# AgoraIO-Community/Solo

Measured on AMD Instinct MI355X. Metric: 40 ms frames/sec (encode+decode) per GPU; concurrent real-time WB streams @1/2/4/8 MI355X, higher is better.
Workload: dtype int32 fixed point (int16 PCM, Q-format arithmetic, bit-exact); 1 GPU; BASELINE configs[2]: 4096 synthetic 16 kHz WB streams, full encode -> two-description bitstream -...; streams_per_gpu=4096, input_workers=16, launch=single process

## Files before the change

include/solo_mi355x.h:

```cpp
#ifndef SOLO_MI355X_H
#define SOLO_MI355X_H

#include <stdint.h>

#ifdef __cplusplus
extern "C" {
#endif

typedef struct {
    int32_t mode;
    int32_t targetRate_bps;
    int32_t samplerate;
    int32_t dtx_enable;
    int32_t framesize_ms;
    int32_t joint_enable;
    int32_t joint_mode;
    int32_t useMDIndex;
} USER_Ctrl_enc;

typedef struct {
    int32_t packetLoss_perc;
    int32_t samplerate;
    int32_t framesize_ms;
    int32_t joint_enable;
// ... 44 lines not shown
int32_t solo_batch_decode_streams(solo_batch_t *b, const int32_t *d_streams, int32_t n, const uint8_t *d_bits,
                                  const int16_t *d_nbytes, const uint8_t *d_recv, int32_t n_packets, int16_t *d_pcm,
                                  int32_t *d_status, void *hip_stream);
int32_t solo_recv_decode_streams(solo_batch_t *b, const int32_t *d_streams, int32_t n, int32_t n_packets, int16_t *d_pcm,
                                 int32_t *d_status, void *hip_stream);
typedef struct {
    int32_t  play;
    int32_t  queued;
    int32_t  complete;
    int32_t  ready;
    int32_t  span;
    int32_t  head;
    uint32_t inserted, late, ahead, duplicate, bad;
    uint32_t played_both, played_md1, played_md2, played_none;
    int32_t  margin_min;
} solo_recv_report_t;
typedef struct { int32_t selected, listed; } solo_recv_report_count_t;

#define SOLO_RECV_REPORT_CLEAR_MARGIN 1

int32_t solo_recv_track(solo_batch_t *b, int32_t on, void *hip_stream);
int32_t solo_recv_report(solo_batch_t *b, const int32_t *d_streams, int32_t n,
                         const int32_t *d_min_ready, int32_t min_ready, int32_t max_span, int32_t flags,
                         solo_recv_report_t *d_reports, int32_t *d_play_list, int32_t *d_play_rows,
                         solo_recv_report_count_t *d_count, void *hip_stream);
typedef struct {
    int32_t records, records_needed;
    int64_t bytes, bytes_needed;
    int32_t empty, refused;
} solo_send_count_t;
int32_t solo_send_pack(solo_batch_t *b, const uint8_t *d_bits, const int16_t *d_nbytes, const uint8_t *d_send,
                       int32_t n_packets, const int32_t *d_seq_base, int32_t first_seq,
                       solo_arrival_t *d_records, int32_t max_records, uint8_t *d_payload, int64_t payload_capacity,
                       solo_send_count_t *d_count, void *hip_stream);
int32_t solo_send_pack_streams(solo_batch_t *b, const int32_t *d_streams, int32_t n, const uint8_t *d_bits, const int16_t *d_nbytes,
                               const uint8_t *d_send, int32_t n_packets, const int32_t *d_seq_base, int32_t first_seq,
                               solo_arrival_t *d_records, int32_t max_records, uint8_t *d_payload, int64_t payload_capacity,
                               solo_send_count_t *d_count, void *hip_stream);
typedef struct {
    int32_t rows, rooms;
    int64_t clipped;
} solo_mix_count_t;
int32_t solo_mix(solo_batch_t *b, const int16_t *d_pcm_in, int32_t n, int32_t n_packets,
                 const int32_t *d_room, int32_t n_rooms, const int16_t *d_gain_q12, int32_t max_speakers,
                 int16_t *d_pcm_out, int64_t *d_energy, uint8_t *d_mixed,
                 solo_mix_count_t *d_count, void *hip_stream);
typedef struct solo_resampler solo_resampler_t;
typedef struct { int32_t rows, listed; } solo_resample_count_t;
solo_resampler_t *solo_resample_create(int32_t n_rows, int32_t fs_in, int32_t fs_out);
void solo_resample_destroy(solo_resampler_t *r);
int32_t solo_resample_out_samples(const solo_resampler_t *r, int32_t in_samples);
int32_t solo_resample_reset(solo_resampler_t *r, void *hip_stream);
int32_t solo_resample_reset_rows(solo_resampler_t *r, const int32_t *h_rows, int32_t n, void *hip_stream);
int32_t solo_resample(solo_resampler_t *r, const int16_t *d_in, int32_t n_packets, int32_t in_samples,
                      int16_t *d_out, void *hip_stream);
int32_t solo_resample_rows(solo_resampler_t *r, const int32_t *d_rows, int32_t n, const int16_t *d_in, int32_t n_packets,
                           int32_t in_samples, int16_t *d_out, solo_resample_count_t *d_count, void *hip_stream);
typedef struct { int32_t streams, refused; int64_t bytes; } solo_migrate_count_t;
int64_t solo_batch_state_bytes(const solo_batch_t *b, int32_t which);
int32_t solo_batch_export_streams(solo_batch_t *b, const int32_t *d_streams, int32_t n, int32_t which,
                                  uint8_t *d_blob, int64_t blob_stride, solo_migrate_count_t *d_count, void *hip_stream);
int32_t solo_batch_import_streams(solo_batch_t *b, const int32_t *d_streams, int32_t n, int32_t which,
                                  const uint8_t *d_blob, int64_t blob_stride, solo_migrate_count_t *d_count, void *hip_stream);
int32_t solo_batch_set_async_join(solo_batch_t *b, int32_t on);
int32_t solo_batch_wait_encode(solo_batch_t *b, void *hip_stream, int32_t which);
int32_t solo_batch_n_streams(const solo_batch_t *b);
int32_t solo_batch_slot_bytes(const solo_batch_t *b);
const char *solo_kernel_name(int32_t which);
int32_t solo_batch_set_timing(solo_batch_t *b, int32_t on);
int32_t solo_batch_last_kernel_ms(solo_batch_t *b, float *ms4);
int32_t solo_batch_last_encode_chunks(const solo_batch_t *b);
int32_t solo_debug_l0(int32_t op, int32_t n, const int32_t *d_a, const int32_t *d_b, const int32_t *d_c, int32_t *d_out);
int32_t solo_debug_sum_sqr_shift(const int16_t *d_x, int32_t rows, int32_t len, int32_t stride, int32_t odd_start,
                                 int32_t *d_energy, int32_t *d_shift);
int32_t solo_debug_waveops(int32_t mode, int32_t n_vec, int32_t waves_per_block, const int32_t *d_v, const int32_t *d_aux,
                           int32_t *d_out);
int32_t solo_debug_rowops(const int32_t *d_in, const int32_t *d_idx, int32_t *d_out, void *hip_stream);
int32_t solo_debug_nsq(int32_t n_streams, int32_t n_packets, const void *h_in, void *h_out);
int32_t solo_debug_nsq_ex(int32_t samplerate, int32_t silk_rate_bps, int32_t useMDIndex, int32_t joint, int32_t dtx, int32_t frames_per_packet,
                          int32_t n_streams, int32_t n_packets, const void *h_in, void *h_out);
int32_t solo_debug_analysis(int32_t samplerate, int32_t silk_rate_bps, int32_t useMDIndex, int32_t joint, int32_t dtx, int32_t frames_per_packet,
                            int32_t n_streams, int32_t n_packets, int32_t chunk, const int16_t *h_pcm, void *h_nsq_in, void *h_code_in,
                            int32_t *h_sizes);
int32_t solo_debug_coding(int32_t samplerate, int32_t silk_rate_bps, int32_t useMDIndex, int32_t joint, int32_t dtx, int32_t frames_per_packet,
                          int32_t n_streams, int32_t n_packets, int32_t chunk, int32_t slot_bytes, const void *h_code_in, const void *h_nsq_out,
                          uint8_t *h_bits, int16_t *h_nbytes, int32_t *h_status);
int32_t solo_debug_dec_extract(int32_t samplerate, int32_t useMDIndex, int32_t joint, int32_t frames_per_packet, int32_t n_streams,
                               int32_t n_packets, int32_t chunk, int32_t slot_bytes, const uint8_t *h_bits, const int16_t *h_nbytes,
                               const uint8_t *h_recv, void *h_recs, int32_t *h_counts);
int32_t solo_debug_dec_synth(int32_t samplerate, int32_t useMDIndex, int32_t joint, int32_t frames_per_packet, int32_t n_streams,
                             int32_t n_packets, int32_t chunk, int32_t slot_bytes, const uint8_t *h_bits, const int16_t *h_nbytes,
                             const uint8_t *h_recv, const void *h_recs, int16_t *h_pcm, int32_t *h_status, void *h_state, int32_t state_bytes);
int32_t solo_debug_clock(double *mhz_out);
const char *solo_version(void);

#ifdef __cplusplus
}
#endif
#endif
```

solo_amd/__init__.py:

```python
import ctypes as C
import os

_HERE = os.path.dirname(os.path.abspath(__file__))
LIB_PATH = os.environ.get("SOLO_LIB_OVERRIDE") or os.path.join(_HERE, "libsolo_mi355x.so")

PACKET_SAMPLES = 640
DEFAULT_SLOT_BYTES = 512

ABI_SYMBOLS = [
    "AGR_Sate_Encoder_Init", "AGR_Sate_Encoder_Encode", "AGR_Sate_Encoder_Uninit",
    "AGR_Sate_Decoder_Init", "AGR_Sate_Decoder_Decode", "AGR_Sate_Decoder_Uninit",
    "solo_batch_create", "solo_batch_destroy", "solo_batch_reset", "solo_batch_encode", "solo_batch_decode",
    "solo_batch_n_streams", "solo_batch_slot_bytes", "solo_kernel_name", "solo_version", "solo_batch_set_timing",
    "solo_batch_last_kernel_ms", "solo_batch_last_encode_chunks", "solo_batch_decode_split", "solo_batch_set_async_join",
    "solo_batch_wait_encode", "solo_debug_l0", "solo_debug_sum_sqr_shift", "solo_debug_rowops", "solo_debug_clock", "solo_debug_nsq",
    "solo_debug_waveops", "solo_debug_nsq_ex", "solo_debug_analysis", "solo_debug_coding", "solo_debug_dec_extract", "solo_debug_dec_synth",
    "solo_recv_create", "solo_recv_insert", "solo_recv_decode", "solo_recv_stats",
    "solo_batch_reset_streams", "solo_recv_reset_streams", "solo_batch_update_streams",
    "solo_batch_encode_streams", "solo_batch_decode_streams", "solo_recv_decode_streams",
    "solo_send_pack", "solo_send_pack_streams", "solo_mix", "solo_recv_track", "solo_recv_report",
    "solo_batch_state_bytes", "solo_batch_export_streams", "solo_batch_import_streams",
    "solo_resample_create", "solo_resample_destroy", "solo_resample_out_samples", "solo_resample_reset", "solo_resample_reset_rows",
    "solo_resample", "solo_resample_rows",
]


class USER_Ctrl_enc(C.Structure):
    _fields_ = [(n, C.c_int32) for n in (
        "mode", "targetRate_bps", "samplerate", "dtx_enable", "framesize_ms",
        "joint_enable", "joint_mode", "useMDIndex")]


class USER_Ctrl_dec(C.Structure):
    _fields_ = [(n, C.c_int32) for n in (
        "packetLoss_perc", "samplerate", "framesize_ms", "joint_enable", "joint_mode", "useMDIndex")]


class solo_send_count_t(C.Structure):
    _fields_ = [("records", C.c_int32), ("records_needed", C.c_int32), ("bytes", C.c_int64), ("bytes_needed", C.c_int64),
                ("empty", C.c_int32), ("refused", C.c_int32)]


class solo_mix_count_t(C.Structure):
    _fields_ = [("rows", C.c_int32), ("rooms", C.c_int32), ("clipped", C.c_int64)]


class solo_resample_count_t(C.Structure):
    _fields_ = [("rows", C.c_int32), ("listed", C.c_int32)]


class solo_migrate_count_t(C.Structure):
    _fields_ = [("streams", C.c_int32), ("refused", C.c_int32), ("bytes", C.c_int64)]


class solo_recv_report_t(C.Structure):
    _fields_ = [(n, C.c_int32) for n in ("play", "queued", "complete", "ready", "span", "head")] + \
               [(n, C.c_uint32) for n in ("inserted", "late", "ahead", "duplicate", "bad", "played_both", "played_md1", "played_md2", "played_none")] + \
               [("margin_min", C.c_int32)]


class solo_recv_report_count_t(C.Structure):
    _fields_ = [("selected", C.c_int32), ("listed", C.c_int32)]


RECV_REPORT_CLEAR_MARGIN = 1

_lib = None


def kernel_source_hash():
    import hashlib
    h = hashlib.sha256()
    d = os.path.join(_HERE, "csrc")
    for f in sorted(os.listdir(d)):
        if f.endswith((".h", ".hip", ".inc")):
            h.update(f.encode())
            h.update(open(os.path.join(d, f), "rb").read())
    flags = build_flags()
    if flags:
        h.update(" ".join(flags).encode())
    return h.hexdigest()[:16]


def build_flags():
    p = os.path.join(_HERE, "build_flags.txt")
    if not os.path.exists(p):
        return []
    return [l.strip() for l in open(p) if l.strip() and not l.strip().startswith("#")]


def load_library():
    global _lib
    if _lib is not None:
        return _lib
    if not os.path.exists(LIB_PATH):
        raise RuntimeError("libsolo_mi355x.so is not built (%s). Run `python -c 'import __graft_entry__ as g; g.build()'`; "
                           "this package has no CPU fallback." % LIB_PATH)
    lib = C.CDLL(LIB_PATH)
    lib.solo_batch_create.restype = C.c_void_p
# ... 3 lines not shown
    lib.solo_batch_reset.restype = C.c_int32
    lib.solo_batch_reset_streams.restype = C.c_int32
    lib.solo_batch_reset_streams.argtypes = [C.c_void_p, C.c_void_p, C.c_int32, C.c_int32, C.c_void_p, C.c_void_p, C.c_void_p]
    lib.solo_batch_update_streams.restype = C.c_int32
    lib.solo_batch_update_streams.argtypes = [C.c_void_p, C.c_void_p, C.c_int32, C.c_int32, C.c_void_p, C.c_void_p, C.c_void_p]
    lib.solo_recv_reset_streams.restype = C.c_int32
    lib.solo_recv_reset_streams.argtypes = [C.c_void_p, C.c_void_p, C.c_int32, C.c_void_p, C.c_void_p]
    lib.solo_batch_encode.restype = C.c_int32
    lib.solo_batch_encode.argtypes = [C.c_void_p, C.c_void_p, C.c_int32, C.c_void_p, C.c_void_p, C.c_void_p, C.c_void_p]
    lib.solo_batch_encode_streams.restype = C.c_int32
    lib.solo_batch_encode_streams.argtypes = [C.c_void_p, C.c_void_p, C.c_int32, C.c_void_p, C.c_int32, C.c_void_p, C.c_void_p, C.c_void_p, C.c_void_p]
    lib.solo_batch_decode_streams.restype = C.c_int32
    lib.solo_batch_decode_streams.argtypes = [C.c_void_p, C.c_void_p, C.c_int32, C.c_void_p, C.c_void_p, C.c_void_p, C.c_int32, C.c_void_p, C.c_void_p,
                                              C.c_void_p]
    lib.solo_recv_decode_streams.restype = C.c_int32
    lib.solo_recv_decode_streams.argtypes = [C.c_void_p, C.c_void_p, C.c_int32, C.c_int32, C.c_void_p, C.c_void_p, C.c_void_p]
    lib.solo_batch_decode.restype = C.c_int32
    lib.solo_batch_decode.argtypes = [C.c_void_p, C.c_void_p, C.c_void_p, C.c_void_p, C.c_int32, C.c_void_p, C.c_void_p, C.c_void_p]
    lib.solo_batch_n_streams.argtypes = [C.c_void_p]
    lib.solo_batch_slot_bytes.argtypes = [C.c_void_p]
    lib.solo_batch_set_timing.restype = C.c_int32
    lib.solo_batch_set_timing.argtypes = [C.c_void_p, C.c_int32]
    lib.solo_batch_last_kernel_ms.restype = C.c_int32
    lib.solo_batch_last_kernel_ms.argtypes = [C.c_void_p, C.c_void_p]
    lib.solo_batch_decode_split.restype = C.c_int32
    lib.solo_batch_decode_split.argtypes = [C.c_void_p, C.c_void_p, C.c_void_p, C.c_void_p, C.c_void_p, C.c_int32, C.c_int32, C.c_void_p,
                                            C.c_void_p, C.c_void_p]
    lib.solo_recv_create.restype = C.c_int32
    lib.solo_recv_create.argtypes = [C.c_void_p, C.c_int32, C.c_int32, C.c_int32, C.c_void_p]
    lib.solo_recv_insert.restype = C.c_int32
    lib.solo_recv_insert.argtypes = [C.c_void_p, C.c_void_p, C.c_int32, C.c_void_p, C.c_int64, C.c_void_p]
    lib.solo_recv_decode.restype = C.c_int32
    lib.solo_recv_decode.argtypes = [C.c_void_p, C.c_int32, C.c_void_p, C.c_void_p, C.c_void_p]
    lib.solo_recv_stats.restype = C.c_int32
    lib.solo_recv_stats.argtypes = [C.c_void_p, C.c_void_p, C.c_void_p]
    lib.solo_recv_track.restype = C.c_int32
    lib.solo_recv_track.argtypes = [C.c_void_p, C.c_int32, C.c_void_p]
    lib.solo_recv_report.restype = C.c_int32
    lib.solo_recv_report.argtypes = [C.c_void_p, C.c_void_p, C.c_int32, C.c_void_p, C.c_int32, C.c_int32, C.c_int32, C.c_void_p, C.c_void_p, C.c_void_p,
                                     C.c_void_p, C.c_void_p]
    _send = [C.c_void_p, C.c_void_p, C.c_void_p, C.c_int32, C.c_void_p, C.c_int32, C.c_void_p, C.c_int32, C.c_void_p, C.c_int64, C.c_void_p, C.c_void_p]
    lib.solo_send_pack.restype = C.c_int32
    lib.solo_send_pack.argtypes = [C.c_void_p] + _send
    lib.solo_send_pack_streams.restype = C.c_int32
    lib.solo_send_pack_streams.argtypes = [C.c_void_p, C.c_void_p, C.c_int32] + _send
    lib.solo_mix.restype = C.c_int32
    lib.solo_mix.argtypes = [C.c_void_p, C.c_void_p, C.c_int32, C.c_int32, C.c_void_p, C.c_int32, C.c_void_p, C.c_int32, C.c_void_p, C.c_void_p, C.c_void_p,
                             C.c_void_p, C.c_void_p]
    lib.solo_batch_state_bytes.restype = C.c_int64
    lib.solo_batch_state_bytes.argtypes = [C.c_void_p, C.c_int32]
    for f in (lib.solo_batch_export_streams, lib.solo_batch_import_streams):
        f.restype = C.c_int32
        f.argtypes = [C.c_void_p, C.c_void_p, C.c_int32, C.c_int32, C.c_void_p, C.c_int64, C.c_void_p, C.c_void_p]
    lib.solo_resample_create.restype = C.c_void_p
    lib.solo_resample_create.argtypes = [C.c_int32, C.c_int32, C.c_int32]
    lib.solo_resample_destroy.restype = None
    lib.solo_resample_destroy.argtypes = [C.c_void_p]
    lib.solo_resample_out_samples.restype = C.c_int32
    lib.solo_resample_out_samples.argtypes = [C.c_void_p, C.c_int32]
    lib.solo_resample_reset.restype = C.c_int32
    lib.solo_resample_reset.argtypes = [C.c_void_p, C.c_void_p]
    lib.solo_resample_reset_rows.restype = C.c_int32
    lib.solo_resample_reset_rows.argtypes = [C.c_void_p, C.c_void_p, C.c_int32, C.c_void_p]
    lib.solo_resample.restype = C.c_int32
    lib.solo_resample.argtypes = [C.c_void_p, C.c_void_p, C.c_int32, C.c_int32, C.c_void_p, C.c_void_p]
    lib.solo_resample_rows.restype = C.c_int32
    lib.solo_resample_rows.argtypes = [C.c_void_p, C.c_void_p, C.c_int32, C.c_void_p, C.c_int32, C.c_int32, C.c_void_p, C.c_void_p, C.c_void_p]
    lib.solo_batch_set_async_join.restype = C.c_int32
    lib.solo_batch_set_async_join.argtypes = [C.c_void_p, C.c_int32]
    lib.solo_batch_wait_encode.restype = C.c_int32
    lib.solo_batch_wait_encode.argtypes = [C.c_void_p, C.c_void_p, C.c_int32]
    lib.solo_batch_last_encode_chunks.restype = C.c_int32
    lib.solo_batch_last_encode_chunks.argtypes = [C.c_void_p]
    lib.solo_debug_rowops.restype = C.c_int32
    lib.solo_debug_rowops.argtypes = [C.c_void_p, C.c_void_p, C.c_void_p, C.c_void_p]
    lib.solo_debug_waveops.restype = C.c_int32
    lib.solo_debug_waveops.argtypes = [C.c_int32, C.c_int32, C.c_int32, C.c_void_p, C.c_void_p, C.c_void_p]
    lib.solo_debug_nsq.restype = C.c_int32
    lib.solo_debug_nsq.argtypes = [C.c_int32, C.c_int32, C.c_void_p, C.c_void_p]
    lib.solo_debug_nsq_ex.restype = C.c_int32
    lib.solo_debug_nsq_ex.argtypes = [C.c_int32] * 8 + [C.c_void_p, C.c_void_p]
    lib.solo_debug_analysis.restype = C.c_int32
    lib.solo_debug_analysis.argtypes = [C.c_int32] * 9 + [C.c_void_p, C.c_void_p, C.c_void_p, C.c_void_p]
    lib.solo_debug_coding.restype = C.c_int32
    lib.solo_debug_coding.argtypes = [C.c_int32] * 10 + [C.c_void_p, C.c_void_p, C.c_void_p, C.c_void_p, C.c_void_p]
    lib.solo_debug_dec_extract.restype = C.c_int32
    lib.solo_debug_dec_extract.argtypes = [C.c_int32] * 8 + [C.c_void_p] * 5
    lib.solo_debug_dec_synth.restype = C.c_int32
    lib.solo_debug_dec_synth.argtypes = [C.c_int32] * 8 + [C.c_void_p] * 7 + [C.c_int32]
    lib.solo_debug_clock.restype = C.c_int32
    lib.solo_debug_clock.argtypes = [C.c_void_p]
    lib.solo_kernel_name.restype = C.c_char_p
    lib.solo_kernel_name.argtypes = [C.c_int32]
    lib.solo_version.restype = C.c_char_p
    lib.AGR_Sate_Encoder_Init.restype = C.c_void_p
    lib.AGR_Sate_Encoder_Init.argtypes = [C.c_void_p]
    lib.AGR_Sate_Encoder_Encode.restype = C.c_int32
    lib.AGR_Sate_Encoder_Encode.argtypes = [C.c_void_p, C.c_void_p, C.c_void_p, C.c_int32, C.c_void_p]
    lib.AGR_Sate_Encoder_Uninit.argtypes = [C.c_void_p]
    lib.AGR_Sate_Decoder_Init.restype = C.c_void_p
    lib.AGR_Sate_Decoder_Init.argtypes = [C.c_void_p]
    lib.AGR_Sate_Decoder_Decode.restype = C.c_int32
    lib.AGR_Sate_Decoder_Decode.argtypes = [C.c_void_p, C.c_void_p, C.c_void_p, C.c_void_p, C.c_void_p, C.c_int32]
    lib.AGR_Sate_Decoder_Uninit.argtypes = [C.c_void_p]
    _lib = lib
    return lib


def shader_clock_mhz():
    v = C.c_double(0.0)
    if load_library().solo_debug_clock(C.byref(v)) != 0:
        return None
    return float(v.value)


def default_enc_ctrl(rate=13600, use_md_index=0, joint=0, dtx=0, samplerate=16000, framesize_ms=40):
    return USER_Ctrl_enc(mode=2, targetRate_bps=rate, samplerate=samplerate, dtx_enable=1 if dtx else 0, framesize_ms=framesize_ms,
                         joint_enable=1 if joint else 0, joint_mode=1 if joint else 0, useMDIndex=use_md_index)


def default_dec_ctrl(use_md_index=0, joint=0, samplerate=16000, framesize_ms=40):
    return USER_Ctrl_dec(packetLoss_perc=0, samplerate=samplerate, framesize_ms=framesize_ms, joint_enable=1 if joint else 0,
                         joint_mode=1 if joint else 0, useMDIndex=use_md_index)


class SoloBatch:

    def __init__(self, n_streams, rate=13600, encoder=True, decoder=True, slot_bytes=DEFAULT_SLOT_BYTES, use_md_index=0, joint=0, dtx=0,
                 samplerate=16000, framesize_ms=40):
        import torch
        if not torch.cuda.is_available():
            raise RuntimeError("solo_amd needs a HIP device (MI355X); there is no CPU path")
        self.torch = torch
        self.lib = load_library()
        self.n_streams = int(n_streams)
        self.slot = int(slot_bytes)
        if framesize_ms not in (20, 40):
            raise ValueError("framesize_ms must be 40 or 20")
        self._enc = default_enc_ctrl(rate, use_md_index, joint, dtx, samplerate, framesize_ms) if encoder else None
        if samplerate not in (16000, 32000):
            raise ValueError("samplerate must be 16000 or 32000")
        self.packet_samples = PACKET_SAMPLES * samplerate // 16000 * framesize_ms // 40
        self._dec = default_dec_ctrl(use_md_index, joint, samplerate, framesize_ms) if decoder else None
        self.h = self.lib.solo_batch_create(self.n_streams, C.byref(self._enc) if encoder else None,
                                            C.byref(self._dec) if decoder else None, self.slot)
        if not self.h:
            raise RuntimeError("solo_batch_create failed (unsupported configuration, no GPU, or out of memory)")
        self.device = torch.device("cuda", torch.cuda.current_device())

    def _stream(self):
        return C.c_void_p(self.torch.cuda.current_stream().cuda_stream)

    def reset(self):
        r = self.lib.solo_batch_reset(self.h, self._stream())
        if r:
            raise RuntimeError("solo_batch_reset -> %d" % r)

    _WHICH = {"enc": 1, "encoder": 1, "dec": 2, "decoder": 2, "both": 3, 1: 1, 2: 2, 3: 3}

    def _stream_list(self, streams):
        idx = [int(s) for s in (streams.tolist() if hasattr(streams, "tolist") else streams)]
        if not 0 < len(idx) <= self.n_streams:
            raise ValueError("between 1 and %d streams must be listed" % self.n_streams)
        if any(s < 0 or s >= self.n_streams for s in idx):
            raise ValueError("stream index out of range")
        if len(set(idx)) != len(idx):
# ... 529 lines not shown
```

solo_amd/csrc/solo_api.hip:

```cpp
#include <hip/hip_runtime.h>
#include <vector>
#include <stdio.h>
#include <stdlib.h>
#include <string.h>
#include <new>

#include "../../include/solo_mi355x.h"
#include "solo_dec.h"

#define SOLO_CHECK(expr)                                        \
    do {                                                        \
        hipError_t e_ = (expr);                                 \
        if (e_ != hipSuccess) return -(int32_t)e_;              \
    } while (0)

#include "solo_dec_kernels.h"
#include "solo_l0_probe.h"
#include "solo_send.h"
#include "solo_mix.h"
#include "solo_recv_report.h"
#include "solo_migrate.h"
#include "solo_resample.h"

__global__ void __launch_bounds__(64) solo_l0_probe_kernel(int op, int n, const i32* a, const i32* b, const i32* c, i32* out) {
// ... 67 lines not shown
        i32 z = sx_lcg_first(aux0);
        ROW(21, z);
        z = sx_lcg_next(z); ROW(22, z);
        z = sx_lcg_next(z); ROW(23, z);
        z = sx_lcg_next(z); ROW(24, z);
        const i32 vmin = wv_min(v);
        ROW(25, vmin);
        ROW(26, wv_min(v == vmin ? lane : SX_I32_MAX));
    } else {
        i32 a, b, c, d, e, f, g;
        i64 h;
        SOLO_WAVEOPS_CHAIN(v)
        ROW(0, a); ROW(1, b); ROW(2, c); ROW(3, d); ROW(4, e); ROW(5, f); ROW(6, g); ROW(7, (u32)h); ROW(8, (u32)((u64)h >> 32));
        const int trips = (aux0 & 7) + 1;
        i32 x = v;
        for (int t = 0; t < trips; t++) {
            if (t) x = sx_add(sx_add(x, a), sx_add(f, sx_add(g, (i32)(u32)h)));
            SOLO_WAVEOPS_CHAIN(x)
        }
        ROW(9, a); ROW(10, b); ROW(11, c); ROW(12, d); ROW(13, e); ROW(14, f); ROW(15, g); ROW(16, (u32)h); ROW(17, (u32)((u64)h >> 32));
    }
#undef ROW
#endif
}

__global__ void __launch_bounds__(256) solo_stream_list_check_kernel(const i32* map, int n, int n_streams, u32* verdict, i32* status) {
    __shared__ int bad;
    if (threadIdx.x == 0) bad = 0;
    __syncthreads();
    int mine = 0;
    for (int i = threadIdx.x; i < n; i += 256) {
        const i32 v = map[i];
        if (v < 0 || v >= n_streams || (i > 0 && map[i - 1] >= v)) mine = 1;
    }
    if (mine) atomicOr(&bad, 1);
    __syncthreads();
    const int verdict_bad = bad;
    if (threadIdx.x == 0) *verdict = (u32)verdict_bad;
    if (verdict_bad && status)
        for (int i = threadIdx.x; i < n; i += 256) status[i] = -1;
}

extern "C" const solo_dec_ops* solo_nb_dec_ops() { return &solo_dec_ops_table; }
extern "C" const solo_dec_ops* solo_wb_dec_ops();

#ifdef SOLO_WITH_ENCODER
#include "solo_enc_ops.h"
extern "C" int solo_launch_gate(const unsigned int* flag, unsigned int target, void* hip_stream);
extern "C" const solo_enc_ops* solo_nb_enc_ops();
extern "C" const solo_enc_ops* solo_wb_enc_ops();
#endif

#define SOLO_MAX_CHUNKS 64
#define SOLO_N_VERDICTS 10
struct solo_batch {
    int32_t n_streams;
    int32_t slot;
    int have_enc, have_dec;
    USER_Ctrl_enc enc_ctrl;
    USER_Ctrl_dec dec_ctrl;
    void* d_enc_state;
#ifdef SOLO_WITH_ENCODER
    const solo_enc_ops* eops;
#endif
    void* d_nsq_ring;
    hipStream_t sP, sS;
    hipEvent_t evDFork, evDJoin, evDJoin2, evP[2], evS[2];
    void* d_parsed[2];
    size_t parsed_bytes;
    int parsed_two;
    int dec_pipe_ready, dec_split, dec_chunk, dec_first;
    size_t dec_scratch_cap;
    unsigned int dec_calls;
    void* d_rc_scratch;
    size_t rc_scratch_bytes;
    void* d_enc_work;
    int32_t enc_work_packets;
    int timing;
    hipEvent_t evDec[2];
    int ev_ready, ev_enc, ev_dec;
    int pipe_ready, chunk_packets;
    hipStream_t sA, sB, sC;
    hipEvent_t evFork, evJoinA[2], evJoinC[2], evA[SOLO_MAX_CHUNKS], evB[SOLO_MAX_CHUNKS], evC[SOLO_MAX_CHUNKS];
    int async_join;
    unsigned int enc_seq;
    int evC_valid;
    int last_np, last_cp;
    hipEvent_t tev[3][SOLO_MAX_CHUNKS][2];
    int tev_ready, last_chunks;
    unsigned int* d_started;
    unsigned int started_target[SOLO_MAX_CHUNKS];
    int group_streams;
    int gate;
    int persist;
    int persist_group;
    unsigned int* d_flags;
    unsigned int ticket;
    unsigned int final_wait_ticks;
    int front_defer;
    void* d_nsq_stage;
    void* d_front_scratch;
    const solo_dec_ops* dops;
    void* d_dec_state;
    uint8_t* d_recv_ring;
    uint32_t* d_recv_lens;
    int32_t* d_recv_play;
    uint32_t* d_recv_stats;
    int32_t recv_depth, recv_slot;
    uint32_t* d_recv_trk;
    int recv_track;
    int32_t* d_recv_sel;
    uint32_t* d_verdict;
    void* d_send_scratch;
    size_t send_scratch_bytes;
    void* d_mix_scratch;
    size_t mix_scratch_bytes;
};

static int ctrl_hb_joint(int joint_enable, int joint_mode) { return joint_enable != 0 && joint_mode == 1; }
static int ctrl_silk_rate(const USER_Ctrl_enc* c) { return c->targetRate_bps - (ctrl_hb_joint(c->joint_enable, c->joint_mode) ? 800 : 1600); }
static bool ctrl_enc_supported(const USER_Ctrl_enc* c) {
    if (!(c->framesize_ms == 40 || (c->framesize_ms == 20 && c->joint_enable == 0)) || !(c->joint_enable == 0 || c->joint_mode == 1)) return false;
    if (c->samplerate == 16000) return true;
    USER_Ctrl_enc d = *c;
    if (d.targetRate_bps <= 0) d.targetRate_bps = 15600;
    return c->samplerate == 32000 && ctrl_silk_rate(&d) >= 14000;
}
static bool ctrl_dec_supported(const USER_Ctrl_dec* c) {
    return (c->samplerate == 16000 || c->samplerate == 32000) && (c->framesize_ms == 40 || (c->framesize_ms == 20 && c->joint_enable == 0)) &&
           (c->joint_enable == 0 || c->joint_mode == 1);
}
static int ctrl_hb_bytes(int joint_enable, int joint_mode, int framesize_ms) { return (ctrl_hb_joint(joint_enable, joint_mode) || framesize_ms == 20) ? SX_HB_BYTES / 2 : SX_HB_BYTES; }
static int ctrl_frames_per_packet(int framesize_ms) { return framesize_ms == 20 ? 1 : 2; }
static int ctrl_packet_samples(int samples_40ms, int framesize_ms) { return framesize_ms == 20 ? samples_40ms / 2 : samples_40ms; }
static int dec_packet_samples(const solo_batch* b) { return ctrl_packet_samples(b->dops->packet_samples, b->dec_ctrl.framesize_ms); }
static int dec_hb_mode(const solo_batch* b) { return ctrl_hb_joint(b->dec_ctrl.joint_enable, b->dec_ctrl.joint_mode) | (ctrl_frames_per_packet(b->dec_ctrl.framesize_ms) == 1 ? 2 : 0); }

static int env_int(const char* name, int dflt) {
    const char* e = getenv(name);
    return e ? atoi(e) : dflt;
}
template <typename T>
static void dev_free(T*& p) {
    if (p) (void)hipFree(p);
    p = NULL;
}

#ifdef SOLO_WITH_ENCODER
static int enc_hb_joint(const solo_batch* b) { return ctrl_hb_joint(b->enc_ctrl.joint_enable, b->enc_ctrl.joint_mode); }
static int enc_frames_per_packet(const solo_batch* b) { return ctrl_frames_per_packet(b->enc_ctrl.framesize_ms); }
static int enc_packet_samples(const solo_batch* b) { return ctrl_packet_samples(b->eops->packet_samples, b->enc_ctrl.framesize_ms); }
static int32_t solo_enc_reset(solo_batch* b, hipStream_t s) {
    SOLO_CHECK(b->eops->init(b->d_enc_state, b->n_streams, ctrl_silk_rate(&b->enc_ctrl), b->enc_ctrl.useMDIndex, enc_hb_joint(b),
                             b->enc_ctrl.dtx_enable ? 1 : 0, enc_frames_per_packet(b), s));
    return 0;
}
static void solo_enc_free(solo_batch* b) {
    dev_free(b->d_enc_state);
    dev_free(b->d_enc_work);
    dev_free(b->d_nsq_ring);
    dev_free(b->d_rc_scratch);
    dev_free(b->d_flags);
    dev_free(b->d_front_scratch);
    dev_free(b->d_nsq_stage);
}
#endif
// ... 138 lines not shown
    std::vector<SxStreamCtl> er, dr;
    if (!stream_ctl_records(b, h_streams, n, which, h_enc, h_dec, er, dr)) return -1;
    {
        const int32_t r = solo_wait_in_flight(b, s);
        if (r) return r;
    }
    if (!dr.empty()) SOLO_CHECK(reinit ? b->dops->init_list(b->d_dec_state, dr.data(), n, dec_hb_mode(b), s) : b->dops->ctl_list(b->d_dec_state, dr.data(), n, s));
#ifdef SOLO_WITH_ENCODER
    if (!er.empty())
        SOLO_CHECK(reinit ? b->eops->init_list(b->d_enc_state, er.data(), n, enc_hb_joint(b), enc_frames_per_packet(b), s)
                          : b->eops->ctl_list(b->d_enc_state, er.data(), n, s));
#endif
    return 0;
}
int32_t solo_batch_reset_streams(solo_batch_t* b, const int32_t* h_streams, int32_t n, int32_t which, const USER_Ctrl_enc* h_enc,
                                 const USER_Ctrl_dec* h_dec, void* hip_stream) {
    return stream_ctl_apply(b, true, h_streams, n, which, h_enc, h_dec, (hipStream_t)hip_stream);
}
int32_t solo_batch_update_streams(solo_batch_t* b, const int32_t* h_streams, int32_t n, int32_t which, const USER_Ctrl_enc* h_enc,
                                  const USER_Ctrl_dec* h_dec, void* hip_stream) {
    return stream_ctl_apply(b, false, h_streams, n, which, h_enc, h_dec, (hipStream_t)hip_stream);
}

solo_batch_t* solo_batch_create(int32_t n_streams, const USER_Ctrl_enc* enc, const USER_Ctrl_dec* dec, int32_t slot_bytes) {
    if (n_streams <= 0) return NULL;
    int ndev = 0;
    if (hipGetDeviceCount(&ndev) != hipSuccess || ndev <= 0) {
        fprintf(stderr, "solo_mi355x: no HIP device available -- this library has no CPU path\n");
        return NULL;
    }
    if (enc && !ctrl_enc_supported(enc)) return NULL;
    if (dec && !ctrl_dec_supported(dec)) return NULL;
    solo_batch* b = new (std::nothrow) solo_batch();
    if (!b) return NULL;
    memset(b, 0, sizeof(*b));
    b->n_streams = n_streams;
    b->slot = slot_bytes > 0 ? slot_bytes : SOLO_DEFAULT_SLOT_BYTES;
    if (enc) {
#ifdef SOLO_WITH_ENCODER
        b->have_enc = 1;
        b->enc_ctrl = *enc;
        if (b->enc_ctrl.targetRate_bps <= 0) b->enc_ctrl.targetRate_bps = 15600;
        b->eops = enc->samplerate == 32000 ? solo_wb_enc_ops() : solo_nb_enc_ops();
        if (hipMalloc(&b->d_enc_state, b->eops->state_bytes * (size_t)n_streams) != hipSuccess) { solo_batch_destroy(b); return NULL; }
#else
        delete b;
        return NULL;
#endif
    }
    if (dec) {
        b->have_dec = 1;
        b->dec_ctrl = *dec;
        b->dops = dec->samplerate == 32000 ? solo_wb_dec_ops() : solo_nb_dec_ops();
        if (enc && enc->samplerate != dec->samplerate) { solo_batch_destroy(b); return NULL; }
        if (hipMalloc(&b->d_dec_state, b->dops->state_bytes * (size_t)n_streams) != hipSuccess) { solo_batch_destroy(b); return NULL; }
    }
    if (hipMalloc((void**)&b->d_verdict, SOLO_N_VERDICTS * sizeof(uint32_t)) != hipSuccess || hipMemset(b->d_verdict, 0, SOLO_N_VERDICTS * sizeof(uint32_t)) != hipSuccess) {
        solo_batch_destroy(b);
        return NULL;
    }
    if (solo_batch_reset(b, NULL) != 0 || hipDeviceSynchronize() != hipSuccess) { solo_batch_destroy(b); return NULL; }
    return b;
}

static void solo_recv_free(solo_batch_t* b);
void solo_batch_destroy(solo_batch_t* b) {
    if (!b) return;
    solo_recv_free(b);
    dev_free(b->d_recv_trk);
    if (b->dec_pipe_ready && b->dec_split) {
        (void)hipStreamSynchronize(b->sP); (void)hipStreamSynchronize(b->sS);
        (void)hipStreamDestroy(b->sP); (void)hipStreamDestroy(b->sS);
        (void)hipEventDestroy(b->evDFork); (void)hipEventDestroy(b->evDJoin); (void)hipEventDestroy(b->evDJoin2);
        for (int i = 0; i < 2; i++) { (void)hipEventDestroy(b->evP[i]); (void)hipEventDestroy(b->evS[i]); }
    }
    for (int i = 0; i < 2; i++) dev_free(b->d_parsed[i]);
    dev_free(b->d_dec_state);
    dev_free(b->d_verdict);
    dev_free(b->d_send_scratch);
    dev_free(b->d_mix_scratch);
    if (b->ev_ready) for (int i = 0; i < 2; i++) (void)hipEventDestroy(b->evDec[i]);
    if (b->tev_ready) for (int k = 0; k < 3; k++) for (int c = 0; c < SOLO_MAX_CHUNKS; c++) for (int e = 0; e < 2; e++) (void)hipEventDestroy(b->tev[k][c][e]);
    if (b->pipe_ready) {
        (void)hipStreamSynchronize(b->sA); (void)hipStreamSynchronize(b->sB); (void)hipStreamSynchronize(b->sC);
        (void)hipStreamDestroy(b->sA); (void)hipStreamDestroy(b->sB); (void)hipStreamDestroy(b->sC);
        dev_free(b->d_started);
        (void)hipEventDestroy(b->evFork);
        for (int i = 0; i < 2; i++) { (void)hipEventDestroy(b->evJoinA[i]); (void)hipEventDestroy(b->evJoinC[i]); }
        for (int c = 0; c < SOLO_MAX_CHUNKS; c++) (void)hipEventDestroy(b->evC[c]);
        for (int c = 0; c < SOLO_MAX_CHUNKS; c++) { (void)hipEventDestroy(b->evA[c]); (void)hipEventDestroy(b->evB[c]); }
    }
#ifdef SOLO_WITH_ENCODER
    solo_enc_free(b);
#endif
    delete b;
}

#define SOLO_DEC_FIRST_CHUNK 64
#define SOLO_DEC_CHUNK_DEFAULT 64
static_assert(2 * sizeof(SxExtracted) + 8 == 2216, "include/solo_mi355x.h documents 2216 bytes of extraction records (2 x 1104 B + two list entries) per packet (16 kHz API rate)");
static int32_t solo_decode_impl(solo_batch_t* b, const int32_t* map, int32_t n, const uint8_t* d_bits, const int16_t* d_nbytes, const uint8_t* d_recv,
                                int32_t n_packets, int16_t* d_pcm, int32_t* d_status, hipStream_t st) {
    const int ns = map ? n : b->n_streams;
    uint32_t* verdict = map ? b->d_verdict + 2 : NULL;
    const bool tm = b->timing && b->ev_ready;
    if (!b->dec_pipe_ready) {
        b->dec_split = env_int("SOLO_DEC_SPLIT", 1);
        if (ctrl_frames_per_packet(b->dec_ctrl.framesize_ms) == 1) b->dec_split = 0;
        b->dec_chunk = env_int("SOLO_DEC_CHUNK", SOLO_DEC_CHUNK_DEFAULT);
        if (b->dec_chunk <= 0) b->dec_chunk = 1 << 30;
        b->dec_first = env_int("SOLO_DEC_FIRST_CHUNK", SOLO_DEC_FIRST_CHUNK);
        if (b->dec_first <= 0) b->dec_first = SOLO_DEC_FIRST_CHUNK;
        const char* e = getenv("SOLO_DEC_SCRATCH_CAP");
        b->dec_scratch_cap = e ? (size_t)strtoull(e, NULL, 10) : 0;
        if (b->dec_scratch_cap == 0) b->dec_scratch_cap = (size_t)1 << 30;
        if (b->dec_split) {
            SOLO_CHECK(hipStreamCreateWithFlags(&b->sP, hipStreamNonBlocking));
            SOLO_CHECK(hipStreamCreateWithFlags(&b->sS, hipStreamNonBlocking));
            SOLO_CHECK(hipEventCreateWithFlags(&b->evDFork, hipEventDisableTiming));
            SOLO_CHECK(hipEventCreateWithFlags(&b->evDJoin, hipEventDisableTiming));
            SOLO_CHECK(hipEventCreateWithFlags(&b->evDJoin2, hipEventDisableTiming));
            for (int i = 0; i < 2; i++) {
                SOLO_CHECK(hipEventCreateWithFlags(&b->evP[i], hipEventDisableTiming));
                SOLO_CHECK(hipEventCreateWithFlags(&b->evS[i], hipEventDisableTiming));
            }
        }
        b->dec_pipe_ready = 1;
    }
    if (tm) (void)hipEventRecord(b->evDec[0], st);
    if (!b->dec_split) {
        if (map) SOLO_CHECK(launch_list_check(b, map, n, verdict, d_status, st));
        const hipError_t e = b->dops->decode(b->d_dec_state, d_bits, d_nbytes, d_recv, ns, n_packets, b->slot, d_pcm, d_status, map, verdict, st);
        if (tm) { (void)hipEventRecord(b->evDec[1], st); b->ev_dec = 1; }
        SOLO_CHECK(e);
        return 0;
    }
    const size_t rec_bytes = b->dops->extracted_bytes;
    int cp = n_packets < b->dec_chunk ? n_packets : b->dec_chunk;
    {
        const size_t fit = b->dec_scratch_cap / ((size_t)ns * rec_bytes);
        if ((size_t)cp > fit) cp = fit < 1 ? 1 : (int)fit;
    }
    const int c0 = (n_packets > 2 * b->dec_first && cp > b->dec_first) ? b->dec_first : cp;
    const int nchunks = 1 + (n_packets - c0 + cp - 1) / cp;
    const size_t need = (size_t)ns * (size_t)cp * rec_bytes + 256;
    if (need > b->parsed_bytes || (nchunks > 1 && !b->parsed_two)) {
        SOLO_CHECK(hipStreamSynchronize(st));
        (void)hipStreamSynchronize(b->sP);
        (void)hipStreamSynchronize(b->sS);
        for (int i = 0; i < 2; i++) dev_free(b->d_parsed[i]);
        b->parsed_bytes = 0;
        for (int i = 0; i < 2; i++) SOLO_CHECK(hipMalloc(&b->d_parsed[i], i == 0 || nchunks > 1 ? need : 256));
        b->parsed_bytes = need;
        b->parsed_two = nchunks > 1;
    }
    if (b->dec_calls > 0) {
        SOLO_CHECK(hipStreamWaitEvent(st, b->evDJoin, 0));
        SOLO_CHECK(hipStreamWaitEvent(st, b->evDJoin2, 0));
    }
    if (map) SOLO_CHECK(launch_list_check(b, map, n, verdict, d_status, st));
    SOLO_CHECK(hipEventRecord(b->evDFork, st));
    SOLO_CHECK(hipStreamWaitEvent(b->sP, b->evDFork, 0));
    SOLO_CHECK(hipStreamWaitEvent(b->sS, b->evDFork, 0));
    b->dec_calls++;
    hipError_t lerr = hipSuccess;
    for (int c = 0; c < nchunks && lerr == hipSuccess; c++) {
        const int p0 = c == 0 ? 0 : c0 + (c - 1) * cp, pc = c == 0 ? c0 : ((p0 + cp <= n_packets) ? cp : n_packets - p0), k = c & 1;
        if (c >= 2 && (lerr = hipStreamWaitEvent(b->sP, b->evS[k], 0)) != hipSuccess) break;
// ... 277 lines not shown
}
int32_t solo_resample(solo_resampler_t* r, const int16_t* d_in, int32_t n_packets, int32_t in_samples, int16_t* d_out, void* hip_stream) {
    if (!r) return -1;
    return resample_call(r, NULL, r->n_rows, d_in, n_packets, in_samples, d_out, NULL, (hipStream_t)hip_stream);
}
int32_t solo_resample_rows(solo_resampler_t* r, const int32_t* d_rows, int32_t n, const int16_t* d_in, int32_t n_packets, int32_t in_samples,
                           int16_t* d_out, solo_resample_count_t* d_count, void* hip_stream) {
    if (!r || !d_rows || !d_count) return -1;
    return resample_call(r, d_rows, n, d_in, n_packets, in_samples, d_out, d_count, (hipStream_t)hip_stream);
}

static_assert(sizeof(solo_migrate_count_t) == sizeof(SxMigCount), "include/solo_mi355x.h and solo_migrate.h agree");
static bool migrate_which_ok(const solo_batch* b, int32_t which) {
    return b && which > 0 && which <= SX_MIG_ALL && !((which & SX_MIG_ENC) && !b->have_enc) && !((which & SX_MIG_DEC) && !b->have_dec) &&
           !((which & SX_MIG_RECV) && !b->d_recv_ring);
}
static SxMigHandle migrate_handle(const solo_batch* b) {
    SxMigHandle h;
    memset(&h, 0, sizeof(h));
    h.n_streams = b->n_streams;
#ifdef SOLO_WITH_ENCODER
    if (b->have_enc) {
        h.enc = (uint8_t*)b->d_enc_state;
        h.g.enc_rate = b->enc_ctrl.samplerate; h.g.enc_mode = sx_mig_mode(enc_frames_per_packet(b), enc_hb_joint(b)); h.g.enc_bytes = (int32_t)b->eops->state_bytes;
    }
#endif
    if (b->have_dec) {
        h.dec = (uint8_t*)b->d_dec_state;
        h.g.dec_rate = b->dec_ctrl.samplerate;
        h.g.dec_mode = sx_mig_mode(ctrl_frames_per_packet(b->dec_ctrl.framesize_ms), ctrl_hb_joint(b->dec_ctrl.joint_enable, b->dec_ctrl.joint_mode));
        h.g.dec_bytes = (int32_t)b->dops->state_bytes;
    }
    if (b->d_recv_ring) {
        h.ring = b->d_recv_ring; h.lens = b->d_recv_lens; h.play = b->d_recv_play; h.trk = b->d_recv_trk;
        h.g.depth = b->recv_depth; h.g.slot = b->recv_slot;
    }
    return h;
}
int64_t solo_batch_state_bytes(const solo_batch_t* b, int32_t which) {
    if (!migrate_which_ok(b, which)) return -1;
    const SxMigHandle h = migrate_handle(b);
    return SX_MIG_HDR_BYTES + sx_mig_body_bytes(sx_mig_geom_of(h.g, which), which);
}
static bool migrate_args_ok(const solo_batch* b, const int32_t* d_streams, int32_t n, int32_t which, const uint8_t* d_blob, int64_t blob_stride,
                            const solo_migrate_count_t* d_count) {
    if (!migrate_which_ok(b, which) || !d_streams || !d_blob || !d_count || n <= 0 || n > b->n_streams) return false;
    return blob_stride >= solo_batch_state_bytes(b, which) && !(blob_stride & 15) && !((uintptr_t)d_blob & 15);
}
int32_t solo_batch_export_streams(solo_batch_t* b, const int32_t* d_streams, int32_t n, int32_t which, uint8_t* d_blob, int64_t blob_stride,
                                  solo_migrate_count_t* d_count, void* hip_stream) {
    if (!migrate_args_ok(b, d_streams, n, which, d_blob, blob_stride, d_count)) return -1;
    hipStream_t st = (hipStream_t)hip_stream;
    {
        const int32_t r = solo_wait_in_flight(b, st);
        if (r) return r;
    }
    uint32_t* verdict = b->d_verdict + 7;
    SOLO_CHECK(launch_list_check(b, d_streams, n, verdict, NULL, st));
    SOLO_CHECK(solo_migrate_export_launch(migrate_handle(b), d_streams, n, which, d_blob, (long long)blob_stride, (SxMigCount*)d_count, verdict, st));
    return 0;
}
int32_t solo_batch_import_streams(solo_batch_t* b, const int32_t* d_streams, int32_t n, int32_t which, const uint8_t* d_blob, int64_t blob_stride,
                                  solo_migrate_count_t* d_count, void* hip_stream) {
    if (!migrate_args_ok(b, d_streams, n, which, d_blob, blob_stride, d_count)) return -1;
    hipStream_t st = (hipStream_t)hip_stream;
    {
        const int32_t r = solo_wait_in_flight(b, st);
        if (r) return r;
    }
    uint32_t* verdict = b->d_verdict + 8;
    SOLO_CHECK(launch_list_check(b, d_streams, n, verdict, NULL, st));
    SOLO_CHECK(solo_migrate_import_launch(migrate_handle(b), d_streams, n, which, d_blob, (long long)blob_stride, (SxMigCount*)d_count, verdict, st));
    return 0;
}

#ifdef SOLO_WITH_ENCODER
static int32_t solo_enc_pipe_setup(solo_batch* b) {
    const solo_enc_ops* ops = b->eops;
    int lo = 0, hi = 0;
    (void)hipDeviceGetStreamPriorityRange(&lo, &hi);
    SOLO_CHECK(hipStreamCreateWithPriority(&b->sA, hipStreamNonBlocking, lo));
    SOLO_CHECK(hipStreamCreateWithPriority(&b->sB, hipStreamNonBlocking, hi));
    SOLO_CHECK(hipStreamCreateWithPriority(&b->sC, hipStreamNonBlocking, lo));
    SOLO_CHECK(hipEventCreateWithFlags(&b->evFork, hipEventDisableTiming));
    for (int i = 0; i < 2; i++) {
        SOLO_CHECK(hipEventCreateWithFlags(&b->evJoinA[i], hipEventDisableTiming));
        SOLO_CHECK(hipEventCreateWithFlags(&b->evJoinC[i], hipEventDisableTiming));
    }
    for (int c = 0; c < SOLO_MAX_CHUNKS; c++) {
        SOLO_CHECK(hipEventCreateWithFlags(&b->evA[c], hipEventDisableTiming));
        SOLO_CHECK(hipEventCreateWithFlags(&b->evB[c], hipEventDisableTiming));
        SOLO_CHECK(hipEventCreateWithFlags(&b->evC[c], hipEventDisableTiming));
    }
    int dev = 0, ncu = 0;
    SOLO_CHECK(hipGetDevice(&dev));
    SOLO_CHECK(hipDeviceGetAttribute(&ncu, hipDeviceAttributeMultiprocessorCount, dev));
    b->persist = env_int("SOLO_ENC_PERSIST", 0) != 0;
    b->chunk_packets = env_int("SOLO_ENC_CHUNK", 1);
    if (b->chunk_packets < 0) b->chunk_packets = 1;
    b->gate = getenv("SOLO_ENC_GATE") ? (env_int("SOLO_ENC_GATE", 0) != 0) : -1;
    const int g_env = env_int("SOLO_ENC_GROUP", -1);
    b->group_streams = g_env >= 0 ? g_env : 8192;
    b->persist_group = g_env > 0 ? ((g_env + 3) & ~3) : ((ops->front_per_cu * (ncu > 0 ? ncu : 256)) & ~3);
    if (b->persist_group < 4) b->persist_group = 4;
    {
        const long us = env_int("SOLO_ENC_FINAL_WAIT_US", 20000);
        b->front_defer = us < 0;
        b->final_wait_ticks = (unsigned int)((us < 0 ? 0 : (us > 10000000 ? 10000000 : us)) * 100);
    }
    {
        int gs = (b->group_streams > 0 && b->group_streams < b->n_streams) ? b->group_streams : b->n_streams;
        if (b->persist && b->persist_group > gs) gs = b->persist_group < b->n_streams ? b->persist_group : b->n_streams;
        SOLO_CHECK(hipMalloc(&b->d_nsq_ring, ops->nsq_ring_bytes(gs)));
    }
    SOLO_CHECK(hipMalloc((void**)&b->d_started, SOLO_MAX_CHUNKS * sizeof(unsigned int)));
    SOLO_CHECK(hipMemset(b->d_started, 0, SOLO_MAX_CHUNKS * sizeof(unsigned int)));
    memset(b->started_target, 0, sizeof(b->started_target));
    if (b->persist) {
        const size_t nflags = (size_t)b->n_streams * 2 + (size_t)b->n_streams / 4 + 1 + 4;
        SOLO_CHECK(hipMalloc((void**)&b->d_flags, nflags * sizeof(unsigned int)));
        SOLO_CHECK(hipMemset(b->d_flags, 0, nflags * sizeof(unsigned int)));
        const int gs = b->persist_group < b->n_streams ? b->persist_group : b->n_streams;
        SOLO_CHECK(hipMalloc(&b->d_front_scratch, ops->front_scratch_bytes(gs)));
        SOLO_CHECK(hipMalloc(&b->d_nsq_stage, ops->nsq_stage_bytes(gs)));
    }
    b->ticket = 0;
    b->pipe_ready = 1;
    return 0;
}

static int32_t solo_encode_persist(solo_batch* b, const int16_t* d_pcm, int32_t n_packets, uint8_t* d_bits, int16_t* d_nbytes, int32_t* d_status,
                                   hipStream_t st, void* nin, void* nout, void* cin) {
    const solo_enc_ops* ops = b->eops;
    const int G = b->persist_group, ngroups = (b->n_streams + G - 1) / G;
    const bool tm = b->timing && b->tev_ready && ngroups <= SOLO_MAX_CHUNKS;
    unsigned int* ana = b->d_flags;
    unsigned int* nsqf = ana + b->n_streams;
    unsigned int* prog = nsqf + (size_t)b->n_streams / 4 + 1;
    unsigned int* err = prog + b->n_streams;
    const unsigned int ticket0 = b->ticket;
    b->ticket += (unsigned int)n_packets;
    const size_t frame_samples = (size_t)enc_packet_samples(b);
    SOLO_CHECK(hipEventRecord(b->evFork, st));
    SOLO_CHECK(hipStreamWaitEvent(b->sA, b->evFork, 0));
    SOLO_CHECK(hipStreamWaitEvent(b->sB, b->evFork, 0));
    if (b->enc_seq > 0) {
        const int jp = (int)((b->enc_seq - 1u) & 1u);
        SOLO_CHECK(hipStreamWaitEvent(b->sA, b->evJoinC[jp], 0));
        SOLO_CHECK(hipStreamWaitEvent(b->sB, b->evJoinC[jp], 0));
        SOLO_CHECK(hipStreamWaitEvent(b->sB, b->evJoinA[jp], 0));
    }
    b->evC_valid = 0;
    b->last_np = n_packets;
    b->last_cp = 0;
    hipError_t lerr = hipSuccess;
    for (int g = 0; g < ngroups && lerr == hipSuccess; g++) {
        const int s0 = g * G, ns = (s0 + G <= b->n_streams) ? G : b->n_streams - s0, c = g % SOLO_MAX_CHUNKS;
        const size_t pk0 = (size_t)s0 * (size_t)n_packets;
        void* g_states = (char*)b->d_enc_state + (size_t)s0 * ops->state_bytes;
        void* g_nin = (char*)nin + pk0 * 2 * ops->nsq_in_bytes;
        void* g_nout = (char*)nout + pk0 * 2 * ops->nsq_out_bytes;
        void* g_cin = (char*)cin + pk0 * ops->code_in_bytes;
        const int16_t* g_pcm = d_pcm + pk0 * frame_samples;
        uint8_t* g_bits = d_bits + pk0 * (size_t)b->slot;
        int16_t* g_nbytes = d_nbytes + pk0 * 2;
        int32_t* g_status = d_status ? d_status + s0 : NULL;
        if ((lerr = hipEventRecord(b->evA[c], b->sA)) != hipSuccess) break;
        if ((lerr = hipStreamWaitEvent(b->sB, b->evA[c], 0)) != hipSuccess) break;
        if (tm) (void)hipEventRecord(b->tev[0][c][0], b->sA);
        lerr = ops->front(g_states, g_pcm, ns, n_packets, g_nin, g_cin, g_nout, ana + s0, nsqf + s0 / 4, prog + s0, ticket0, b->front_defer ? 2 : 0, b->final_wait_ticks, b->slot,
                          g_bits, g_nbytes, g_status, b->d_front_scratch, &b->d_started[c], b->sA);
        if (lerr != hipSuccess) break;
        b->started_target[c] += (unsigned int)((ns + ops->front_waves - 1) / ops->front_waves);
        if (tm) (void)hipEventRecord(b->tev[0][c][1], b->sA);
        if (b->gate != 0) (void)solo_launch_gate(&b->d_started[c], b->started_target[c], b->sB);
        if (tm) (void)hipEventRecord(b->tev[1][c][0], b->sB);
        lerr = (hipError_t)ops->nsq_persist(g_states, g_nin, g_nout, ns, n_packets, NULL, b->d_nsq_ring, ana + s0, nsqf + s0 / 4, ticket0, err, b->d_nsq_stage, b->sB);
        if (lerr != hipSuccess) break;
        if (tm) (void)hipEventRecord(b->tev[1][c][1], b->sB);
        if ((lerr = hipEventRecord(b->evB[c], b->sB)) != hipSuccess) break;
        if ((lerr = hipStreamWaitEvent(b->sA, b->evB[c], 0)) != hipSuccess) break;
        if (tm) (void)hipEventRecord(b->tev[2][c][0], b->sA);
        lerr = ops->front(g_states, g_pcm, ns, n_packets, g_nin, g_cin, g_nout, ana + s0, nsqf + s0 / 4, prog + s0, ticket0, 1, 0u, b->slot, g_bits, g_nbytes,
                          g_status, b->d_front_scratch, NULL, b->sA);
        if (tm) (void)hipEventRecord(b->tev[2][c][1], b->sA);
    }
    const int js = (int)(b->enc_seq & 1u);
    b->enc_seq++;
    (void)hipEventRecord(b->evJoinA[js], b->sA);
    (void)hipEventRecord(b->evJoinC[js], b->sB);
    if (!b->async_join || lerr != hipSuccess) {
        (void)hipStreamWaitEvent(st, b->evJoinA[js], 0);
        (void)hipStreamWaitEvent(st, b->evJoinC[js], 0);
    }
    b->last_chunks = (lerr == hipSuccess && (tm || ngroups <= SOLO_MAX_CHUNKS)) ? ngroups : 0;
    if (tm && lerr == hipSuccess) b->ev_enc = 1;
    SOLO_CHECK(lerr);
    SOLO_CHECK(hipGetLastError());
    return 0;
}

static int32_t solo_encode_impl(solo_batch_t* b, const int32_t* map, int32_t n, const int16_t* d_pcm, int32_t n_packets, uint8_t* d_bits, int16_t* d_nbytes,
                                int32_t* d_status, hipStream_t st) {
    const size_t np = (size_t)b->n_streams * (size_t)n_packets;
    const solo_enc_ops* ops = b->eops;
    if (map && (unsigned long long)b->n_streams * (unsigned long long)ops->state_bytes >= (1ull << 32)) return -1;
    const unsigned long long per_wave = 64ull / (unsigned long long)ops->nsq_workgroups(64);
    if (((per_wave - 1ull) * 2ull * (unsigned long long)n_packets + 1ull) * (unsigned long long)ops->nsq_out_bytes >= (1ull << 32)) return -1;
    const size_t sz_in = np * 2 * ops->nsq_in_bytes, sz_out = np * 2 * ops->nsq_out_bytes, sz_code = np * ops->code_in_bytes;
    if (n_packets > b->enc_work_packets) {
        SOLO_CHECK(hipStreamSynchronize(st));
        if (b->pipe_ready) { (void)hipStreamSynchronize(b->sA); (void)hipStreamSynchronize(b->sB); (void)hipStreamSynchronize(b->sC); }
        dev_free(b->d_enc_work);
        SOLO_CHECK(hipMalloc(&b->d_enc_work, sz_in + sz_out + sz_code + 256));
        b->enc_work_packets = n_packets;
    }
    void* nin = b->d_enc_work;
    void* nout = (char*)b->d_enc_work + ((sz_in + 63) & ~(size_t)63);
    void* cin = (char*)nout + ((sz_out + 63) & ~(size_t)63);
    void* states = b->d_enc_state;
    if (!b->pipe_ready) {
        const int32_t r = solo_enc_pipe_setup(b);
        if (r) return r;
    }
    if (!map && b->persist && n_packets >= 2) return solo_encode_persist(b, d_pcm, n_packets, d_bits, d_nbytes, d_status, st, nin, nout, cin);

    int cp = b->chunk_packets > 0 ? b->chunk_packets : n_packets;
    int nchunks = (n_packets + cp - 1) / cp;
    if (nchunks > SOLO_MAX_CHUNKS) { cp = (n_packets + SOLO_MAX_CHUNKS - 1) / SOLO_MAX_CHUNKS; nchunks = (n_packets + cp - 1) / cp; }
    {
        const int gs = (b->group_streams > 0 && b->group_streams < b->n_streams) ? b->group_streams : b->n_streams;
        const size_t need = ops->rc_scratch_bytes(gs, cp);
        if (need > b->rc_scratch_bytes) {
            if (b->d_rc_scratch) {
                SOLO_CHECK(hipStreamSynchronize(b->sC));
                dev_free(b->d_rc_scratch);
                b->rc_scratch_bytes = 0;
            }
            SOLO_CHECK(hipMalloc(&b->d_rc_scratch, need));
            b->rc_scratch_bytes = need;
        }
    }
    const bool tm_req = b->timing && b->tev_ready;
    uint32_t* verdict = NULL;
    if (map) {
        b->evC_valid = 0;
        verdict = b->d_verdict + (b->enc_seq & 1u);
        if (b->enc_seq >= 2) {
            SOLO_CHECK(hipStreamWaitEvent(st, b->evJoinA[b->enc_seq & 1u], 0));
            SOLO_CHECK(hipStreamWaitEvent(st, b->evJoinC[b->enc_seq & 1u], 0));
        }
        SOLO_CHECK(launch_list_check(b, map, n, verdict, d_status, st));
    }
    if (b->enc_seq > 0 && (b->last_np != n_packets || b->last_cp != cp || b->evC_valid == 0)) {
        SOLO_CHECK(hipStreamWaitEvent(b->sA, b->evJoinC[(b->enc_seq - 1u) & 1u], 0));
        SOLO_CHECK(hipStreamWaitEvent(b->sB, b->evJoinA[(b->enc_seq - 1u) & 1u], 0));
        b->evC_valid = 0;
    }
    b->last_np = n_packets;
    b->last_cp = cp;
    SOLO_CHECK(hipEventRecord(b->evFork, st));
    SOLO_CHECK(hipStreamWaitEvent(b->sA, b->evFork, 0));
    SOLO_CHECK(hipStreamWaitEvent(b->sB, b->evFork, 0));
    SOLO_CHECK(hipStreamWaitEvent(b->sC, b->evFork, 0));
    const int nall = map ? n : b->n_streams;
    const int G = b->group_streams > 0 ? b->group_streams : nall;
    const int ngroups = (nall + G - 1) / G;
    const bool tm = tm_req && (size_t)ngroups * (size_t)nchunks <= SOLO_MAX_CHUNKS;
    const size_t frame_samples = (size_t)enc_packet_samples(b);
    int idx = 0;
    hipError_t lerr = hipSuccess;
    for (int g = 0; g < ngroups && lerr == hipSuccess; g++) {
        const int s0 = g * G, ns = (s0 + G <= nall) ? G : nall - s0;
        const size_t pk0 = (size_t)s0 * (size_t)n_packets;
        void* g_states = map ? states : (char*)states + (size_t)s0 * ops->state_bytes;
        const int32_t* g_map = map ? map + s0 : NULL;
        const int16_t* g_pcm = d_pcm + pk0 * frame_samples;
        void* g_nin = (char*)nin + pk0 * 2 * ops->nsq_in_bytes;
        void* g_nout = (char*)nout + pk0 * 2 * ops->nsq_out_bytes;
        void* g_cin = (char*)cin + pk0 * ops->code_in_bytes;
        uint8_t* g_bits = d_bits + pk0 * (size_t)b->slot;
        int16_t* g_nbytes = d_nbytes + pk0 * 2;
        int32_t* g_status = d_status ? d_status + s0 : NULL;
        for (int cc = 0; cc < nchunks; cc++, idx++) {
            const int c = idx % SOLO_MAX_CHUNKS, cprev = (idx + SOLO_MAX_CHUNKS - 1) % SOLO_MAX_CHUNKS;
            const int p0 = cc * cp, pc = (p0 + cp <= n_packets) ? cp : n_packets - p0;
            if (ngroups == 1 && cc < b->evC_valid) SOLO_CHECK(hipStreamWaitEvent(b->sA, b->evC[c], 0));
            if (idx > 0 && b->gate > 0) (void)solo_launch_gate(&b->d_started[cprev], b->started_target[cprev], b->sA);
            if (tm) (void)hipEventRecord(b->tev[0][c][0], b->sA);
            if ((lerr = ops->analysis(g_states, g_pcm, ns, n_packets, p0, pc, g_nin, g_cin, g_map, verdict, b->sA)) != hipSuccess) break;
            if (tm) (void)hipEventRecord(b->tev[0][c][1], b->sA);
            SOLO_CHECK(hipEventRecord(b->evA[c], b->sA));
            SOLO_CHECK(hipStreamWaitEvent(b->sB, b->evA[c], 0));
            if (tm) (void)hipEventRecord(b->tev[1][c][0], b->sB);
#ifdef SX_EXPERIMENTS
            static const int exp_skip = env_int("SOLO_EXP_SKIP", 0);
#else
            constexpr int exp_skip = 0;
#endif
            if (!(exp_skip & 1)) {
            if ((lerr = (hipError_t)ops->nsq(g_states, g_nin, g_nout, ns, n_packets, p0, pc, &b->d_started[c], b->d_nsq_ring, g_map, verdict, b->sB)) != hipSuccess) break;
            b->started_target[c] += (unsigned int)ops->nsq_workgroups(ns);
            }
            if (tm) (void)hipEventRecord(b->tev[1][c][1], b->sB);
            SOLO_CHECK(hipEventRecord(b->evB[c], b->sB));
            SOLO_CHECK(hipStreamWaitEvent(b->sC, b->evB[c], 0));
            if (tm) (void)hipEventRecord(b->tev[2][c][0], b->sC);
            if (!(exp_skip & 2))
            if ((lerr = ops->coding(g_states, g_cin, g_nout, ns, n_packets, p0, pc, b->slot, g_bits, g_nbytes, g_status, b->d_rc_scratch, g_map, verdict, b->sC)) != hipSuccess) break;
            if (tm) (void)hipEventRecord(b->tev[2][c][1], b->sC);
            SOLO_CHECK(hipEventRecord(b->evC[c], b->sC));
        }
    }
    const bool ok = lerr == hipSuccess;
    b->evC_valid = (ok && ngroups == 1 && !map) ? nchunks : 0;
    const int js = (int)(b->enc_seq & 1u);
    b->enc_seq++;
    (void)hipEventRecord(b->evJoinA[js], b->sA);
    (void)hipEventRecord(b->evJoinC[js], b->sC);
    if (!b->async_join || !ok) {
        (void)hipStreamWaitEvent(st, b->evJoinA[js], 0);
        (void)hipStreamWaitEvent(st, b->evJoinC[js], 0);
    }
    if (!ok) {
        (void)hipEventRecord(b->evFork, b->sB);
        (void)hipStreamWaitEvent(st, b->evFork, 0);
    }
    b->last_chunks = !ok ? 0 : (tm ? ngroups * nchunks : (ngroups == 1 ? nchunks : 0));
    if (tm && ok) b->ev_enc = 1;
    SOLO_CHECK(lerr);
    SOLO_CHECK(hipGetLastError());
    return 0;
}
int32_t solo_batch_encode(solo_batch_t* b, const int16_t* d_pcm, int32_t n_packets, uint8_t* d_bits, int16_t* d_nbytes,
                          int32_t* d_status, void* hip_stream) {
    if (!b || !b->have_enc || !d_pcm || !d_bits || !d_nbytes || n_packets <= 0) return -1;
    return solo_encode_impl(b, NULL, 0, d_pcm, n_packets, d_bits, d_nbytes, d_status, (hipStream_t)hip_stream);
}
int32_t solo_batch_encode_streams(solo_batch_t* b, const int32_t* d_streams, int32_t n, const int16_t* d_pcm, int32_t n_packets, uint8_t* d_bits,
                                  int16_t* d_nbytes, int32_t* d_status, void* hip_stream) {
    if (!b || !b->have_enc || !d_streams || n <= 0 || n > b->n_streams || !d_pcm || !d_bits || !d_nbytes || n_packets <= 0) return -1;
    return solo_encode_impl(b, d_streams, n, d_pcm, n_packets, d_bits, d_nbytes, d_status, (hipStream_t)hip_stream);
}
#else
int32_t solo_batch_encode(solo_batch_t*, const int16_t*, int32_t, uint8_t*, int16_t*, int32_t*, void*) { return -1; }
int32_t solo_batch_encode_streams(solo_batch_t*, const int32_t*, int32_t, const int16_t*, int32_t, uint8_t*, int16_t*, int32_t*, void*) { return -1; }
#endif

struct solo_single {
    solo_batch* b;
    uint8_t* d_blk;
    uint8_t* h_blk;
    int16_t* d_pcm;
    uint8_t* d_bits;
    int16_t* d_nbytes;
    int32_t* d_status;
    int is_enc;
};
#define SOLO_SINGLE_PCM_OFF 16
#define SOLO_SINGLE_NB_OFF (16 + 2 * SX_PACKET * 2)
#define SOLO_SINGLE_BITS_OFF (SOLO_SINGLE_NB_OFF + 16)

static void single_free(solo_single* h) {
    if (!h) return;
    if (h->d_blk) (void)hipFree(h->d_blk);
    if (h->h_blk) (void)hipHostFree(h->h_blk);
    solo_batch_destroy(h->b);
    free(h);
}

static solo_single* single_new(const USER_Ctrl_enc* e, const USER_Ctrl_dec* d) {
    solo_single* h = (solo_single*)calloc(1, sizeof(solo_single));
    if (!h) return NULL;
    h->is_enc = e != NULL;
    h->b = solo_batch_create(1, e, d, 1024 + 64);
    const size_t blk = h->b ? (size_t)SOLO_SINGLE_BITS_OFF + (size_t)h->b->slot : 0;
    if (!h->b || hipHostMalloc((void**)&h->h_blk, blk, hipHostMallocDefault) != hipSuccess) { single_free(h); return NULL; }
    memset(h->h_blk, 0, blk);
    if (hipMalloc((void**)&h->d_blk, blk) != hipSuccess || hipMemset(h->d_blk, 0, blk) != hipSuccess) {
        single_free(h);
        return NULL;
    }
    h->d_status = (int32_t*)h->d_blk;
    h->d_pcm = (int16_t*)(h->d_blk + SOLO_SINGLE_PCM_OFF);
    h->d_nbytes = (int16_t*)(h->d_blk + SOLO_SINGLE_NB_OFF);
    h->d_bits = h->d_blk + SOLO_SINGLE_BITS_OFF;
    return h;
}

void* AGR_Sate_Encoder_Init(USER_Ctrl_enc* enc_Ctrl) {
    if (!enc_Ctrl) return NULL;
    if (enc_Ctrl->targetRate_bps <= 0) enc_Ctrl->targetRate_bps = 15600;
    return single_new(enc_Ctrl, NULL);
}

int32_t AGR_Sate_Encoder_Encode(void* st, const int16_t* pcm, uint8_t* bits, int32_t bufSize, int16_t* nBytesOut) {
    solo_single* h = (solo_single*)st;
    if (!h || !h->is_enc) return -1;
    const size_t pcm_bytes = (size_t)enc_packet_samples(h->b) * 2;
    memcpy(h->h_blk + SOLO_SINGLE_PCM_OFF, pcm, pcm_bytes);
// ... 138 lines not shown
        return -1;
    const size_t rec = (ops->extracted_bytes - 2 * sizeof(uint32_t)) / 2;
    const size_t np = (size_t)n_streams * n_packets, sz_bits = np * (size_t)slot_bytes, sz_nb = np * 2 * sizeof(int16_t);
    const size_t samples = (size_t)(ops->packet_samples / 2 * frames_per_packet), sz_pcm = np * samples * sizeof(int16_t), sz_st = (size_t)n_streams * sizeof(int32_t);
    const int cp = chunk > 0 && chunk < n_packets ? chunk : n_packets;
    const size_t sz_recs = (size_t)n_streams * cp * ops->extracted_bytes + 256;
    void *st = NULL, *d_bits = NULL, *d_nb = NULL, *d_recv = NULL, *d_recs = NULL, *d_pcm = NULL, *d_status = NULL;
    int32_t rc = -1;
    bool ok = hipMalloc(&st, ops->state_bytes * (size_t)n_streams) == hipSuccess && hipMalloc(&d_bits, sz_bits) == hipSuccess && hipMalloc(&d_nb, sz_nb) == hipSuccess &&
              hipMalloc(&d_pcm, sz_pcm) == hipSuccess && hipMalloc(&d_status, sz_st) == hipSuccess && hipMalloc(&d_recv, np) == hipSuccess &&
              (!h_recs || hipMalloc(&d_recs, sz_recs) == hipSuccess) && hipMemset(d_pcm, 0, sz_pcm) == hipSuccess && hipMemset(d_status, 0xFF, sz_st) == hipSuccess &&
              ops->init(st, n_streams, (joint ? 1 : 0) | (frames_per_packet == 1 ? 2 : 0), useMDIndex, (hipStream_t)0) == hipSuccess;
    if (ok && h_recs) {
        ok = hipMemcpy(d_bits, h_bits, sz_bits, hipMemcpyHostToDevice) == hipSuccess && hipMemcpy(d_nb, h_nbytes, sz_nb, hipMemcpyHostToDevice) == hipSuccess &&
             (h_recv ? hipMemcpy(d_recv, h_recv, np, hipMemcpyHostToDevice) : hipMemset(d_recv, 3, np)) == hipSuccess;
    }
    int launch = 0;
    for (int p0 = 0; ok && p0 < n_packets; p0 += cp, launch++) {
        const int pc = p0 + cp <= n_packets ? cp : n_packets - p0;
        if (h_recs) {
            ok = hipMemcpy2D(d_recs, (size_t)pc * 2 * rec, (const char*)h_recs + (size_t)p0 * 2 * rec, (size_t)n_packets * 2 * rec, (size_t)pc * 2 * rec, (size_t)n_streams,
                             hipMemcpyHostToDevice) == hipSuccess &&
                 ops->synth(st, (const uint8_t*)d_bits, (const int16_t*)d_nb, (const uint8_t*)d_recv, n_streams, n_packets, p0, pc, slot_bytes, d_recs, (int16_t*)d_pcm,
                            (int32_t*)d_status, NULL, NULL, (hipStream_t)0) == hipSuccess && hipDeviceSynchronize() == hipSuccess &&
                 hipMemcpy2D(h_pcm + (size_t)p0 * samples, (size_t)n_packets * samples * 2, (const int16_t*)d_pcm + (size_t)p0 * samples, (size_t)n_packets * samples * 2,
                             (size_t)pc * samples * 2, (size_t)n_streams, hipMemcpyDeviceToHost) == hipSuccess;
        } else {
            ok = hipMemcpy2D(d_bits, (size_t)pc * slot_bytes, h_bits + (size_t)p0 * slot_bytes, (size_t)n_packets * slot_bytes, (size_t)pc * slot_bytes, (size_t)n_streams,
                             hipMemcpyHostToDevice) == hipSuccess &&
                 hipMemcpy2D(d_nb, (size_t)pc * 4, h_nbytes + (size_t)p0 * 2, (size_t)n_packets * 4, (size_t)pc * 4, (size_t)n_streams, hipMemcpyHostToDevice) == hipSuccess &&
                 (h_recv ? hipMemcpy2D(d_recv, (size_t)pc, h_recv + p0, (size_t)n_packets, (size_t)pc, (size_t)n_streams, hipMemcpyHostToDevice) : hipMemset(d_recv, 3, np)) ==
                     hipSuccess &&
                 ops->decode(st, (const uint8_t*)d_bits, (const int16_t*)d_nb, (const uint8_t*)d_recv, n_streams, pc, slot_bytes, (int16_t*)d_pcm, (int32_t*)d_status, NULL,
                             NULL, (hipStream_t)0) == hipSuccess && hipDeviceSynchronize() == hipSuccess &&
                 hipMemcpy2D(h_pcm + (size_t)p0 * samples, (size_t)n_packets * samples * 2, d_pcm, (size_t)pc * samples * 2, (size_t)pc * samples * 2, (size_t)n_streams,
                             hipMemcpyDeviceToHost) == hipSuccess;
        }
        ok = ok && hipMemcpy(h_status + (size_t)launch * n_streams, d_status, sz_st, hipMemcpyDeviceToHost) == hipSuccess &&
             (!h_state || hipMemcpy2D((char*)h_state + (size_t)launch * n_streams * state_bytes, (size_t)state_bytes, st, ops->state_bytes, (size_t)state_bytes,
                                      (size_t)n_streams, hipMemcpyDeviceToHost) == hipSuccess);
    }
    if (ok) rc = (int32_t)rec;
    (void)hipFree(st); (void)hipFree(d_bits); (void)hipFree(d_nb); (void)hipFree(d_recv); (void)hipFree(d_recs); (void)hipFree(d_pcm); (void)hipFree(d_status);
    return rc;
}

#ifdef SOLO_WITH_ENCODER
static const solo_enc_ops* debug_enc_ops(int32_t samplerate) { return samplerate == 16000 ? solo_nb_enc_ops() : (samplerate == 32000 ? solo_wb_enc_ops() : NULL); }
static bool debug_enc_args(const solo_enc_ops* ops, int32_t fpp, int32_t n_streams, int32_t n_packets) {
    return ops && (fpp == 1 || fpp == 2) && n_streams > 0 && n_packets > 0 && (long long)n_streams * n_packets <= (1 << 20);
}
int32_t solo_debug_nsq_ex(int32_t samplerate, int32_t silk_rate_bps, int32_t useMDIndex, int32_t joint, int32_t dtx, int32_t frames_per_packet,
                          int32_t n_streams, int32_t n_packets, const void* h_in, void* h_out) {
    const solo_enc_ops* ops = debug_enc_ops(samplerate);
    if (!debug_enc_args(ops, frames_per_packet, n_streams, n_packets) || !h_in || !h_out) return -1;
    const size_t sz_in = (size_t)n_streams * n_packets * 2 * ops->nsq_in_bytes, sz_out = (size_t)n_streams * n_packets * 2 * ops->nsq_out_bytes;
    void *st = NULL, *d_in = NULL, *d_out = NULL, *ring = NULL;
    int32_t rc = -1;
    if (hipMalloc(&st, ops->state_bytes * (size_t)n_streams) == hipSuccess && hipMalloc(&d_in, sz_in) == hipSuccess && hipMalloc(&d_out, sz_out) == hipSuccess &&
        hipMalloc(&ring, ops->nsq_ring_bytes(n_streams)) == hipSuccess && hipMemset(d_out, 0, sz_out) == hipSuccess &&
        ops->init(st, n_streams, silk_rate_bps, useMDIndex, joint, dtx, frames_per_packet, (hipStream_t)0) == hipSuccess &&
        hipMemcpy(d_in, h_in, sz_in, hipMemcpyHostToDevice) == hipSuccess &&
        ops->nsq(st, d_in, d_out, n_streams, n_packets, 0, n_packets, NULL, ring, NULL, NULL, NULL) == 0 && hipDeviceSynchronize() == hipSuccess &&
        hipMemcpy(h_out, d_out, sz_out, hipMemcpyDeviceToHost) == hipSuccess)
        rc = (int32_t)ops->nsq_out_bytes;
    (void)hipFree(st); (void)hipFree(d_in); (void)hipFree(d_out); (void)hipFree(ring);
    return rc;
}
int32_t solo_debug_nsq(int32_t n_streams, int32_t n_packets, const void* h_in, void* h_out) {
    return solo_debug_nsq_ex(16000, 12000, 0, 0, 0, 2, n_streams, n_packets, h_in, h_out);
}
int32_t solo_debug_analysis(int32_t samplerate, int32_t silk_rate_bps, int32_t useMDIndex, int32_t joint, int32_t dtx, int32_t frames_per_packet,
                            int32_t n_streams, int32_t n_packets, int32_t chunk, const int16_t* h_pcm, void* h_nsq_in, void* h_code_in, int32_t* h_sizes) {
    const solo_enc_ops* ops = debug_enc_ops(samplerate);
    if (!ops) return -1;
    if (h_sizes) {
        h_sizes[0] = (int32_t)ops->nsq_in_bytes; h_sizes[1] = (int32_t)ops->nsq_out_bytes; h_sizes[2] = (int32_t)ops->code_in_bytes;
        h_sizes[3] = ops->packet_samples; h_sizes[4] = ops->front_waves;
    }
    if (n_streams == 0) return (int32_t)ops->nsq_in_bytes;
    if (!debug_enc_args(ops, frames_per_packet, n_streams, n_packets) || chunk < 0 || !h_pcm || !h_nsq_in || !h_code_in) return -1;
    const size_t np = (size_t)n_streams * n_packets;
    const size_t sz_pcm = np * (size_t)(ops->packet_samples / 2 * frames_per_packet) * 2, sz_in = np * 2 * ops->nsq_in_bytes, sz_code = np * ops->code_in_bytes;
    void *st = NULL, *d_pcm = NULL, *d_in = NULL, *d_code = NULL;
    int32_t rc = -1;
    const int cp = chunk > 0 ? chunk : n_packets;
    bool ok = hipMalloc(&st, ops->state_bytes * (size_t)n_streams) == hipSuccess && hipMalloc(&d_pcm, sz_pcm) == hipSuccess && hipMalloc(&d_in, sz_in) == hipSuccess &&
              hipMalloc(&d_code, sz_code) == hipSuccess && hipMemset(d_in, 0, sz_in) == hipSuccess && hipMemset(d_code, 0, sz_code) == hipSuccess &&
              ops->init(st, n_streams, silk_rate_bps, useMDIndex, joint, dtx, frames_per_packet, (hipStream_t)0) == hipSuccess &&
              hipMemcpy(d_pcm, h_pcm, sz_pcm, hipMemcpyHostToDevice) == hipSuccess;
    for (int p0 = 0; ok && p0 < n_packets; p0 += cp)
        ok = ops->analysis(st, (const int16_t*)d_pcm, n_streams, n_packets, p0, p0 + cp <= n_packets ? cp : n_packets - p0, d_in, d_code, NULL, NULL, (hipStream_t)0) == hipSuccess;
    if (ok && hipDeviceSynchronize() == hipSuccess && hipMemcpy(h_nsq_in, d_in, sz_in, hipMemcpyDeviceToHost) == hipSuccess &&
        hipMemcpy(h_code_in, d_code, sz_code, hipMemcpyDeviceToHost) == hipSuccess)
        rc = (int32_t)ops->nsq_in_bytes;
    (void)hipFree(st); (void)hipFree(d_pcm); (void)hipFree(d_in); (void)hipFree(d_code);
    return rc;
}
int32_t solo_debug_coding(int32_t samplerate, int32_t silk_rate_bps, int32_t useMDIndex, int32_t joint, int32_t dtx, int32_t frames_per_packet,
                          int32_t n_streams, int32_t n_packets, int32_t chunk, int32_t slot_bytes, const void* h_code_in, const void* h_nsq_out,
                          uint8_t* h_bits, int16_t* h_nbytes, int32_t* h_status) {
    const solo_enc_ops* ops = debug_enc_ops(samplerate);
    if (!debug_enc_args(ops, frames_per_packet, n_streams, n_packets) || chunk < 0 || slot_bytes <= 0 || slot_bytes > 4096 || !h_code_in || !h_nsq_out || !h_bits ||
        !h_nbytes || !h_status)
        return -1;
    const size_t np = (size_t)n_streams * n_packets;
    const size_t sz_code = np * ops->code_in_bytes, sz_out = np * 2 * ops->nsq_out_bytes, sz_bits = np * (size_t)slot_bytes, sz_nb = np * 2 * sizeof(int16_t),
                 sz_st = (size_t)n_streams * sizeof(int32_t);
    const int cp = chunk > 0 && chunk < n_packets ? chunk : n_packets;
    void *st = NULL, *d_code = NULL, *d_out = NULL, *d_bits = NULL, *d_nb = NULL, *d_status = NULL, *scratch = NULL;
    int32_t rc = -1;
    bool ok = hipMalloc(&st, ops->state_bytes * (size_t)n_streams) == hipSuccess && hipMalloc(&d_code, sz_code) == hipSuccess && hipMalloc(&d_out, sz_out) == hipSuccess &&
              hipMalloc(&d_bits, sz_bits) == hipSuccess && hipMalloc(&d_nb, sz_nb) == hipSuccess && hipMalloc(&d_status, sz_st) == hipSuccess &&
              hipMalloc(&scratch, ops->rc_scratch_bytes(n_streams, cp)) == hipSuccess && hipMemset(d_bits, 0, sz_bits) == hipSuccess &&
              hipMemset(d_nb, 0xFF, sz_nb) == hipSuccess && hipMemset(d_status, 0xFF, sz_st) == hipSuccess &&
              ops->init(st, n_streams, silk_rate_bps, useMDIndex, joint, dtx, frames_per_packet, (hipStream_t)0) == hipSuccess &&
              hipMemcpy(d_code, h_code_in, sz_code, hipMemcpyHostToDevice) == hipSuccess && hipMemcpy(d_out, h_nsq_out, sz_out, hipMemcpyHostToDevice) == hipSuccess;
    for (int p0 = 0; ok && p0 < n_packets; p0 += cp)
        ok = ops->coding(st, d_code, d_out, n_streams, n_packets, p0, p0 + cp <= n_packets ? cp : n_packets - p0, slot_bytes, (uint8_t*)d_bits, (int16_t*)d_nb,
                         (int32_t*)d_status, scratch, NULL, NULL, (hipStream_t)0) == hipSuccess;
    if (ok && hipDeviceSynchronize() == hipSuccess && hipMemcpy(h_bits, d_bits, sz_bits, hipMemcpyDeviceToHost) == hipSuccess &&
        hipMemcpy(h_nbytes, d_nb, sz_nb, hipMemcpyDeviceToHost) == hipSuccess && hipMemcpy(h_status, d_status, sz_st, hipMemcpyDeviceToHost) == hipSuccess)
        rc = (int32_t)ops->code_in_bytes;
    (void)hipFree(st); (void)hipFree(d_code); (void)hipFree(d_out); (void)hipFree(d_bits); (void)hipFree(d_nb); (void)hipFree(d_status); (void)hipFree(scratch);
    return rc;
}
#endif

#if defined(SX_PROF)
int32_t solo_debug_prof(unsigned long long* out64, int32_t reset) {
    if (hipMemcpyFromSymbol(out64, HIP_SYMBOL(g_sx_prof), 64 * sizeof(unsigned long long)) != hipSuccess) return -1;
    if (reset) {
        unsigned long long z[64] = {0};
        if (hipMemcpyToSymbol(HIP_SYMBOL(g_sx_prof), z, sizeof(z)) != hipSuccess) return -1;
    }
    return 0;
}
#endif

#if defined(SX_STOPS)
int32_t solo_debug_stop_dec(int32_t site_hit) { return hipMemcpyToSymbol(HIP_SYMBOL(g_sx_stop), &site_hit, sizeof(site_hit)) == hipSuccess ? 0 : -1; }
int32_t solo_debug_site_hits_dec(unsigned long long* out64, int32_t reset) {
    if (hipMemcpyFromSymbol(out64, HIP_SYMBOL(g_sx_site_hits), 128 * sizeof(unsigned long long)) != hipSuccess) return -1;
    if (reset) {
        unsigned long long z[128] = {0};
        if (hipMemcpyToSymbol(HIP_SYMBOL(g_sx_site_hits), z, sizeof(z)) != hipSuccess) return -1;
    }
    return 0;
}
#endif

}
```

solo_amd/csrc/solo_enc.h:

```cpp
#pragma once
#include <stddef.h>
#include "solo_enc_analysis.h"
#if defined(SOLO_HOST_EMU)
#include "solo_enc_nsq_row.h"
#endif
#include "solo_cdf.h"

struct SxFrameIdx {
    i32 sigtype, QuantOffsetType;
    i32 GainsIndices[SX_NB_SUBFR], DeltaGainsIndices;
    i32 NLSFIndices[SX_NLSF_STAGES], NLSFInterpCoef_Q2;
    i32 lagIndex, contourIndex, PERIndex, LTPIndex[SX_NB_SUBFR], LTP_scaleIndex;
    i32 Seed, vadFlag;
    i32 inDTX, pad_;
};

#define SX_RC_PW_SIGNS (SX_FRAME + 2 * (SX_FRAME / 16) + 8 - ((SX_FRAME + 2 * (SX_FRAME / 16)) & 7))
#define SX_RC_PW_ROW (SX_RC_PW_SIGNS + SX_FRAME / 8 + (((SX_RC_PW_SIGNS + SX_FRAME / 8) / 4) & 1 ? 0 : 4))
static_assert(((SX_RC_PW_ROW / 4) & 1) == 1 && SX_RC_PW_ROW % 4 == 0, "odd dword rows");
#define SX_RC_BUF_STRIDE (SX_MAX_ARITHM_BYTES + 16)
struct SxRcInfo { i32 nBytes, error; };

struct SxCodeWork {
#if SX_NLANES == 1
    u8 buf[2][SX_RC_BUF_STRIDE];
    alignas(4) u8 pulses[SX_RC_PW_ROW];
    SxCdf cdf;
#else
    i32 unused_;
#endif
};

struct SxFrontWork {
    i16 x_buf[SX_XBUF];
    i16 res_pitch[2 * SX_FRAME + SX_LA_PITCH];
    i16 Wsig[SX_PITCH_LPC_WIN];
    union {
        SxPitchWork pitch;
        SxShapeWork shape;
        SxPredWork pred;
        SxPrefWork pref;
    } u;
};

struct SxHbWork {
    i16 x_hb_buf[SX_HB_XBUF];
    i16 lpc_in[4 * (10 * SX_FS_KHZ + SX_HB_LPC)];
    i16 exc[2 * SX_FRAME];
    i32 NLSF_Q15[SX_MAX_LPC];
    i32 weight[SX_MAX_LPC];
    i16 A_Q12[SX_MAX_LPC];
    i32 ws[SX_NLSF2A_WS];
    SxLpcWork lpc;
};

#define SX_HB_Q (SX_FS_KHZ == 8 ? 10 : 8)
struct SxEncWork {
    SxEncState st;
    SxEncCtrl ctrl;
    i16 xfw[SX_FRAME];
    u8 hb_bytes[8 * SX_HB_Q];
    union {
        i16 qmf_tl[63 + SX_PACKET];
        SxFrontWork front;
#if defined(SOLO_HOST_EMU)
        SxRowWork nsq;
#endif
        SxCodeWork code;
        SxHbWork hb;
    } u;
};

SX_HD void sx_enc_split(SxRangeEnc* rc, int p_child1, int p, const u16* shell_table, const SxCdf* cdf) {
    if (p > 0) sx_rc_enc(rc, p_child1, &shell_table[cdf->shell_offsets[p]]);
}

SX_HD void sx_shell_encoder(SxRangeEnc* rc, const u8* pa, int sh, const SxCdf* cdf) {
    i32 p0[16], p1[8], p2[4], p3[2], p4;
    for (int k = 0; k < 16; k++) p0[k] = (i32)pa[k] >> sh;
    for (int k = 0; k < 8; k++) p1[k] = p0[2 * k] + p0[2 * k + 1];
    for (int k = 0; k < 4; k++) p2[k] = p1[2 * k] + p1[2 * k + 1];
    for (int k = 0; k < 2; k++) p3[k] = p2[2 * k] + p2[2 * k + 1];
    p4 = p3[0] + p3[1];
    sx_enc_split(rc, p3[0], p4, cdf->cdf_shell3, cdf);
    for (int h = 0; h < 2; h++) {
// ... 238 lines not shown
#if defined(SX_LANE_STREAM)
    if (__builtin_amdgcn_ballot_w64(!sx_row_nlsf2a_stable_n<SX_HB_LPC>(A_Q12, NLSF_Q15)) != 0)
#endif
    {
        wv_sync();
        if (SX_LANE == 0) sx_nlsf2a_stable_ws(SX_VPTR(A_Q12), SX_VPTR(NLSF_Q15), SX_HB_LPC, SX_VPTR(hw->ws));
    }
    wv_sync();
    SX_S(61)
    u32 word = (u32)hb_lsp_idx << 20;
    SX_PAR(t, N) {
        const int sub = t / sub_len, k = t - sub * sub_len;
        const i16* in = xb + N + sub * sub_len;
        i32 acc = 0;
        for (int j = 0; j < SX_HB_LPC; j++) {
            int u = k - 1 - j;
            if (u >= 0) acc = sx_smlabb(acc, in[u], A_Q12[j]);
        }
        i32 o = sx_sub_sat32(sx_shl((i32)in[k], 12), acc);
        exc[t] = (i16)sx_sat16(sx_rshift_round(o, 12));
    }
    wv_sync();
    SX_S(62)
#ifdef SX_LANE_STREAM
    {
        const int sub = SX_LANE >> 4, jl = SX_LANE & 15;
        i32 res_nrg0 = 0, res_nrg1 = 0;
        for (int i = jl; i < sub_len; i += 16) {
            const int n = sub * sub_len + i;
            const i32 e = exc[n];
            res_nrg0 = sx_add(res_nrg0, sx_mul(e, e));
            i32 tmp = sx_pub_ld(n < SX_FRAME ? &residue0[n] : &residue1[n - SX_FRAME]) >> 10;
            res_nrg1 = sx_smlabb(res_nrg1, tmp, tmp);
        }
        res_nrg0 = sx_sqrt_approx(wv_row_sum(res_nrg0));
        res_nrg1 = sx_sqrt_approx(wv_row_sum(res_nrg1));
        const i16 gain = (i16)(sx_shl(res_nrg0 + 1, 4) / (res_nrg1 + 1));
        i32 bv = SX_I32_MAX, bi = SX_I32_MAX;
        for (int i = jl; i < 32; i += 16) {
            i16 tmp = (i16)(gain - T_hb_gain_cb[i]);
            const i32 dist = sx_smulbb(tmp, tmp);
            if (dist < bv) { bv = dist; bi = i; }
        }
        SX_ARG_STEP(0xB1, <) SX_ARG_STEP(0x4E, <) SX_ARG_STEP(0x141, <) SX_ARG_STEP(0x140, <)
#pragma unroll
        for (int r = 0; r < 4; r++) word |= (u32)__builtin_amdgcn_readlane(bi, 16 * r) << (15 - 5 * r);
    }
#else
    for (int sub = 0; sub < 4; sub++) {
        i32 res_nrg0 = 0, res_nrg1 = 0;
        SX_PAR(i, sub_len) {
            const int n = sub * sub_len + i;
            const i32 e = exc[n];
            res_nrg0 = sx_add(res_nrg0, sx_mul(e, e));
            i32 tmp = sx_pub_ld(n < SX_FRAME ? &residue0[n] : &residue1[n - SX_FRAME]) >> 10;
            res_nrg1 = sx_smlabb(res_nrg1, tmp, tmp);
        }
        res_nrg0 = wv_sum(res_nrg0);
        res_nrg1 = wv_sum(res_nrg1);
        res_nrg0 = sx_sqrt_approx(res_nrg0);
        res_nrg1 = sx_sqrt_approx(res_nrg1);
        const i16 gain = (i16)(sx_shl(res_nrg0 + 1, 4) / (res_nrg1 + 1));
        i32 min_dist = SX_I32_MAX;
        int gidx = SX_I32_MAX;
        SX_PAR(i, 32) {
            i16 tmp = (i16)(gain - T_hb_gain_cb[i]);
            const i32 dist = sx_smulbb(tmp, tmp);
            if (dist < min_dist) { min_dist = dist; gidx = i; }
        }
        wv_argmin(&min_dist, &gidx);
        word |= (u32)gidx << (15 - 5 * sub);
    }
#endif
    SX_S(45)
    out4[0] = (u8)(word >> 24); out4[1] = (u8)(word >> 16); out4[2] = (u8)(word >> 8); out4[3] = (u8)word;
    SX_PAR(i, N + SX_HB_DELAY) hist->x_hb_buf[i] = xb[N + i];
    wv_sync();
}

#ifndef SX_ENC_TAP
#define SX_ENC_TAP(stage, st, w, sig)
#endif

SX_FNW void sx_enc_analyse_frame(SxEncStream* rec, SxEncWork* w, const i16* pIn, int frame, SxNsqIn* in, SxFrameIdx* x) {
    SX_IN_LDS(w);
    SxEncHist* hist = &rec->hist;
    SxEncState* st = &w->st;
    SxEncCtrl* c = &w->ctrl;
    SxFrontWork* f = &w->u.front;
    c->Seed = st->frameCounter++ & 3;
    i32 SNR_dB_Q7;
    SX_T_BEGIN
    SX_PAR(i, SX_FRAME + SX_LA_SHAPE) f->x_buf[i] = hist->x_buf[i];
    SX_PAR(i, SX_FRAME) f->res_pitch[i] = pIn[i];
    wv_sync();
    SX_STRETCH_LATENCY();
    constexpr int vad_bands_ = 240 + SX_FRAME / 2;
    static_assert(offsetof(SxFrontWork, u) == offsetof(SxFrontWork, Wsig) + sizeof(f->Wsig) && (offsetof(SxFrontWork, Wsig) + vad_bands_ * sizeof(i16)) % 16 == 0 &&
                  sizeof(f->Wsig) + sizeof(f->u) >= vad_bands_ * sizeof(i16) + SX_FRAME * sizeof(i32), "VAD bands + raw band sums in Wsig and the work area");
    sx_vad(st, c, f->res_pitch, f->Wsig, &SNR_dB_Q7, (i32*)(void*)(f->Wsig + vad_bands_));
    wv_sync();
    static_assert(sizeof(f->u) >= SX_HP_SCRATCH_WORDS * sizeof(i32), "the pitch work area doubles as the high-pass filter's scratch");
    SX_S(32)
    sx_hp_variable_cutoff(st, c, f->x_buf + SX_FRAME + SX_LA_SHAPE, f->res_pitch, (i32*)&f->u);
    wv_sync();
    SX_T(1)
    sx_find_pitch_lags(st, c, f->x_buf, f->res_pitch, f->Wsig, &f->u.pitch);
    wv_sync();
    SX_ENC_TAP(1, st, w, f->x_buf + SX_FRAME + SX_LA_SHAPE);
    SX_T(2)
    sx_noise_shape_analysis(st, c, f->res_pitch + SX_FRAME, f->x_buf + SX_FRAME, &f->u.shape);
    wv_sync();
    SX_ENC_TAP(2, st, w, f->res_pitch + SX_FRAME);
    SX_T(3)
    SX_PAR(i, SX_LTP_BUF) f->u.pref.ring[i] = hist->pf_sLTP_shp[i];
    wv_sync();
    sx_prefilter(st, c, w->xfw, f->x_buf + SX_FRAME, &f->u.pref);
    wv_sync();
    SX_PAR(i, SX_LTP_BUF) hist->pf_sLTP_shp[i] = f->u.pref.ring[i];
    wv_sync();
    SX_ENC_TAP(3, st, w, w->xfw);
    SX_T(4)
    static_assert(offsetof(SxFrontWork, Wsig) == offsetof(SxFrontWork, res_pitch) + sizeof(f->res_pitch) && offsetof(SxFrontWork, res_pitch) % 4 == 0,
                  "res_pitch and Wsig are one scratch area for the NLSF quantiser");
    sx_find_pred_coefs(st, c, f->x_buf, f->res_pitch, &f->u.pred);
    wv_sync();
    SX_ENC_TAP(4, st, w, w->xfw);
    SX_T(5)
    sx_process_gains(st, c);
    wv_sync();
    SX_ENC_TAP(5, st, w, w->xfw);
    SX_T(6)
    SX_PAR(i, SX_FRAME + SX_LA_SHAPE) hist->x_buf[i] = f->x_buf[SX_FRAME + i];
    wv_sync();
    {
        if (SX_LANE == 0) {
            sx_pub_st(&in->sigtype, c->sigtype); sx_pub_st(&in->QuantOffsetType, c->QuantOffsetType); sx_pub_st(&in->NLSFInterpCoef_Q2, c->NLSFInterpCoef_Q2);
            sx_pub_st(&in->Seed, c->Seed); sx_pub_st(&in->Lambda_Q10, c->Lambda_Q10); sx_pub_st(&in->LTP_scale_Q14, c->LTP_scale_Q14); sx_pub_st(&in->DeltaGains_Q16, c->DeltaGains_Q16);
        }
        SX_PAR(i, SX_NB_SUBFR) {
            sx_pub_st(&in->pitchL[i], c->pitchL[i]); sx_pub_st(&in->Gains_Q16[i], c->Gains_Q16[i]); sx_pub_st(&in->LF_shp_Q14[i], c->LF_shp_Q14[i]);
            sx_pub_st(&in->Tilt_Q14[i], c->Tilt_Q14[i]); sx_pub_st(&in->HarmShapeGain_Q14[i], c->HarmShapeGain_Q14[i]);
        }
        SX_PAR(i, 2 * SX_MAX_LPC) sx_pub_st(&(&in->PredCoef_Q12[0][0])[i], (i & (SX_MAX_LPC - 1)) < SX_LPC ? (&c->PredCoef_Q12[0][0])[i] : (i16)0);
        SX_PAR(i, SX_LTP_ORDER * SX_NB_SUBFR) sx_pub_st(&in->LTPCoef_Q14[i], c->LTPCoef_Q14[i]);
        SX_PAR(i, SX_NB_SUBFR * SX_SHAPE_ORDER) sx_pub_st(&in->AR2_Q13[i], c->AR2_Q13[i]);
        SX_PAR(i, SX_FRAME) sx_pub_st(&in->xfw[i], w->xfw[i]);
        wv_sync();
    }
    SX_T(7)
    if (st->speech_activity_Q8 < K_SPEECH_ACTIVITY_DTX_THRES_Q8) {
        st->vadFlag = 0;
        st->noSpeechCounter++;
        if (st->noSpeechCounter > 5) st->inDTX = 1;
        if (st->noSpeechCounter > 20 + 5) { st->noSpeechCounter = 5; st->inDTX = 0; }
    } else {
        st->noSpeechCounter = 0;
        st->inDTX = 0;
        st->vadFlag = 1;
    }
    x->sigtype = c->sigtype; x->QuantOffsetType = c->QuantOffsetType;
    for (int i = 0; i < 4; i++) { x->GainsIndices[i] = c->GainsIndices[i]; x->LTPIndex[i] = c->LTPIndex[i]; }
    x->DeltaGainsIndices = c->DeltaGainsIndices;
    for (int i = 0; i < SX_NLSF_STAGES; i++) x->NLSFIndices[i] = c->NLSFIndices[i];
    x->NLSFInterpCoef_Q2 = c->NLSFInterpCoef_Q2;
    x->lagIndex = c->lagIndex; x->contourIndex = c->contourIndex; x->PERIndex = c->PERIndex;
    x->LTP_scaleIndex = c->LTP_scaleIndex;
    x->Seed = c->Seed;
    x->vadFlag = st->vadFlag;
    x->inDTX = st->inDTX; x->pad_ = 0;
    st->prev_sigtype = c->sigtype;
    st->prevLag = c->pitchL[SX_NB_SUBFR - 1];
    st->first_frame_after_reset = 0;
    st->nFramesInPayloadBuf = frame + 1 < st->fpp ? frame + 1 : 0;
    wv_sync();
    SX_T(8)
}

struct SxCodeIn {
    SxFrameIdx idx[2];
    i16 hi[SX_BAND];
};

SX_FNW void sx_enc_stage_a(SxEncStream* rec, SxEncWork* w, const i16* pcm, SxNsqIn* in2, SxCodeIn* cin) {
    SX_IN_LDS(w);
    SxEncHist* hist = &rec->hist;
    SX_T_BEGIN
    SX_STRETCH_DENSE();
    const int fpp = SX_UNI(w->st.fpp);
    sx_qmf_decomp(hist, pcm, w->u.qmf_tl, hist->lo, cin->hi, fpp * 2 * SX_FRAME);
    wv_sync();
    SX_T(0)
    for (int frame = 0; frame < fpp; frame++) {
        sx_enc_analyse_frame(rec, w, hist->lo + frame * SX_FRAME, frame, &in2[frame], &cin->idx[frame]);
        wv_sync();
    }
}

SX_FNW void sx_enc_stage_c_hb(SxEncStream* rec, SxEncWork* w, const SxCodeIn* cin, const SxNsqOut* out2, int hb_slot = 0) {
    SX_IN_LDS(w);
    SxEncHist* hist = &rec->hist;
    SxEncState* st = &w->st;
    SX_T_BEGIN
    if (st->hb_joint) {
        sx_hb_encode_frame<2 * SX_FRAME>(hist, cin->hi, out2[0].r, out2[1].r, &w->u.hb, &w->hb_bytes[8 * hb_slot]);
        wv_sync();
        SX_T(9)
    } else {
        const int fpp = SX_UNI(st->fpp);
        for (int frame = 0; frame < fpp; frame++) {
            sx_hb_encode_frame<SX_FRAME>(hist, cin->hi + frame * SX_FRAME, out2[frame].r, out2[frame].r, &w->u.hb, &w->hb_bytes[8 * hb_slot + 4 * frame]);
            wv_sync();
            SX_T(9)
        }
    }
}

SX_HD bool sx_enc_packet_in_dtx(int useDTX, const SxCodeIn* cin, int fpp = 2) { return useDTX && SX_UNI(cin->idx[fpp - 1].inDTX); }

SX_FN i32 sx_enc_stage_c_out(SxEncWork* w, const SxCodeIn* cin, const u8* buf0, const u8* buf1, const SxRcInfo* info2, u8* bits, i32 buf_size,
                             i16* nBytesOut) {
    SX_IN_LDS(w);
    SxEncState* st = &w->st;
    SX_T_BEGIN
    const int fpp = SX_UNI(st->fpp);
    const int hb_bytes = st->hb_joint ? 4 : 4 * fpp;
    if (sx_enc_packet_in_dtx(st->useDTX, cin, fpp)) {
        nBytesOut[0] = 0;
        nBytesOut[1] = 0;
        SX_PAR(i, hb_bytes) bits[i] = w->hb_bytes[i];
        wv_sync();
        return hb_bytes;
    }
    const i32 nb0 = SX_UNI(info2[0].nBytes), nb1 = SX_UNI(info2[1].nBytes);
    const i32 err = SX_UNI(info2[0].error | info2[1].error);
    const i32 total = nb0 + nb1 + hb_bytes;
    if (err || total > buf_size || nb0 > SX_MAX_ARITHM_BYTES || nb1 > SX_MAX_ARITHM_BYTES) {
        nBytesOut[0] = 0;
        nBytesOut[1] = 0;
        return -1;
    }
    SX_PAR(i, total) {
        u8 b;
        if (i < nb0) b = buf0[i];
        else if (i < nb0 + nb1) b = buf1[i - nb0];
        else b = w->hb_bytes[i - nb0 - nb1];
        bits[i] = b;
    }
    nBytesOut[0] = (i16)total;
    nBytesOut[1] = (i16)(nb1 + hb_bytes);
    wv_sync();
    SX_T(11)
    return total;
}

#if SX_NLANES == 1
SX_FN i32 sx_enc_stage_c(SxEncStream* rec, SxEncWork* w, const SxCodeIn* cin, const SxNsqOut* out2, u8* bits, i32 buf_size, i16* nBytesOut) {
    sx_enc_stage_c_hb(rec, w, cin, out2);
    SxRcInfo info[2] = {{0, 0}, {0, 0}};
    const int fpp = w->st.fpp;
    if (!sx_enc_packet_in_dtx(w->st.useDTX, cin, fpp)) {
        sx_cdf_load(&w->u.code.cdf);
        for (int md = 0; md < 2; md++)
            sx_code_description(cin->idx, out2[0].Seed, out2[1].Seed, out2[0].q[md], out2[1].q[md], md, w->st.useMDIndex, &w->u.code.cdf, w->u.code.pulses,
                                w->u.code.buf[md], &info[md], fpp);
    }
    return sx_enc_stage_c_out(w, cin, w->u.code.buf[0], w->u.code.buf[1], info, bits, buf_size, nBytesOut);
}
#endif

#if defined(SOLO_HOST_EMU)
SX_FN i32 sx_encode_packet(SxEncStream* rec, SxEncWork* w, SxCodeIn* cin, const i16* pcm, u8* bits, i32 buf_size, i16* nBytesOut) {
    sx_enc_stage_a(rec, w, pcm, rec->nsq_in, cin);
    wv_sync();
    for (int frame = 0; frame < w->st.fpp; frame++) {
        sx_nsq_del_dec((char*)&rec->nsq, 0u, &rec->nsq_in[frame], (char*)&rec->nsq_out[frame], 0u, &w->u.nsq, w->u.nsq.ring_emu, 0u, 12);
        wv_sync();
    }
    return sx_enc_stage_c(rec, w, cin, rec->nsq_out, bits, buf_size, nBytesOut);
}
// ... 2 lines not shown
```

solo_amd/csrc/solo_enc_front.h:

```cpp
#pragma once
#include "solo_enc_state.h"

SX_FN1 void sx_qmf_decomp(SxEncHist* hist, const i16* pcm, i16* tl, i16* lo, i16* hi, int n = SX_PACKET) {
    SX_IN_LDS(tl);
    n = SX_UNI(n);
    SX_PAR(i, 63) tl[i] = hist->qmf_hist[i];
    SX_PAR(i, n) tl[63 + i] = (i16)(pcm[i] >> 1);
    wv_sync();
    SX_PAR(k, n >> 1) {
        i32 y1 = 0, y2 = 0;
        const i16* xa = tl + 2 * k;
        const i16* xb = tl + 63 + 2 * k;
        for (int j = 0; j < 32; j++) {
            i32 a = T_qmf_taps[63 - j];
            i32 p = xa[j], q = xb[-j];
            y1 = sx_add(y1, sx_mul(a, (i32)(i16)(p + q)));
            i32 d = sx_mul(a, (i32)(i16)(p - q));
            y2 = (j & 1) ? sx_add(y2, d) : sx_sub(y2, d);
        }
        lo[k] = (i16)sx_saturate(sx_pshr32(y1, 15), 32767);
        hi[k] = (i16)sx_saturate(sx_pshr32(y2, 15), 32767);
    }
    wv_sync();
    SX_PAR(i, 63) hist->qmf_hist[i] = tl[n + i];
// ... 3 lines not shown
struct alignas(16) SxV4i { i32 v[4]; };
#ifdef SX_LANE_STREAM
static_assert((SX_FRAME / 8) % 4 == 0 && SX_FRAME / 8 >= 4, "all-pass pairs are processed in blocks of four");
SX_HD void sx_allpass2_lanes(const i16* in, int npairs, i32* S, i32 cA, i32 cB, i16* outL, i16* outH) {
    if (SX_LANE < 2) {
        const int l = SX_LANE;
        i32 s = S ? S[l] : 0;
        i32 cpre = sx_pre16(l ? cB : cA);
        SX_VEC(cpre);
        const i32 mask = l ? 0 : -1;
        const i16* ip = in + l;
        i16* op = l ? outH : outL;
        i32 x[4], xn[4];
#pragma unroll
        for (int u = 0; u < 4; u++) xn[u] = ip[2 * u];
        for (int k = 0; k < npairs; k += 4) {
#pragma unroll
            for (int u = 0; u < 4; u++) x[u] = xn[u];
            if (k + 4 < npairs) {
#pragma unroll
                for (int u = 0; u < 4; u++) xn[u] = ip[2 * (k + 4 + u)];
            }
#pragma unroll
            for (int u = 0; u < 4; u++) {
                const i32 in32 = sx_shl(x[u], 10);
                const i32 Y = sx_sub(in32, s);
                const i32 X = sx_add(sx_smulw_pre(Y, cpre), Y & mask);
                const i32 o = sx_add(s, X);
                s = sx_add(in32, X);
                const i32 p = SX_DPP_(l ? o : sx_neg(o), 0xB1);
                const i32 v = sx_add(o, p);
                op[k + u] = (i16)sx_sat16(sx_rshift_round_small(v, 11));
            }
        }
        if (S) S[l] = s;
    }
    wv_sync();
}
#endif

#ifdef SX_LANE_STREAM
SX_HD void sx_allpass2_lanes_raw(const i16* in, int npairs, i32* S, i32 cA, i32 cB, i32* rawL, i32* rawH, i32* dump4) {
    if (SX_LANE < 2) {
        const int l = SX_LANE;
        i32 s = S ? S[l] : 0;
        i32 cpre = sx_pre16(l ? cB : cA);
        SX_VEC(cpre);
        const i32 mask = l ? 0 : -1;
        const i16* ip = in + l;
        SxV4i* op = (SxV4i*)(l ? (rawH ? rawH : dump4) : rawL);
        const int ostep = (l && !rawH) ? 0 : 1;
        i32 x[4], xn[4];
#pragma unroll
        for (int u = 0; u < 4; u++) xn[u] = ip[2 * u];
        for (int k = 0; k < npairs; k += 4) {
#pragma unroll
            for (int u = 0; u < 4; u++) x[u] = xn[u];
            if (k + 4 < npairs) {
#pragma unroll
                for (int u = 0; u < 4; u++) xn[u] = ip[2 * (k + 4 + u)];
            }
            SxV4i r;
#pragma unroll
            for (int u = 0; u < 4; u++) {
                const i32 in32 = sx_shl(x[u], 10);
                const i32 Y = sx_sub(in32, s);
                const i32 X = sx_add(sx_smulw_pre(Y, cpre), Y & mask);
                const i32 o = sx_add(s, X);
                s = sx_add(in32, X);
                const i32 p = SX_DPP_(l ? o : sx_neg(o), 0xB1);
                r.v[u] = sx_add(o, p);
            }
            *op = r;
            op += ostep;
        }
        if (S) S[l] = s;
    }
    wv_sync();
}
SX_HD void sx_allpass2_finish(i16* out, const i32* raw, int n) {
    SX_PAR(i, n) out[i] = (i16)sx_sat16(sx_rshift_round_small(raw[i], 11));
}
#endif

SX_HD void sx_ana_filt_bank_1(const i16* in, i32* S, i16* outL, i16* outH, int N, i32* raw) {
    const i32 A20 = (i16)(5394 << 1), A21 = (i16)(20623 << 1);
#if defined(SX_LANE_STREAM) && !defined(SX_NO_RAW_VAD)
    sx_allpass2_lanes_raw(in, N >> 1, S, A21, A20, raw, raw + (N >> 1), (i32*)0);
    sx_allpass2_finish(outL, raw, N >> 1);
    sx_allpass2_finish(outH, raw + (N >> 1), N >> 1);
    wv_sync();
#elif defined(SX_LANE_STREAM)
    sx_allpass2_lanes(in, N >> 1, S, A21, A20, outL, outH);
#elif 0
    i32 r[SX_FCH], oL[(SX_FCH + 1) / 2], oH[(SX_FCH + 1) / 2];
#pragma unroll
    for (int j = 0; j < (SX_FCH + 1) / 2; j++) { oL[j] = 0; oH[j] = 0; }
#pragma unroll
    for (int j = 0; j < SX_FCH; j++) { const int i = SX_LANE + 64 * j; r[j] = i < N ? (i32)in[i] : 0; }
    i32 s0 = SX_UNI(S[0]), s1 = SX_UNI(S[1]);
#pragma unroll
    for (int c = 0; c < SX_FCH; c++) {
        const int kend = sx_min(N >> 1, 32 * (c + 1));
        for (int k = 32 * c; k < kend; k++) {
            i32 in32 = sx_shl(SX_RDLANE(r[c], (2 * k) & 63), 10);
            i32 Y = sx_sub(in32, s0);
            i32 X = sx_smlawb(Y, Y, A21);
            i32 out_1 = sx_add(s0, X);
            s0 = sx_add(in32, X);
            in32 = sx_shl(SX_RDLANE(r[c], (2 * k + 1) & 63), 10);
            Y = sx_sub(in32, s1);
            X = sx_smulwb(Y, A20);
            i32 out_2 = sx_add(s1, X);
            s1 = sx_add(in32, X);
            SX_WRLANE(oL[c >> 1], k & 63, sx_sat16(sx_rshift_round(sx_add(out_2, out_1), 11)));
            SX_WRLANE(oH[c >> 1], k & 63, sx_sat16(sx_rshift_round(sx_sub(out_2, out_1), 11)));
        }
    }
#pragma unroll
    for (int j = 0; j < (SX_FCH + 1) / 2; j++) {
        const int i = SX_LANE + 64 * j;
        if (i < (N >> 1)) { outL[i] = (i16)oL[j]; outH[i] = (i16)oH[j]; }
    }
    S[0] = s0;
    S[1] = s1;
    wv_sync();
#else
    i32 s0 = S[0], s1 = S[1];
    for (int k = 0; k < (N >> 1); k++) {
        i32 in32 = sx_shl((i32)in[2 * k], 10);
        i32 Y = sx_sub(in32, s0);
        i32 X = sx_smlawb(Y, Y, A21);
        i32 out_1 = sx_add(s0, X);
        s0 = sx_add(in32, X);
        in32 = sx_shl((i32)in[2 * k + 1], 10);
        Y = sx_sub(in32, s1);
        X = sx_smulwb(Y, A20);
        i32 out_2 = sx_add(s1, X);
        s1 = sx_add(in32, X);
        outL[k] = (i16)sx_sat16(sx_rshift_round(sx_add(out_2, out_1), 11));
        outH[k] = (i16)sx_sat16(sx_rshift_round(sx_sub(out_2, out_1), 11));
    }
    S[0] = s0;
    S[1] = s1;
#endif
}

SX_FN1 void sx_vad(SxEncState* st, SxEncCtrl* c, const i16* pIn, i16* X, i32* pSNR_dB_Q7, i32* raw) {
    SX_IN_LDS(st); SX_IN_LDS(c); SX_IN_LDS(X); SX_IN_LDS(raw);
    SxVAD* v = &st->vad;
    i16* X0 = X, *X1 = X + 80, *X2 = X + 160, *X3 = X + 240;
    sx_ana_filt_bank_1(pIn, v->AnaState, X0, X3, SX_FRAME, raw);
    sx_ana_filt_bank_1(X0, v->AnaState1, X0, X2, SX_FRAME >> 1, raw);
    sx_ana_filt_bank_1(X0, v->AnaState2, X0, X1, SX_FRAME >> 2, raw);
    const int dfl = SX_FRAME >> 3;
    static_assert((SX_FRAME >> 3) % 2 == 0 && (SX_FRAME >> 3) + 2 * 16 <= 80, "the tail of X0 (its band is SX_FRAME / 8 long by now) is the scratch of the band statistics");
    i32* part = (i32*)(X + dfl);
#if SX_NLANES == 1
    {
        X0[dfl - 1] = (i16)(X0[dfl - 1] >> 1);
        const i16 HPstateTmp = X0[dfl - 1];
        for (int i = dfl - 1; i > 0; i--) {
            X0[i - 1] = (i16)(X0[i - 1] >> 1);
            X0[i] = (i16)(X0[i] - X0[i - 1]);
        }
        X0[0] = (i16)(X0[0] - (i16)v->HPstate);
        v->HPstate = HPstateTmp;
    }
#else
    {
        static_assert((SX_FRAME >> 3) <= 64, "one sample of the lowest band per lane");
        const int i = SX_LANE < dfl ? SX_LANE : 0;
        const i16 h = (i16)(X0[i] >> 1), hm = (i16)(i > 0 ? X0[i - 1] >> 1 : (i16)v->HPstate);
        wv_sync();
        if (SX_LANE < dfl) X0[i] = (i16)(h - hm);
        if (SX_LANE == dfl - 1) v->HPstate = h;
        wv_sync();
    }
#endif
    SX_PAR(t, 16) {
        const int b = t >> 2, q = t & 3;
        const int sub_len = (SX_FRAME >> sx_min(4 - b, 3)) >> 2;
        const i16* Xb = X + 80 * b + q * sub_len;
        i32 sum = 0;
        for (int i = 0; i < sub_len; i++) {
            const i32 x_tmp = Xb[i] >> 3;
            sum = sx_smlabb(sum, x_tmp, x_tmp);
        }
        part[t] = sum;
    }
    wv_sync();
    const i32 min_coef = v->counter < 1000 ? 32767 / ((v->counter >> 4) + 1) : 0;
    SX_PAR(b, 4) {
        i32 e = v->XnrgSubfr[b];
        for (int q = 0; q < 3; q++) e = sx_add_pos_sat32(e, part[4 * b + q]);
        const i32 last = part[4 * b + 3];
        e = sx_add_pos_sat32(e, last >> 1);
        v->XnrgSubfr[b] = last;
        i32 nl = v->NL[b];
        {
            const i32 nrg = sx_add_pos_sat32(e, v->NoiseLevelBias[b]);
            const i32 inv_nrg = SX_I32_MAX / nrg;
            i32 coef;
            if (nrg > sx_shl(nl, 3)) coef = 1024 >> 3;
            else if (nrg < nl) coef = 1024;
            else coef = sx_smulwb(sx_smulww(inv_nrg, nl), 1024 << 1);
            coef = sx_max(coef, min_coef);
            v->inv_NL[b] = sx_smlawb(v->inv_NL[b], inv_nrg - v->inv_NL[b], coef);
            nl = SX_I32_MAX / v->inv_NL[b];
            nl = sx_min(nl, 0x00FFFFFF);
            v->NL[b] = nl;
        }
        i32 ratio = 256, sq = 0, tilt = 0;
        const i32 speech_nrg_b = e - nl;
        if (speech_nrg_b > 0) {
            if ((e & 0xFF800000) == 0) ratio = sx_shl(e, 8) / (nl + 1);
            else ratio = e / ((nl >> 8) + 1);
            i32 SNR_Q7 = sx_lin2log(ratio) - 8 * 128;
            sq = sx_smulbb(SNR_Q7, SNR_Q7);
            if (speech_nrg_b < (1 << 20)) SNR_Q7 = sx_smulwb(sx_shl(sx_sqrt_approx(speech_nrg_b), 6), SNR_Q7);
            tilt = sx_smulwb(T_vad_tilt_weights[b], SNR_Q7);
        }
        part[4 * b] = ratio; part[4 * b + 1] = sq; part[4 * b + 2] = tilt; part[4 * b + 3] = (b + 1) * (speech_nrg_b >> 4);
    }
    v->counter++;
    wv_sync();
    i32 sumSquared = 0, input_tilt = 0, speech_nrg = 0;
    for (int b = 0; b < 4; b++) {
        sumSquared = sx_add(sumSquared, part[4 * b + 1]);
        input_tilt = sx_add(input_tilt, part[4 * b + 2]);
        speech_nrg = sx_add(speech_nrg, part[4 * b + 3]);
    }
    sumSquared = sumSquared / 4;
    *pSNR_dB_Q7 = (i16)(3 * sx_sqrt_approx(sumSquared));
    i32 SA_Q15 = sx_sigm_Q15(sx_smulwb(45000, *pSNR_dB_Q7) - 128);
    c->input_tilt_Q15 = sx_shl(sx_sigm_Q15(input_tilt) - 16384, 1);
    if (speech_nrg <= 0) {
        SA_Q15 = SA_Q15 >> 1;
    } else if (speech_nrg < 32768) {
        speech_nrg = sx_sqrt_approx(sx_shl(speech_nrg, 15));
        SA_Q15 = sx_smulwb(32768 + speech_nrg, SA_Q15);
    }
    st->speech_activity_Q8 = sx_min(SA_Q15 >> 7, 255);
    i32 smooth_coef_Q16 = (i16)sx_smulwb(4096, sx_smulwb(SA_Q15, SA_Q15));
    SX_PAR(b, 4) {
        v->NrgRatioSmth_Q8[b] = sx_smlawb(v->NrgRatioSmth_Q8[b], part[4 * b] - v->NrgRatioSmth_Q8[b], smooth_coef_Q16);
        i32 SNR_Q7 = 3 * (sx_lin2log(v->NrgRatioSmth_Q8[b]) - 8 * 128);
        c->input_quality_bands_Q15[b] = sx_sigm_Q15((SNR_Q7 - 16 * 128) >> 4);
    }
    wv_sync();
}

#define SX_HP_SCRATCH_WORDS (4 * (SX_FRAME + 1))
SX_FN1 void sx_hp_variable_cutoff(SxEncState* st, SxEncCtrl* c, i16* out, const i16* in, i32* scratch) {
    SX_IN_LDS(st); SX_IN_LDS(c); SX_IN_LDS(out); SX_IN_LDS(scratch);
    if (st->prev_sigtype == 0) {
        i32 pitch_freq_Hz_Q16 = sx_shl(SX_FS_KHZ * 1000, 16) / st->prevLag;
        i32 pitch_freq_log_Q7 = sx_lin2log(pitch_freq_Hz_Q16) - (16 << 7);
        i32 quality_Q15 = c->input_quality_bands_Q15[0];
        pitch_freq_log_Q7 = sx_sub(pitch_freq_log_Q7, sx_smulwb(sx_smulwb(sx_shl(quality_Q15, 2), quality_Q15), pitch_freq_log_Q7 - 809));
        pitch_freq_log_Q7 = sx_add(pitch_freq_log_Q7, (K_0p6_Q15 - quality_Q15) >> 9);
        i32 delta_freq_Q7 = pitch_freq_log_Q7 - (st->variable_HP_smth1_Q15 >> 8);
        if (delta_freq_Q7 < 0) delta_freq_Q7 = sx_mul(delta_freq_Q7, 3);
        delta_freq_Q7 = sx_limit(delta_freq_Q7, -K_VARIABLE_HP_MAX_DELTA_FREQ_Q7, K_VARIABLE_HP_MAX_DELTA_FREQ_Q7);
        st->variable_HP_smth1_Q15 = sx_smlawb(st->variable_HP_smth1_Q15,
                                              sx_mul(sx_shl(st->speech_activity_Q8, 1), delta_freq_Q7), K_VARIABLE_HP_SMTH_COEF1_Q16);
    }
    st->variable_HP_smth2_Q15 = sx_smlawb(st->variable_HP_smth2_Q15, st->variable_HP_smth1_Q15 - st->variable_HP_smth2_Q15,
                                          K_VARIABLE_HP_SMTH_COEF2_Q16);
    c->pitch_freq_low_Hz = sx_log2lin(st->variable_HP_smth2_Q15 >> 8);
    c->pitch_freq_low_Hz = sx_limit(c->pitch_freq_low_Hz, K_VARIABLE_HP_MIN_FREQ_Q0, K_VARIABLE_HP_MAX_FREQ_Q0);
    i32 Fc_Q19 = sx_smulbb(1482, c->pitch_freq_low_Hz) / SX_FS_KHZ;
    i32 r_Q28 = K_1p0_Q28 - sx_mul(K_0p92_Q9, Fc_Q19);
    i32 B0 = r_Q28, B1 = sx_shl(sx_neg(r_Q28), 1), B2 = r_Q28;
    i32 r_Q22 = r_Q28 >> 6;
    i32 A0 = sx_smulww(r_Q22, sx_smulww(Fc_Q19, Fc_Q19) - K_2p0_Q22);
    i32 A1 = sx_smulww(r_Q22, r_Q22);
    i32 A0_L = sx_neg(A0) & 0x3FFF, A0_U = sx_neg(A0) >> 14;
    i32 A1_L = sx_neg(A1) & 0x3FFF, A1_U = sx_neg(A1) >> 14;
    A0_L = SX_UNI(A0_L); A0_U = SX_UNI(A0_U); A1_L = SX_UNI(A1_L); A1_U = SX_UNI(A1_U);
    B0 = SX_UNI(B0); B1 = SX_UNI(B1); B2 = SX_UNI(B2);
    i32 S0 = SX_UNI(st->In_HP_State[0]), S1 = SX_UNI(st->In_HP_State[1]);
#ifdef SX_LANE_STREAM
    {
        SxV4i* bx = (SxV4i*)scratch;
        const i32 b0p = B0, b1p = B1, b2p = B2;
        SX_PAR(k, SX_FRAME) {
            const i32 xs = sx_pre16(in[k]);
            SxV4i v;
            v.v[0] = sx_smulw_pre(b0p, xs); v.v[1] = sx_smulw_pre(b1p, xs); v.v[2] = sx_smulw_pre(b2p, xs); v.v[3] = 0;
            bx[k] = v;
        }
        wv_sync();
        {
            const int q = SX_LANE & 3;
            i32 s0 = S0, s1 = S1;
            i32 coef = sx_pre16(q == 0 ? A0_L : (q == 1 ? A0_U : (q == 2 ? A1_L : A1_U)));
            i32 radd = (q & 1) ? 0 : (1 << 13), rsh = (q & 1) ? 0 : 14;
            SX_VEC(s0); SX_VEC(s1); SX_VEC(coef); SX_VEC(radd); SX_VEC(rsh);
            SxV4i cur = bx[0];
#pragma unroll 4
            for (int k = 0; k < SX_FRAME; k++) {
                const SxV4i t = cur;
                cur = bx[k + 1];
                const i32 out32_Q14 = sx_shl(sx_add(s0, t.v[0]), 2);
                i32 p = sx_smulw_pre(out32_Q14, coef);
                SX_VEC(p);
                const i32 r = sx_add(p, radd) >> rsh;
                const i32 w = sx_add(r, SX_DPP_(r, 0xB1));
                const i32 n0 = sx_add(sx_add(s1, t.v[1]), SX_DPP_(w, 0x00));
                const i32 n1 = sx_add(t.v[2], SX_DPP_(w, 0xAA));
                s0 = n0; s1 = n1;
                bx[k].v[3] = out32_Q14;
            }
            if (SX_LANE == 0) {
                st->In_HP_State[0] = s0;
                st->In_HP_State[1] = s1;
            }
        }
        wv_sync();
        SX_PAR(k, SX_FRAME) out[k] = (i16)sx_sat16(sx_add(bx[k].v[3], (1 << 14) - 1) >> 14);
        wv_sync();
        return;
    }
#elif 0
    i32 r[SX_FCH], o[SX_FCH];
#pragma unroll
    for (int j = 0; j < SX_FCH; j++) { const int i = SX_LANE + 64 * j; r[j] = i < SX_FRAME ? (i32)in[i] : 0; o[j] = 0; }
#pragma unroll
    for (int c = 0; c < SX_FCH; c++) {
        const int kend = sx_min(SX_FRAME, 64 * (c + 1));
        for (int k = 64 * c; k < kend; k++) {
// ... 690 lines not shown
```

solo_amd/csrc/solo_enc_kernels.h:

```cpp
#pragma once
#include <hip/hip_runtime.h>
#include "solo_enc.h"
#include "solo_stream_ctl.h"

#ifndef SX_TU_FRONT
__global__ void __launch_bounds__(64) SX_K(solo_enc_init_kernel)(SxEncStream* states, int n_streams, int silk_rate_bps, int useMDIndex, int hb_joint, int useDTX, int fpp) {
    const int s = blockIdx.x;
    if (s >= n_streams) return;
    sx_enc_state_init(&states[s], silk_rate_bps, useMDIndex, hb_joint, useDTX, fpp);
}
__global__ void __launch_bounds__(64) SX_K(solo_enc_init_list_kernel)(SxEncStream* states, const SxStreamCtlList list, int n, int hb_joint, int fpp) {
    if ((int)blockIdx.x >= n) return;
    const SxStreamCtl r = list.r[blockIdx.x];
    sx_enc_state_init(&states[r.stream], r.a, r.b, hb_joint, r.c, fpp);
}
__global__ void __launch_bounds__(64) SX_K(solo_enc_ctl_list_kernel)(SxEncStream* states, const SxStreamCtlList list, int n) {
    if ((int)blockIdx.x >= n || SX_LANE != 0) return;
    const SxStreamCtl r = list.r[blockIdx.x];
    SxEncState* st = &states[r.stream].core;
    sx_enc_setup_rate(st, r.a);
    st->useMDIndex = r.b;
    st->useDTX = r.c;
}

#endif
#ifdef SX_OUTLINE_WRAPPERS
#define SX_ENTER_FN static __device__ __attribute__((noinline))
#else
#define SX_ENTER_FN __device__ __forceinline__
#endif
SX_ENTER_FN void SX_K(solo_enc_enter)(SxEncWork* w, const SxEncStream* rec) {
    const i32* src = (const i32*)&rec->core;
    i32* dst = (i32*)&w->st;
    SX_PAR(i, (int)(sizeof(SxEncState) / 4)) dst[i] = src[i];
    wv_sync();
}
SX_ENTER_FN void SX_K(solo_enc_leave)(SxEncWork* w, SxEncStream* rec) {
    wv_sync();
    const i32* src = (const i32*)&w->st;
    i32* dst = (i32*)&rec->core;
    SX_PAR(i, (int)(sizeof(SxEncState) / 4)) dst[i] = src[i];
}

#ifndef SX_ANALYSIS_WAVES
#define SX_ANALYSIS_WAVES 5
#endif
#ifndef SX_ANALYSIS_PRIO
#define SX_ANALYSIS_PRIO 3
#endif
#ifndef SX_TU_FRONT
__global__ void __launch_bounds__(64, SX_ANALYSIS_WAVES) SX_K(solo_enc_analysis_kernel)(SxEncStream* states, const i16* __restrict__ pcm, int n_streams,
                                                                  int n_packets, int p0, int pc, SxNsqIn* __restrict__ nsq_in,
                                                                  SxCodeIn* __restrict__ code_in, const i32* __restrict__ map, const u32* verdict) {
    __shared__ SxEncWork w;
    const int s = blockIdx.x;
    if (s >= n_streams || sx_map_refused(map, verdict)) return;
    __builtin_amdgcn_s_setprio(SX_ANALYSIS_PRIO);
    SxEncStream* rec = &states[sx_map_stream(map, s)];
#if defined(SX_PROF) && defined(__HIP_DEVICE_COMPILE__)
    const unsigned long long hist_t0_ = wall_clock64();
#endif
#if defined(SX_STOPS) && defined(__HIP_DEVICE_COMPILE__)
    SX_STOPS_ENTER(0)
#endif
    SX_K(solo_enc_enter)(&w, rec);
    for (int p = p0; p < p0 + pc; p++) {
        const size_t pk = (size_t)s * n_packets + p;
        sx_enc_stage_a(rec, &w, pcm + pk * (size_t)(SX_FRAME * 2 * SX_UNI(w.st.fpp)), nsq_in + pk * 2, code_in + pk);
        wv_sync();
    }
    SX_K(solo_enc_leave)(&w, rec);
#if defined(SX_PROF) && defined(__HIP_DEVICE_COMPILE__)
    if (threadIdx.x == 0) {
        unsigned hw; asm volatile("s_getreg_b32 %0, hwreg(HW_REG_HW_ID)" : "=s"(hw));
        const unsigned long long dt = wall_clock64() - hist_t0_;
        const unsigned bin = (unsigned)(dt / 5000u);
        atomicAdd(&g_sx_hist[(hw >> 4) & 3][bin < 63 ? bin : 63], 1ull);
    }
#endif
}

#endif
#ifndef SX_RC_LANES
#define SX_RC_LANES 64
#endif
struct SxRcWork {
    SxCdf cdf;
    u32 pw[SX_RC_LANES][SX_RC_PW_ROW / 4];
};
__device__ __forceinline__ void SX_K(sx_cdf_stage)(SxCdf* c) {
    const int lane = (int)(threadIdx.x & 63u);
    for (int i = lane; i < (int)(sizeof(SxCdf) / 4); i += 64) ((u32*)c)[i] = 0;
    wv_sync();
#define X(type, name, n) for (int i = lane; i < (n); i += 64) c->name[i] = T_##name[i];
    SX_CDF_LIST(X) SX_CDF_LIST_ENC(X)
#undef X
    wv_sync();
}

__device__ __forceinline__ i32 SX_K(sx_rc_code_and_assemble)(const SxFrameIdx* idx2, const SxNsqOut* out2, int md, int useDTX, int useMDIndex, int fpp, int hb_bytes,
                                                             const SxCdf* cdf, u8* pw, u8* mine, const u8* hb, int slot_bytes, u8* out, i16* nb_out, SxRcInfo* info_out) {
    SxRcInfo info = {0, 0};
    const bool dtx = useDTX && idx2[fpp - 1].inDTX;
    if (!dtx) sx_code_description(idx2, sx_pub_ld(&out2[0].Seed), sx_pub_ld(&out2[1].Seed), out2[0].q[md], out2[1].q[md], md, useMDIndex, cdf, pw, mine, &info, fpp);
    if (info_out) *info_out = info;
    const i32 nbo = __shfl_xor(info.nBytes, 1), ero = __shfl_xor(info.error, 1);
    const i32 nb0 = md ? nbo : info.nBytes, nb1 = md ? info.nBytes : nbo;
    const i32 total = nb0 + nb1 + hb_bytes;
    if (dtx) {
        if (md) for (int i = 0; i < hb_bytes; i++) out[i] = hb[i];
        else { nb_out[0] = 0; nb_out[1] = 0; }
        return hb_bytes;
    }
    if ((info.error | ero) || total > slot_bytes || nb0 > SX_MAX_ARITHM_BYTES || nb1 > SX_MAX_ARITHM_BYTES) {
        if (!md) { nb_out[0] = 0; nb_out[1] = 0; }
        return -1;
    }
    u8* dst = out + (md ? nb0 : 0);
    for (int i = 0; i < info.nBytes; i++) dst[i] = mine[i];
    if (md) for (int i = 0; i < hb_bytes; i++) out[nb0 + nb1 + i] = hb[i];
    else { nb_out[0] = (i16)total; nb_out[1] = (i16)(nb1 + hb_bytes); }
    return total;
}

#ifndef SX_TU_FRONT
__global__ void __launch_bounds__(64) SX_K(solo_enc_rc_kernel)(const SxEncStream* states, const SxCodeIn* __restrict__ code_in,
                                                               const SxNsqOut* __restrict__ nsq_out, int n_streams, int n_packets, int p0, int pc,
                                                               u8* __restrict__ rcbuf, SxRcInfo* __restrict__ rcinfo, const u8* __restrict__ hbout,
                                                               int slot_bytes, u8* __restrict__ bits, i16* __restrict__ nbytes, i32* status,
                                                               const i32* __restrict__ map, const u32* verdict) {
    __shared__ SxRcWork w;
    if (sx_map_refused(map, verdict)) return;
    SX_K(sx_cdf_stage)(&w.cdf);
    const int lane = threadIdx.x, md = lane & 1;
    const int s = blockIdx.x * (SX_RC_LANES / 2) + (lane >> 1);
    if (lane >= SX_RC_LANES || s >= n_streams) return;
    const SxEncState* st = &states[map ? map[s] : s].core;
    const int useDTX = st->useDTX, useMDIndex = st->useMDIndex, fpp = st->fpp;
    const int hb_bytes = st->hb_joint ? 4 : 4 * fpp;
    i32 first_err = 0;
    for (int p = p0; p < p0 + pc; p++) {
        const size_t pk = (size_t)s * n_packets + p;
        const size_t slot = ((size_t)s * pc + (size_t)(p - p0)) * 2 + (size_t)md;
        const i32 ret = SX_K(sx_rc_code_and_assemble)(code_in[pk].idx, nsq_out + pk * 2, md, useDTX, useMDIndex, fpp, hb_bytes, &w.cdf, (u8*)&w.pw[lane][0],
                                                      rcbuf + slot * SX_RC_BUF_STRIDE, hbout + (slot & ~(size_t)1) * 4, slot_bytes, bits + pk * (size_t)slot_bytes,
                                                      nbytes + pk * 2, &rcinfo[slot]);
        if (ret < 0 && first_err == 0) first_err = ret;
    }
    if (status && md == 0) {
        if (p0 == 0) status[s] = first_err;
        else if (first_err != 0 && status[s] == 0) status[s] = first_err;
// ... 91 lines not shown
        i32 ret = 0;
        if (j < cnt) {
            const size_t pk = pk0 + (size_t)(rc_done + j);
            ret = SX_K(sx_rc_code_and_assemble)(code_in[pk].idx, nsq_out + pk * 2, md, useDTX, useMDIndex, fpp, hb_bytes, &rw->cdf, (u8*)&rw->pw[lane][0],
                                                rcbuf + ((size_t)s * (2 * SX_FRONT_RB) + (size_t)lane) * SX_RC_BUF_STRIDE, &w.hb_bytes[8 * j], slot_bytes,
                                                bits + pk * (size_t)slot_bytes, nbytes + pk * 2, (SxRcInfo*)nullptr);
        }
        if (first_err == 0 && __builtin_amdgcn_ballot_w64(ret < 0) != 0ull) first_err = -1;
        rc_done = hb_done;
        wv_sync();
    };
    auto code_one = [&]() __attribute__((always_inline)) {
        const size_t pk = pk0 + (size_t)hb_done;
#ifndef SX_FRONT_NO_HB
        sx_enc_stage_c_hb(rec, &w, code_in + pk, nsq_out + pk * 2, hb_done - rc_done);
#endif
        wv_sync();
        hb_done++;
        if (hb_done - rc_done >= SX_FRONT_RB) rc_batch();
    };
    if (!(mode & 1)) {
        for (int p = 0; p < n_packets; p++) {
            const size_t pk = pk0 + (size_t)p;
            sx_enc_stage_a(rec, &w, pcm + pk * (size_t)(SX_FRAME * 2 * fpp), nsq_in + pk * 2, code_in + pk);
            wv_sync();
            sx_pub_drain();
            if (lane == 0) sx_flag_st(&ana_flag[s], ticket0 + (unsigned int)p + 1u);
            for (int it = 0; it < 2 && hb_done <= p && !(mode & 2); it++) {
                const unsigned int f = (unsigned int)SX_UNI(sx_flag_ld(my_nsq_flag));
                if ((int)(f - (ticket0 + (unsigned int)hb_done + 1u)) < 0) break;
                code_one();
            }
        }
        SX_K(solo_enc_leave)(&w, rec);
        wv_sync();
        SX_FRONT_TRACE(s, 1, wall_clock64())
        SX_FRONT_TRACE(s, 3, (unsigned long long)hb_done)
    }
    {
        const unsigned long long t0 = wall_clock64();
        while (hb_done < n_packets && !(mode & 2)) {
            const unsigned int f = (unsigned int)SX_UNI(sx_flag_ld(my_nsq_flag));
            if ((int)(f - (ticket0 + (unsigned int)hb_done + 1u)) >= 0) { code_one(); continue; }
            if (mode & 1) { first_err = first_err ? first_err : SX_FRONT_ERR_HANDOVER; break; }
            if (wall_clock64() - t0 >= (unsigned long long)final_wait_ticks) break;
#pragma unroll
            for (int z = 0; z < SX_FRONT_POLL_SLEEPS; z++) __builtin_amdgcn_s_sleep(127);
        }
    }
    rc_batch();
    if (!(mode & 1)) SX_FRONT_TRACE(s, 2, wall_clock64())
    if (lane == 0) {
        prog[s] = (unsigned int)hb_done;
        if (status) {
            if (!(mode & 1)) status[s] = first_err;
            else if (first_err != 0 && status[s] == 0) status[s] = first_err;
        }
    }
}

#endif
extern "C" int SX_K(solo_launch_nsq)(void* states, const void* in, void* out, int n_streams, int n_packets, int p0, int pc, unsigned int* started,
                                     void* ring, const int32_t* map, const uint32_t* verdict, void* hip_stream);
extern "C" int SX_K(solo_launch_nsq_persist)(void* states, const void* in, void* out, int n_streams, int n_packets, unsigned int* started, void* ring,
                                             const unsigned int* ana_flag, unsigned int* nsq_flag, unsigned int ticket0, unsigned int* err, void* stage,
                                             void* hip_stream);
extern "C" size_t SX_K(solo_nsq_stage_bytes)(int n_streams);
extern "C" int SX_K(solo_nsq_persist_workgroups)(int n_streams);
extern "C" int SX_K(solo_nsq_workgroups)(int n_streams);
extern "C" size_t SX_K(solo_nsq_ring_bytes)(int n_streams);

#include "solo_enc_ops.h"
#ifndef SX_TU_FRONT
static hipError_t SX_K(solo_enc_launch_init)(void* states, int n_streams, int silk_rate_bps, int useMDIndex, int hb_joint, int useDTX, int fpp, hipStream_t s) {
    hipLaunchKernelGGL(SX_K(solo_enc_init_kernel), dim3(n_streams), dim3(64), 0, s, (SxEncStream*)states, n_streams, silk_rate_bps, useMDIndex, hb_joint, useDTX, fpp);
    return hipGetLastError();
}
static hipError_t SX_K(solo_enc_launch_init_list)(void* states, const SxStreamCtl* recs, int n, int hb_joint, int fpp, hipStream_t s) {
    return sx_launch_ctl_batches(recs, n, [&](const SxStreamCtlList& l, int k) { hipLaunchKernelGGL(SX_K(solo_enc_init_list_kernel), dim3(k), dim3(64), 0, s, (SxEncStream*)states, l, k, hb_joint, fpp); });
}
static hipError_t SX_K(solo_enc_launch_ctl_list)(void* states, const SxStreamCtl* recs, int n, hipStream_t s) {
    return sx_launch_ctl_batches(recs, n, [&](const SxStreamCtlList& l, int k) { hipLaunchKernelGGL(SX_K(solo_enc_ctl_list_kernel), dim3(k), dim3(64), 0, s, (SxEncStream*)states, l, k); });
}
static hipError_t SX_K(solo_enc_launch_analysis)(void* states, const int16_t* pcm, int n_streams, int n_packets, int p0, int pc, void* nsq_in,
                                                 void* code_in, const int32_t* map, const uint32_t* verdict, hipStream_t s) {
    hipLaunchKernelGGL(SX_K(solo_enc_analysis_kernel), dim3(n_streams), dim3(64), 0, s, (SxEncStream*)states, pcm, n_streams, n_packets, p0, pc,
                       (SxNsqIn*)nsq_in, (SxCodeIn*)code_in, map, verdict);
    return hipGetLastError();
}
static size_t SX_K(solo_enc_rc_scratch_bytes)(int n_streams, int pc) {
    return (size_t)n_streams * (size_t)pc * 2 * (SX_RC_BUF_STRIDE + sizeof(SxRcInfo) + 4) + 128;
}
static SxRcInfo* SX_K(solo_enc_rcinfo_of)(u8* rcbuf, int n_streams, int pc) {
    return (SxRcInfo*)(rcbuf + (((size_t)n_streams * (size_t)pc * 2 * SX_RC_BUF_STRIDE + 63) & ~(size_t)63));
}
static u8* SX_K(solo_enc_hbout_of)(u8* rcbuf, int n_streams, int pc) {
    return (u8*)(SX_K(solo_enc_rcinfo_of)(rcbuf, n_streams, pc) + (size_t)n_streams * (size_t)pc * 2);
}
static hipError_t SX_K(solo_enc_launch_coding)(void* states, const void* code_in, const void* nsq_out, int n_streams, int n_packets, int p0, int pc,
                                               int slot, uint8_t* bits, int16_t* nbytes, int32_t* status, void* rc_scratch, const int32_t* map,
                                               const uint32_t* verdict, hipStream_t s) {
    u8* rcbuf = (u8*)rc_scratch;
    hipLaunchKernelGGL(SX_K(solo_enc_coding_kernel), dim3(n_streams), dim3(64), 0, s, (SxEncStream*)states, (const SxCodeIn*)code_in,
                       (const SxNsqOut*)nsq_out, n_streams, n_packets, p0, pc, SX_K(solo_enc_hbout_of)(rcbuf, n_streams, pc), map, verdict);
    hipError_t e = hipGetLastError();
    if (e != hipSuccess) return e;
    hipLaunchKernelGGL(SX_K(solo_enc_rc_kernel), dim3((n_streams + SX_RC_LANES / 2 - 1) / (SX_RC_LANES / 2)), dim3(64), 0, s, (const SxEncStream*)states, (const SxCodeIn*)code_in,
                       (const SxNsqOut*)nsq_out, n_streams, n_packets, p0, pc, rcbuf, SX_K(solo_enc_rcinfo_of)(rcbuf, n_streams, pc),
                       (const u8*)SX_K(solo_enc_hbout_of)(rcbuf, n_streams, pc), slot, bits, nbytes, status, map, verdict);
    return hipGetLastError();
}
#endif
#ifdef SX_TU_FRONT
extern "C" size_t SX_K(solo_enc_front_scratch_bytes)(int n_streams) { return (size_t)n_streams * (2 * SX_FRONT_RB) * SX_RC_BUF_STRIDE + 128; }
extern "C" hipError_t SX_K(solo_enc_launch_front)(void* states, const int16_t* pcm, int n_streams, int n_packets, void* nsq_in, void* code_in, const void* nsq_out,
                                              unsigned int* ana_flag, const unsigned int* nsq_flag, unsigned int* prog, unsigned int ticket0, int mode,
                                              unsigned int final_wait_ticks, int slot, uint8_t* bits, int16_t* nbytes, int32_t* status, void* scratch,
                                              unsigned int* started, hipStream_t s) {
    static bool lds_set = false;
    if (!lds_set) {
        const hipError_t e = hipFuncSetAttribute((const void*)SX_K(solo_enc_front_kernel), hipFuncAttributeMaxDynamicSharedMemorySize, (int)(SX_FRONT_WAVES * SX_FRONT_WORK_BYTES));
        if (e != hipSuccess) return e;
        lds_set = true;
    }
    hipLaunchKernelGGL(SX_K(solo_enc_front_kernel), dim3((n_streams + SX_FRONT_WAVES - 1) / SX_FRONT_WAVES), dim3(64 * SX_FRONT_WAVES), SX_FRONT_WAVES * SX_FRONT_WORK_BYTES, s, (SxEncStream*)states, pcm, n_streams, n_packets, (SxNsqIn*)nsq_in,
                       (SxCodeIn*)code_in, (const SxNsqOut*)nsq_out, ana_flag, nsq_flag, prog, ticket0, mode, final_wait_ticks, slot, bits, nbytes, status,
                       (u8*)scratch, started);
    return hipGetLastError();
}
#else
extern "C" size_t SX_K(solo_enc_front_scratch_bytes)(int n_streams);
extern "C" hipError_t SX_K(solo_enc_launch_front)(void* states, const int16_t* pcm, int n_streams, int n_packets, void* nsq_in, void* code_in, const void* nsq_out,
                                                  unsigned int* ana_flag, const unsigned int* nsq_flag, unsigned int* prog, unsigned int ticket0, int mode,
                                                  unsigned int final_wait_ticks, int slot, uint8_t* bits, int16_t* nbytes, int32_t* status, void* scratch,
                                                  unsigned int* started, hipStream_t s);
static const solo_enc_ops SX_K(solo_enc_ops_table) = {
    sizeof(SxEncStream), sizeof(SxNsqIn), sizeof(SxNsqOut), sizeof(SxCodeIn), SX_PACKET,
    SX_K(solo_enc_launch_init), SX_K(solo_enc_launch_init_list), SX_K(solo_enc_launch_ctl_list), SX_K(solo_enc_launch_analysis), SX_K(solo_launch_nsq), SX_K(solo_enc_launch_coding), SX_K(solo_enc_rc_scratch_bytes),
    SX_K(solo_nsq_workgroups), SX_K(solo_nsq_ring_bytes), SX_K(solo_enc_launch_front), SX_K(solo_launch_nsq_persist), SX_K(solo_enc_front_scratch_bytes), SX_K(solo_nsq_persist_workgroups), SX_K(solo_nsq_stage_bytes),
    SX_FRONT_WAVES, SX_FRONT_PER_CU};

#endif
```

solo_amd/csrc/solo_enc_ops.h:

```cpp
#pragma once
#include <hip/hip_runtime.h>
#include <stdint.h>
#include <stddef.h>
#include "solo_stream_ctl.h"
#ifndef SOLO_ENC_OPS_DEFINED
#define SOLO_ENC_OPS_DEFINED
struct solo_enc_ops {
    size_t state_bytes, nsq_in_bytes, nsq_out_bytes, code_in_bytes;
    int packet_samples;
    hipError_t (*init)(void* states, int n_streams, int silk_rate_bps, int useMDIndex, int hb_joint, int useDTX, int frames_per_packet, hipStream_t s);
    hipError_t (*init_list)(void* states, const SxStreamCtl* recs, int n, int hb_joint, int frames_per_packet, hipStream_t s);
    hipError_t (*ctl_list)(void* states, const SxStreamCtl* recs, int n, hipStream_t s);
    hipError_t (*analysis)(void* states, const int16_t* pcm, int n_streams, int n_packets, int p0, int pc, void* nsq_in, void* code_in, const int32_t* map,
                           const uint32_t* verdict, hipStream_t s);
    int (*nsq)(void* states, const void* in, void* out, int n_streams, int n_packets, int p0, int pc, unsigned int* started, void* ring, const int32_t* map,
               const uint32_t* verdict, void* hip_stream);
    hipError_t (*coding)(void* states, const void* code_in, const void* nsq_out, int n_streams, int n_packets, int p0, int pc, int slot,
                         uint8_t* bits, int16_t* nbytes, int32_t* status, void* rc_scratch, const int32_t* map, const uint32_t* verdict, hipStream_t s);
    size_t (*rc_scratch_bytes)(int n_streams, int pc);
    int (*nsq_workgroups)(int n_streams);
    size_t (*nsq_ring_bytes)(int n_streams);
    hipError_t (*front)(void* states, const int16_t* pcm, int n_streams, int n_packets, void* nsq_in, void* code_in, const void* nsq_out,
                        unsigned int* ana_flag, const unsigned int* nsq_flag, unsigned int* prog, unsigned int ticket0, int mode,
                        unsigned int final_wait_ticks, int slot, uint8_t* bits, int16_t* nbytes, int32_t* status, void* scratch,
                        unsigned int* started, hipStream_t s);
    int (*nsq_persist)(void* states, const void* in, void* out, int n_streams, int n_packets, unsigned int* started, void* ring,
                       const unsigned int* ana_flag, unsigned int* nsq_flag, unsigned int ticket0, unsigned int* err, void* stage, void* hip_stream);
    size_t (*front_scratch_bytes)(int n_streams);
    int (*nsq_persist_workgroups)(int n_streams);
    size_t (*nsq_stage_bytes)(int n_streams);
    int front_waves;
    int front_per_cu;
};
#endif
```

Baseline: 3.930 million 40ms packets/s (encode+decode).

## Split QMF decomposition and VAD into a prepass kernel on a separate stream

Adds a prepass kernel that performs QMF band splitting and the VAD detector, with one lane per stream running the VAD, and writes low-band samples and per-frame VAD results to new scratch buffers. The work runs on a new low-priority stream sQ one chunk ahead of analysis, with events gating it. The aim is to take the serial per-stream VAD and QMF work out of the analysis kernel and overlap it with other stages. In exchange it adds extra global memory traffic for the intermediate buffers, more events and a cross-stream dependency. The ops table and analysis signature change.

```diff
diff --git a/include/solo_mi355x.h b/include/solo_mi355x.h
--- a/include/solo_mi355x.h
+++ b/include/solo_mi355x.h
@@ -150,6 +150,9 @@
 int32_t solo_debug_analysis(int32_t samplerate, int32_t silk_rate_bps, int32_t useMDIndex, int32_t joint, int32_t dtx, int32_t frames_per_packet,
                             int32_t n_streams, int32_t n_packets, int32_t chunk, const int16_t *h_pcm, void *h_nsq_in, void *h_code_in,
                             int32_t *h_sizes);
+int32_t solo_debug_pre(int32_t samplerate, int32_t silk_rate_bps, int32_t useMDIndex, int32_t joint, int32_t dtx, int32_t frames_per_packet,
+                       int32_t n_streams, int32_t n_packets, int32_t chunk, const int16_t *h_pcm, int16_t *h_lo, void *h_pre, int16_t *h_hi,
+                       int32_t *h_sizes);
 int32_t solo_debug_coding(int32_t samplerate, int32_t silk_rate_bps, int32_t useMDIndex, int32_t joint, int32_t dtx, int32_t frames_per_packet,
                           int32_t n_streams, int32_t n_packets, int32_t chunk, int32_t slot_bytes, const void *h_code_in, const void *h_nsq_out,
                           uint8_t *h_bits, int16_t *h_nbytes, int32_t *h_status);
diff --git a/solo_amd/__init__.py b/solo_amd/__init__.py
--- a/solo_amd/__init__.py
+++ b/solo_amd/__init__.py
@@ -14,7 +14,7 @@
     "solo_batch_n_streams", "solo_batch_slot_bytes", "solo_kernel_name", "solo_version", "solo_batch_set_timing",
     "solo_batch_last_kernel_ms", "solo_batch_last_encode_chunks", "solo_batch_decode_split", "solo_batch_set_async_join",
     "solo_batch_wait_encode", "solo_debug_l0", "solo_debug_sum_sqr_shift", "solo_debug_rowops", "solo_debug_clock", "solo_debug_nsq",
-    "solo_debug_waveops", "solo_debug_nsq_ex", "solo_debug_analysis", "solo_debug_coding", "solo_debug_dec_extract", "solo_debug_dec_synth",
+    "solo_debug_waveops", "solo_debug_nsq_ex", "solo_debug_analysis", "solo_debug_pre", "solo_debug_coding", "solo_debug_dec_extract", "solo_debug_dec_synth",
     "solo_recv_create", "solo_recv_insert", "solo_recv_decode", "solo_recv_stats",
     "solo_batch_reset_streams", "solo_recv_reset_streams", "solo_batch_update_streams",
     "solo_batch_encode_streams", "solo_batch_decode_streams", "solo_recv_decode_streams",
@@ -184,6 +184,8 @@
     lib.solo_debug_nsq_ex.argtypes = [C.c_int32] * 8 + [C.c_void_p, C.c_void_p]
     lib.solo_debug_analysis.restype = C.c_int32
     lib.solo_debug_analysis.argtypes = [C.c_int32] * 9 + [C.c_void_p, C.c_void_p, C.c_void_p, C.c_void_p]
+    lib.solo_debug_pre.restype = C.c_int32
+    lib.solo_debug_pre.argtypes = [C.c_int32] * 9 + [C.c_void_p] * 5
     lib.solo_debug_coding.restype = C.c_int32
     lib.solo_debug_coding.argtypes = [C.c_int32] * 10 + [C.c_void_p, C.c_void_p, C.c_void_p, C.c_void_p, C.c_void_p]
     lib.solo_debug_dec_extract.restype = C.c_int32
diff --git a/solo_amd/csrc/solo_api.hip b/solo_amd/csrc/solo_api.hip
--- a/solo_amd/csrc/solo_api.hip
+++ b/solo_amd/csrc/solo_api.hip
@@ -173,6 +173,8 @@
     int pipe_ready, chunk_packets;
     hipStream_t sA, sB, sC;
     hipEvent_t evFork, evJoinA[2], evJoinC[2], evA[SOLO_MAX_CHUNKS], evB[SOLO_MAX_CHUNKS], evC[SOLO_MAX_CHUNKS];
+    hipStream_t sQ;
+    hipEvent_t evQ[SOLO_MAX_CHUNKS], evJoinQ;
     int async_join;
     unsigned int enc_seq;
     int evC_valid;
@@ -477,8 +479,10 @@
     if (b->ev_ready) for (int i = 0; i < 2; i++) (void)hipEventDestroy(b->evDec[i]);
     if (b->tev_ready) for (int k = 0; k < 3; k++) for (int c = 0; c < SOLO_MAX_CHUNKS; c++) for (int e = 0; e < 2; e++) (void)hipEventDestroy(b->tev[k][c][e]);
     if (b->pipe_ready) {
-        (void)hipStreamSynchronize(b->sA); (void)hipStreamSynchronize(b->sB); (void)hipStreamSynchronize(b->sC);
-        (void)hipStreamDestroy(b->sA); (void)hipStreamDestroy(b->sB); (void)hipStreamDestroy(b->sC);
+        (void)hipStreamSynchronize(b->sA); (void)hipStreamSynchronize(b->sB); (void)hipStreamSynchronize(b->sC); (void)hipStreamSynchronize(b->sQ);
+        (void)hipStreamDestroy(b->sA); (void)hipStreamDestroy(b->sB); (void)hipStreamDestroy(b->sC); (void)hipStreamDestroy(b->sQ);
+        for (int c = 0; c < SOLO_MAX_CHUNKS; c++) (void)hipEventDestroy(b->evQ[c]);
+        (void)hipEventDestroy(b->evJoinQ);
         dev_free(b->d_started);
         (void)hipEventDestroy(b->evFork);
         for (int i = 0; i < 2; i++) { (void)hipEventDestroy(b->evJoinA[i]); (void)hipEventDestroy(b->evJoinC[i]); }
@@ -922,7 +926,9 @@
     SOLO_CHECK(hipStreamCreateWithPriority(&b->sA, hipStreamNonBlocking, lo));
     SOLO_CHECK(hipStreamCreateWithPriority(&b->sB, hipStreamNonBlocking, hi));
     SOLO_CHECK(hipStreamCreateWithPriority(&b->sC, hipStreamNonBlocking, lo));
+    SOLO_CHECK(hipStreamCreateWithPriority(&b->sQ, hipStreamNonBlocking, lo));
     SOLO_CHECK(hipEventCreateWithFlags(&b->evFork, hipEventDisableTiming));
+    SOLO_CHECK(hipEventCreateWithFlags(&b->evJoinQ, hipEventDisableTiming));
     for (int i = 0; i < 2; i++) {
         SOLO_CHECK(hipEventCreateWithFlags(&b->evJoinA[i], hipEventDisableTiming));
         SOLO_CHECK(hipEventCreateWithFlags(&b->evJoinC[i], hipEventDisableTiming));
@@ -931,6 +937,7 @@
         SOLO_CHECK(hipEventCreateWithFlags(&b->evA[c], hipEventDisableTiming));
         SOLO_CHECK(hipEventCreateWithFlags(&b->evB[c], hipEventDisableTiming));
         SOLO_CHECK(hipEventCreateWithFlags(&b->evC[c], hipEventDisableTiming));
+        SOLO_CHECK(hipEventCreateWithFlags(&b->evQ[c], hipEventDisableTiming));
     }
     int dev = 0, ncu = 0;
     SOLO_CHECK(hipGetDevice(&dev));
@@ -1048,16 +1055,19 @@
     const unsigned long long per_wave = 64ull / (unsigned long long)ops->nsq_workgroups(64);
     if (((per_wave - 1ull) * 2ull * (unsigned long long)n_packets + 1ull) * (unsigned long long)ops->nsq_out_bytes >= (1ull << 32)) return -1;
     const size_t sz_in = np * 2 * ops->nsq_in_bytes, sz_out = np * 2 * ops->nsq_out_bytes, sz_code = np * ops->code_in_bytes;
+    const size_t sz_lo = np * ops->lo_bytes, sz_pre = np * 2 * ops->pre_out_bytes;
     if (n_packets > b->enc_work_packets) {
         SOLO_CHECK(hipStreamSynchronize(st));
-        if (b->pipe_ready) { (void)hipStreamSynchronize(b->sA); (void)hipStreamSynchronize(b->sB); (void)hipStreamSynchronize(b->sC); }
+        if (b->pipe_ready) { (void)hipStreamSynchronize(b->sA); (void)hipStreamSynchronize(b->sB); (void)hipStreamSynchronize(b->sC); (void)hipStreamSynchronize(b->sQ); }
         dev_free(b->d_enc_work);
-        SOLO_CHECK(hipMalloc(&b->d_enc_work, sz_in + sz_out + sz_code + 256));
+        SOLO_CHECK(hipMalloc(&b->d_enc_work, sz_in + sz_out + sz_code + sz_lo + sz_pre + 512));
         b->enc_work_packets = n_packets;
     }
     void* nin = b->d_enc_work;
     void* nout = (char*)b->d_enc_work + ((sz_in + 63) & ~(size_t)63);
     void* cin = (char*)nout + ((sz_out + 63) & ~(size_t)63);
+    void* lob = (char*)cin + ((sz_code + 63) & ~(size_t)63);
+    void* preb = (char*)lob + ((sz_lo + 63) & ~(size_t)63);
     void* states = b->d_enc_state;
     if (!b->pipe_ready) {
         const int32_t r = solo_enc_pipe_setup(b);
@@ -1095,6 +1105,7 @@
     if (b->enc_seq > 0 && (b->last_np != n_packets || b->last_cp != cp || b->evC_valid == 0)) {
         SOLO_CHECK(hipStreamWaitEvent(b->sA, b->evJoinC[(b->enc_seq - 1u) & 1u], 0));
         SOLO_CHECK(hipStreamWaitEvent(b->sB, b->evJoinA[(b->enc_seq - 1u) & 1u], 0));
+        SOLO_CHECK(hipStreamWaitEvent(b->sQ, b->evJoinC[(b->enc_seq - 1u) & 1u], 0));
         b->evC_valid = 0;
     }
     b->last_np = n_packets;
@@ -1103,6 +1114,7 @@
     SOLO_CHECK(hipStreamWaitEvent(b->sA, b->evFork, 0));
     SOLO_CHECK(hipStreamWaitEvent(b->sB, b->evFork, 0));
     SOLO_CHECK(hipStreamWaitEvent(b->sC, b->evFork, 0));
+    SOLO_CHECK(hipStreamWaitEvent(b->sQ, b->evFork, 0));
     const int nall = map ? n : b->n_streams;
     const int G = b->group_streams > 0 ? b->group_streams : nall;
     const int ngroups = (nall + G - 1) / G;
@@ -1110,9 +1122,25 @@
     const size_t frame_samples = (size_t)enc_packet_samples(b);
     int idx = 0;
     hipError_t lerr = hipSuccess;
+    const bool have_pre = ops->pre != NULL;
+    auto enqueue_pre = [&](int k) -> hipError_t {
+        const int g = k / nchunks, cc = k % nchunks, c = k % SOLO_MAX_CHUNKS;
+        const int s0 = g * G, ns = (s0 + G <= nall) ? G : nall - s0;
+        const size_t pk0 = (size_t)s0 * (size_t)n_packets;
+        const int p0 = cc * cp, pc = (p0 + cp <= n_packets) ? cp : n_packets - p0;
+        hipError_t e;
+        if (ngroups == 1 && cc < b->evC_valid && (e = hipStreamWaitEvent(b->sQ, b->evC[c], 0)) != hipSuccess) return e;
+        e = ops->pre(map ? states : (char*)states + (size_t)s0 * ops->state_bytes, d_pcm + pk0 * frame_samples, ns, n_packets, p0, pc, (char*)lob + pk0 * ops->lo_bytes,
+                     (char*)preb + pk0 * 2 * ops->pre_out_bytes, (char*)cin + pk0 * ops->code_in_bytes, map ? map + s0 : NULL, verdict, b->sQ);
+        if (e != hipSuccess) return e;
+        return hipEventRecord(b->evQ[c], b->sQ);
+    };
+    if (have_pre) lerr = enqueue_pre(0);
     for (int g = 0; g < ngroups && lerr == hipSuccess; g++) {
         const int s0 = g * G, ns = (s0 + G <= nall) ? G : nall - s0;
         const size_t pk0 = (size_t)s0 * (size_t)n_packets;
+        void* g_lo = (char*)lob + pk0 * ops->lo_bytes;
+        void* g_pre = (char*)preb + pk0 * 2 * ops->pre_out_bytes;
         void* g_states = map ? states : (char*)states + (size_t)s0 * ops->state_bytes;
         const int32_t* g_map = map ? map + s0 : NULL;
         const int16_t* g_pcm = d_pcm + pk0 * frame_samples;
@@ -1126,9 +1154,13 @@
             const int c = idx % SOLO_MAX_CHUNKS, cprev = (idx + SOLO_MAX_CHUNKS - 1) % SOLO_MAX_CHUNKS;
             const int p0 = cc * cp, pc = (p0 + cp <= n_packets) ? cp : n_packets - p0;
             if (ngroups == 1 && cc < b->evC_valid) SOLO_CHECK(hipStreamWaitEvent(b->sA, b->evC[c], 0));
+            if (have_pre) {
+                if (idx + 1 < ngroups * nchunks && (lerr = enqueue_pre(idx + 1)) != hipSuccess) break;
+                SOLO_CHECK(hipStreamWaitEvent(b->sA, b->evQ[c], 0));
+            }
             if (idx > 0 && b->gate > 0) (void)solo_launch_gate(&b->d_started[cprev], b->started_target[cprev], b->sA);
             if (tm) (void)hipEventRecord(b->tev[0][c][0], b->sA);
-            if ((lerr = ops->analysis(g_states, g_pcm, ns, n_packets, p0, pc, g_nin, g_cin, g_map, verdict, b->sA)) != hipSuccess) break;
+            if ((lerr = ops->analysis(g_states, g_pcm, ns, n_packets, p0, pc, g_nin, g_cin, g_lo, g_pre, 0, g_map, verdict, b->sA)) != hipSuccess) break;
             if (tm) (void)hipEventRecord(b->tev[0][c][1], b->sA);
             SOLO_CHECK(hipEventRecord(b->evA[c], b->sA));
             SOLO_CHECK(hipStreamWaitEvent(b->sB, b->evA[c], 0));
@@ -1156,6 +1188,8 @@
     b->evC_valid = (ok && ngroups == 1 && !map) ? nchunks : 0;
     const int js = (int)(b->enc_seq & 1u);
     b->enc_seq++;
+    (void)hipEventRecord(b->evJoinQ, b->sQ);
+    (void)hipStreamWaitEvent(b->sA, b->evJoinQ, 0);
     (void)hipEventRecord(b->evJoinA[js], b->sA);
     (void)hipEventRecord(b->evJoinC[js], b->sC);
     if (!b->async_join || !ok) {
@@ -1460,19 +1494,50 @@
     if (!debug_enc_args(ops, frames_per_packet, n_streams, n_packets) || chunk < 0 || !h_pcm || !h_nsq_in || !h_code_in) return -1;
     const size_t np = (size_t)n_streams * n_packets;
     const size_t sz_pcm = np * (size_t)(ops->packet_samples / 2 * frames_per_packet) * 2, sz_in = np * 2 * ops->nsq_in_bytes, sz_code = np * ops->code_in_bytes;
-    void *st = NULL, *d_pcm = NULL, *d_in = NULL, *d_code = NULL;
+    void *st = NULL, *d_pcm = NULL, *d_in = NULL, *d_code = NULL, *d_pre = NULL;
     int32_t rc = -1;
     const int cp = chunk > 0 ? chunk : n_packets;
+    const size_t sz_lo = (np * ops->lo_bytes + 63) & ~(size_t)63, sz_pre = np * 2 * ops->pre_out_bytes;
     bool ok = hipMalloc(&st, ops->state_bytes * (size_t)n_streams) == hipSuccess && hipMalloc(&d_pcm, sz_pcm) == hipSuccess && hipMalloc(&d_in, sz_in) == hipSuccess &&
+              hipMalloc(&d_pre, sz_lo + sz_pre + 64) == hipSuccess && hipMemset(d_pre, 0, sz_lo + sz_pre + 64) == hipSuccess &&
               hipMalloc(&d_code, sz_code) == hipSuccess && hipMemset(d_in, 0, sz_in) == hipSuccess && hipMemset(d_code, 0, sz_code) == hipSuccess &&
               ops->init(st, n_streams, silk_rate_bps, useMDIndex, joint, dtx, frames_per_packet, (hipStream_t)0) == hipSuccess &&
               hipMemcpy(d_pcm, h_pcm, sz_pcm, hipMemcpyHostToDevice) == hipSuccess;
     for (int p0 = 0; ok && p0 < n_packets; p0 += cp)
-        ok = ops->analysis(st, (const int16_t*)d_pcm, n_streams, n_packets, p0, p0 + cp <= n_packets ? cp : n_packets - p0, d_in, d_code, NULL, NULL, (hipStream_t)0) == hipSuccess;
+        ok = ops->analysis(st, (const int16_t*)d_pcm, n_streams, n_packets, p0, p0 + cp <= n_packets ? cp : n_packets - p0, d_in, d_code, d_pre, (char*)d_pre + sz_lo, 1, NULL,
+                           NULL, (hipStream_t)0) == hipSuccess;
     if (ok && hipDeviceSynchronize() == hipSuccess && hipMemcpy(h_nsq_in, d_in, sz_in, hipMemcpyDeviceToHost) == hipSuccess &&
         hipMemcpy(h_code_in, d_code, sz_code, hipMemcpyDeviceToHost) == hipSuccess)
         rc = (int32_t)ops->nsq_in_bytes;
-    (void)hipFree(st); (void)hipFree(d_pcm); (void)hipFree(d_in); (void)hipFree(d_code);
+    (void)hipFree(st); (void)hipFree(d_pcm); (void)hipFree(d_in); (void)hipFree(d_code); (void)hipFree(d_pre);
+    return rc;
+}
+int32_t solo_debug_pre(int32_t samplerate, int32_t silk_rate_bps, int32_t useMDIndex, int32_t joint, int32_t dtx, int32_t frames_per_packet,
+                       int32_t n_streams, int32_t n_packets, int32_t chunk, const int16_t* h_pcm, int16_t* h_lo, void* h_pre, int16_t* h_hi, int32_t* h_sizes) {
+    const solo_enc_ops* ops = debug_enc_ops(samplerate);
+    if (!ops || !ops->pre) return -1;
+    const size_t hi_off = ops->code_in_bytes - ops->lo_bytes;
+    if (h_sizes) { h_sizes[0] = (int32_t)ops->lo_bytes; h_sizes[1] = (int32_t)ops->pre_out_bytes; h_sizes[2] = (int32_t)hi_off; h_sizes[3] = (int32_t)ops->code_in_bytes; }
+    if (n_streams == 0) return (int32_t)ops->pre_out_bytes;
+    if (!debug_enc_args(ops, frames_per_packet, n_streams, n_packets) || chunk < 0 || !h_pcm || !h_lo || !h_pre || !h_hi) return -1;
+    const size_t np = (size_t)n_streams * n_packets;
+    const size_t sz_pcm = np * (size_t)(ops->packet_samples / 2 * frames_per_packet) * 2, sz_code = np * ops->code_in_bytes, sz_lo = np * ops->lo_bytes,
+                 sz_pre = np * 2 * ops->pre_out_bytes;
+    void *st = NULL, *d_pcm = NULL, *d_code = NULL, *d_lo = NULL, *d_pre = NULL;
+    int32_t rc = -1;
+    const int cp = chunk > 0 ? chunk : n_packets;
+    bool ok = hipMalloc(&st, ops->state_bytes * (size_t)n_streams) == hipSuccess && hipMalloc(&d_pcm, sz_pcm) == hipSuccess && hipMalloc(&d_code, sz_code) == hipSuccess &&
+              hipMalloc(&d_lo, sz_lo) == hipSuccess && hipMalloc(&d_pre, sz_pre) == hipSuccess && hipMemset(d_code, 0, sz_code) == hipSuccess &&
+              hipMemset(d_lo, 0, sz_lo) == hipSuccess && hipMemset(d_pre, 0, sz_pre) == hipSuccess &&
+              ops->init(st, n_streams, silk_rate_bps, useMDIndex, joint, dtx, frames_per_packet, (hipStream_t)0) == hipSuccess &&
+              hipMemcpy(d_pcm, h_pcm, sz_pcm, hipMemcpyHostToDevice) == hipSuccess;
+    for (int p0 = 0; ok && p0 < n_packets; p0 += cp)
+        ok = ops->pre(st, (const int16_t*)d_pcm, n_streams, n_packets, p0, p0 + cp <= n_packets ? cp : n_packets - p0, d_lo, d_pre, d_code, NULL, NULL, (hipStream_t)0) == hipSuccess;
+    if (ok && hipDeviceSynchronize() == hipSuccess && hipMemcpy(h_lo, d_lo, sz_lo, hipMemcpyDeviceToHost) == hipSuccess &&
+        hipMemcpy(h_pre, d_pre, sz_pre, hipMemcpyDeviceToHost) == hipSuccess &&
+        hipMemcpy2D(h_hi, ops->lo_bytes, (const char*)d_code + hi_off, ops->code_in_bytes, ops->lo_bytes, np, hipMemcpyDeviceToHost) == hipSuccess)
+        rc = (int32_t)ops->pre_out_bytes;
+    (void)hipFree(st); (void)hipFree(d_pcm); (void)hipFree(d_code); (void)hipFree(d_lo); (void)hipFree(d_pre);
     return rc;
 }
 int32_t solo_debug_coding(int32_t samplerate, int32_t silk_rate_bps, int32_t useMDIndex, int32_t joint, int32_t dtx, int32_t frames_per_packet,
diff --git a/solo_amd/csrc/solo_enc.h b/solo_amd/csrc/solo_enc.h
--- a/solo_amd/csrc/solo_enc.h
+++ b/solo_amd/csrc/solo_enc.h
@@ -1,6 +1,7 @@
 #pragma once
 #include <stddef.h>
 #include "solo_enc_analysis.h"
+#include "solo_enc_pre.h"
 #if defined(SOLO_HOST_EMU)
 #include "solo_enc_nsq_row.h"
 #endif
@@ -405,7 +406,7 @@
 #define SX_ENC_TAP(stage, st, w, sig)
 #endif
 
-SX_FNW void sx_enc_analyse_frame(SxEncStream* rec, SxEncWork* w, const i16* pIn, int frame, SxNsqIn* in, SxFrameIdx* x) {
+SX_FNW void sx_enc_analyse_frame(SxEncStream* rec, SxEncWork* w, const i16* pIn, int frame, SxNsqIn* in, SxFrameIdx* x, const SxPreOut* pre = nullptr) {
     SX_IN_LDS(w);
     SxEncHist* hist = &rec->hist;
     SxEncState* st = &w->st;
@@ -418,11 +419,22 @@
     SX_PAR(i, SX_FRAME) f->res_pitch[i] = pIn[i];
     wv_sync();
     SX_STRETCH_LATENCY();
+#ifdef SX_ENC_PREPASS
+    if (SX_LANE == 0) {
+        st->speech_activity_Q8 = pre->speech_activity_Q8;
+        c->input_tilt_Q15 = pre->input_tilt_Q15;
+    }
+    SX_PAR(b, 4) c->input_quality_bands_Q15[b] = pre->input_quality_bands_Q15[b];
+    SNR_dB_Q7 = SX_UNI(pre->SNR_dB_Q7);
+    wv_sync();
+#else
     constexpr int vad_bands_ = 240 + SX_FRAME / 2;
     static_assert(offsetof(SxFrontWork, u) == offsetof(SxFrontWork, Wsig) + sizeof(f->Wsig) && (offsetof(SxFrontWork, Wsig) + vad_bands_ * sizeof(i16)) % 16 == 0 &&
                   sizeof(f->Wsig) + sizeof(f->u) >= vad_bands_ * sizeof(i16) + SX_FRAME * sizeof(i32), "VAD bands + raw band sums in Wsig and the work area");
     sx_vad(st, c, f->res_pitch, f->Wsig, &SNR_dB_Q7, (i32*)(void*)(f->Wsig + vad_bands_));
     wv_sync();
+#endif
+    (void)SNR_dB_Q7; (void)pre;
     static_assert(sizeof(f->u) >= SX_HP_SCRATCH_WORDS * sizeof(i32), "the pitch work area doubles as the high-pass filter's scratch");
     SX_S(32)
     sx_hp_variable_cutoff(st, c, f->x_buf + SX_FRAME + SX_LA_SHAPE, f->res_pitch, (i32*)&f->u);
@@ -505,6 +517,19 @@
     i16 hi[SX_BAND];
 };
 
+#ifdef SX_ENC_PREPASS
+SX_FNW void sx_enc_stage_a(SxEncStream* rec, SxEncWork* w, const i16* lo, const SxPreOut* pre2, SxNsqIn* in2, SxCodeIn* cin) {
+    SX_IN_LDS(w);
+    SX_T_BEGIN
+    SX_STRETCH_DENSE();
+    const int fpp = SX_UNI(w->st.fpp);
+    SX_T(0)
+    for (int frame = 0; frame < fpp; frame++) {
+        sx_enc_analyse_frame(rec, w, lo + frame * SX_FRAME, frame, &in2[frame], &cin->idx[frame], &pre2[frame]);
+        wv_sync();
+    }
+}
+#else
 SX_FNW void sx_enc_stage_a(SxEncStream* rec, SxEncWork* w, const i16* pcm, SxNsqIn* in2, SxCodeIn* cin) {
     SX_IN_LDS(w);
     SxEncHist* hist = &rec->hist;
@@ -519,6 +544,7 @@
         wv_sync();
     }
 }
+#endif
 
 SX_FNW void sx_enc_stage_c_hb(SxEncStream* rec, SxEncWork* w, const SxCodeIn* cin, const SxNsqOut* out2, int hb_slot = 0) {
     SX_IN_LDS(w);
diff --git a/solo_amd/csrc/solo_enc_front.h b/solo_amd/csrc/solo_enc_front.h
--- a/solo_amd/csrc/solo_enc_front.h
+++ b/solo_amd/csrc/solo_enc_front.h
@@ -109,6 +109,69 @@
     SX_PAR(i, n) out[i] = (i16)sx_sat16(sx_rshift_round_small(raw[i], 11));
 }
 #endif
+
+SX_HD void sx_ana_filt_pair(i32 x_even, i32 x_odd, i32& s0, i32& s1, i32& lo, i32& hi) {
+    const i32 A20 = (i16)(5394 << 1), A21 = (i16)(20623 << 1);
+    i32 in32 = sx_shl(x_even, 10);
+    i32 Y = sx_sub(in32, s0);
+    i32 X = sx_smlawb(Y, Y, A21);
+    const i32 out_1 = sx_add(s0, X);
+    s0 = sx_add(in32, X);
+    in32 = sx_shl(x_odd, 10);
+    Y = sx_sub(in32, s1);
+    X = sx_smulwb(Y, A20);
+    const i32 out_2 = sx_add(s1, X);
+    s1 = sx_add(in32, X);
+    lo = sx_sat16(sx_rshift_round(sx_add(out_2, out_1), 11));
+    hi = sx_sat16(sx_rshift_round(sx_sub(out_2, out_1), 11));
+}
+
+SX_HD void sx_vad_band_terms(int b, i32 e, i32 min_coef, i32 bias, i32& NL, i32& inv_NL, i32* t4) {
+    i32 nl = NL;
+    {
+        const i32 nrg = sx_add_pos_sat32(e, bias);
+        const i32 inv_nrg = SX_I32_MAX / nrg;
+        i32 coef;
+        if (nrg > sx_shl(nl, 3)) coef = 1024 >> 3;
+        else if (nrg < nl) coef = 1024;
+        else coef = sx_smulwb(sx_smulww(inv_nrg, nl), 1024 << 1);
+        coef = sx_max(coef, min_coef);
+        inv_NL = sx_smlawb(inv_NL, inv_nrg - inv_NL, coef);
+        nl = SX_I32_MAX / inv_NL;
+        nl = sx_min(nl, 0x00FFFFFF);
+        NL = nl;
+    }
+    i32 ratio = 256, sq = 0, tilt = 0;
+    const i32 speech_nrg_b = e - nl;
+    if (speech_nrg_b > 0) {
+        if ((e & 0xFF800000) == 0) ratio = sx_shl(e, 8) / (nl + 1);
+        else ratio = e / ((nl >> 8) + 1);
+        i32 SNR_Q7 = sx_lin2log(ratio) - 8 * 128;
+        sq = sx_smulbb(SNR_Q7, SNR_Q7);
+        if (speech_nrg_b < (1 << 20)) SNR_Q7 = sx_smulwb(sx_shl(sx_sqrt_approx(speech_nrg_b), 6), SNR_Q7);
+        tilt = sx_smulwb(T_vad_tilt_weights[b], SNR_Q7);
+    }
+    t4[0] = ratio; t4[1] = sq; t4[2] = tilt; t4[3] = (b + 1) * (speech_nrg_b >> 4);
+}
+SX_HD i32 sx_vad_frame_terms(i32 sumSquared, i32 input_tilt, i32 speech_nrg, i32* pSNR_dB_Q7, i32* input_tilt_Q15, i32* speech_activity_Q8) {
+    sumSquared = sumSquared / 4;
+    *pSNR_dB_Q7 = (i16)(3 * sx_sqrt_approx(sumSquared));
+    i32 SA_Q15 = sx_sigm_Q15(sx_smulwb(45000, *pSNR_dB_Q7) - 128);
+    *input_tilt_Q15 = sx_shl(sx_sigm_Q15(input_tilt) - 16384, 1);
+    if (speech_nrg <= 0) {
+        SA_Q15 = SA_Q15 >> 1;
+    } else if (speech_nrg < 32768) {
+        speech_nrg = sx_sqrt_approx(sx_shl(speech_nrg, 15));
+        SA_Q15 = sx_smulwb(32768 + speech_nrg, SA_Q15);
+    }
+    *speech_activity_Q8 = sx_min(SA_Q15 >> 7, 255);
+    return (i16)sx_smulwb(4096, sx_smulwb(SA_Q15, SA_Q15));
+}
+SX_HD i32 sx_vad_band_quality(i32& NrgRatioSmth_Q8, i32 ratio, i32 smooth_coef_Q16) {
+    NrgRatioSmth_Q8 = sx_smlawb(NrgRatioSmth_Q8, ratio - NrgRatioSmth_Q8, smooth_coef_Q16);
+    const i32 SNR_Q7 = 3 * (sx_lin2log(NrgRatioSmth_Q8) - 8 * 128);
+    return sx_sigm_Q15((SNR_Q7 - 16 * 128) >> 4);
+}
 
 SX_HD void sx_ana_filt_bank_1(const i16* in, i32* S, i16* outL, i16* outH, int N, i32* raw) {
     const i32 A20 = (i16)(5394 << 1), A21 = (i16)(20623 << 1);
@@ -153,20 +216,13 @@
     S[1] = s1;
     wv_sync();
 #else
+    (void)A20; (void)A21;
     i32 s0 = S[0], s1 = S[1];
     for (int k = 0; k < (N >> 1); k++) {
-        i32 in32 = sx_shl((i32)in[2 * k], 10);
-        i32 Y = sx_sub(in32, s0);
-        i32 X = sx_smlawb(Y, Y, A21);
-        i32 out_1 = sx_add(s0, X);
-        s0 = sx_add(in32, X);
-        in32 = sx_shl((i32)in[2 * k + 1], 10);
-        Y = sx_sub(in32, s1);
-        X = sx_smulwb(Y, A20);
-        i32 out_2 = sx_add(s1, X);
-        s1 = sx_add(in32, X);
-        outL[k] = (i16)sx_sat16(sx_rshift_round(sx_add(out_2, out_1), 11));
-        outH[k] = (i16)sx_sat16(sx_rshift_round(sx_sub(out_2, out_1), 11));
+        i32 lo, hi;
+        sx_ana_filt_pair(in[2 * k], in[2 * k + 1], s0, s1, lo, hi);
+        outL[k] = (i16)lo;
+        outH[k] = (i16)hi;
     }
     S[0] = s0;
     S[1] = s1;
@@ -224,31 +280,7 @@
         const i32 last = part[4 * b + 3];
         e = sx_add_pos_sat32(e, last >> 1);
         v->XnrgSubfr[b] = last;
-        i32 nl = v->NL[b];
-        {
-            const i32 nrg = sx_add_pos_sat32(e, v->NoiseLevelBias[b]);
-            const i32 inv_nrg = SX_I32_MAX / nrg;
-            i32 coef;
-            if (nrg > sx_shl(nl, 3)) coef = 1024 >> 3;
-            else if (nrg < nl) coef = 1024;
-            else coef = sx_smulwb(sx_smulww(inv_nrg, nl), 1024 << 1);
-            coef = sx_max(coef, min_coef);
-            v->inv_NL[b] = sx_smlawb(v->inv_NL[b], inv_nrg - v->inv_NL[b], coef);
-            nl = SX_I32_MAX / v->inv_NL[b];
-            nl = sx_min(nl, 0x00FFFFFF);
-            v->NL[b] = nl;
-        }
-        i32 ratio = 256, sq = 0, tilt = 0;
-        const i32 speech_nrg_b = e - nl;
-        if (speech_nrg_b > 0) {
-            if ((e & 0xFF800000) == 0) ratio = sx_shl(e, 8) / (nl + 1);
-            else ratio = e / ((nl >> 8) + 1);
-            i32 SNR_Q7 = sx_lin2log(ratio) - 8 * 128;
-            sq = sx_smulbb(SNR_Q7, SNR_Q7);
-            if (speech_nrg_b < (1 << 20)) SNR_Q7 = sx_smulwb(sx_shl(sx_sqrt_approx(speech_nrg_b), 6), SNR_Q7);
-            tilt = sx_smulwb(T_vad_tilt_weights[b], SNR_Q7);
-        }
-        part[4 * b] = ratio; part[4 * b + 1] = sq; part[4 * b + 2] = tilt; part[4 * b + 3] = (b + 1) * (speech_nrg_b >> 4);
+        sx_vad_band_terms(b, e, min_coef, v->NoiseLevelBias[b], v->NL[b], v->inv_NL[b], &part[4 * b]);
     }
     v->counter++;
     wv_sync();
@@ -258,23 +290,8 @@
         input_tilt = sx_add(input_tilt, part[4 * b + 2]);
         speech_nrg = sx_add(speech_nrg, part[4 * b + 3]);
     }
-    sumSquared = sumSquared / 4;
-    *pSNR_dB_Q7 = (i16)(3 * sx_sqrt_approx(sumSquared));
-    i32 SA_Q15 = sx_sigm_Q15(sx_smulwb(45000, *pSNR_dB_Q7) - 128);
-    c->input_tilt_Q15 = sx_shl(sx_sigm_Q15(input_tilt) - 16384, 1);
-    if (speech_nrg <= 0) {
-        SA_Q15 = SA_Q15 >> 1;
-    } else if (speech_nrg < 32768) {
-        speech_nrg = sx_sqrt_approx(sx_shl(speech_nrg, 15));
-        SA_Q15 = sx_smulwb(32768 + speech_nrg, SA_Q15);
-    }
-    st->speech_activity_Q8 = sx_min(SA_Q15 >> 7, 255);
-    i32 smooth_coef_Q16 = (i16)sx_smulwb(4096, sx_smulwb(SA_Q15, SA_Q15));
-    SX_PAR(b, 4) {
-        v->NrgRatioSmth_Q8[b] = sx_smlawb(v->NrgRatioSmth_Q8[b], part[4 * b] - v->NrgRatioSmth_Q8[b], smooth_coef_Q16);
-        i32 SNR_Q7 = 3 * (sx_lin2log(v->NrgRatioSmth_Q8[b]) - 8 * 128);
-        c->input_quality_bands_Q15[b] = sx_sigm_Q15((SNR_Q7 - 16 * 128) >> 4);
-    }
+    const i32 smooth_coef_Q16 = sx_vad_frame_terms(sumSquared, input_tilt, speech_nrg, pSNR_dB_Q7, &c->input_tilt_Q15, &st->speech_activity_Q8);
+    SX_PAR(b, 4) c->input_quality_bands_Q15[b] = sx_vad_band_quality(v->NrgRatioSmth_Q8[b], part[4 * b], smooth_coef_Q16);
     wv_sync();
 }
 
diff --git a/solo_amd/csrc/solo_enc_kernels.h b/solo_amd/csrc/solo_enc_kernels.h
--- a/solo_amd/csrc/solo_enc_kernels.h
+++ b/solo_amd/csrc/solo_enc_kernels.h
@@ -1,5 +1,8 @@
 #pragma once
 #include <hip/hip_runtime.h>
+#if !defined(SX_TU_FRONT) && !defined(SX_NO_PREPASS) && (!defined(SX_FS_KHZ) || SX_FS_KHZ == 8)
+#define SX_ENC_PREPASS 1
+#endif
 #include "solo_enc.h"
 #include "solo_stream_ctl.h"
 
@@ -39,7 +42,12 @@
     wv_sync();
     const i32* src = (const i32*)&w->st;
     i32* dst = (i32*)&rec->core;
+#ifdef SX_ENC_PREPASS
+    constexpr int v0 = (int)(offsetof(SxEncState, vad) / 4), v1 = v0 + (int)(sizeof(SxVAD) / 4);
+    SX_PAR(i, (int)(sizeof(SxEncState) / 4)) { if (i < v0 || i >= v1) dst[i] = src[i]; }
+#else
     SX_PAR(i, (int)(sizeof(SxEncState) / 4)) dst[i] = src[i];
+#endif
 }
 
 #ifndef SX_ANALYSIS_WAVES
@@ -49,9 +57,24 @@
 #define SX_ANALYSIS_PRIO 3
 #endif
 #ifndef SX_TU_FRONT
+#ifdef SX_ENC_PREPASS
+#ifndef SX_PRE_STREAMS
+#define SX_PRE_STREAMS 8
+#endif
+__global__ void __launch_bounds__(64, SX_ANALYSIS_WAVES) SX_K(solo_enc_pre_kernel)(SxEncStream* states, const i16* __restrict__ pcm, int n_streams, int n_packets, int p0, int pc,
+                                                                i16* lo, SxPreOut* pre, SxCodeIn* code_in, const i32* __restrict__ map, const u32* verdict) {
+    __shared__ __attribute__((aligned(16))) i16 tl[63 + SX_PACKET + 1];
+    if (sx_map_refused(map, verdict)) return;
+    const int base = (int)blockIdx.x * SX_PRE_STREAMS;
+    const int cnt = n_streams - base < SX_PRE_STREAMS ? n_streams - base : SX_PRE_STREAMS;
+    if (cnt <= 0) return;
+    sx_enc_pre(states, map, pcm, base, cnt, n_packets, p0, pc, tl, lo, pre, code_in);
+}
+#endif
 __global__ void __launch_bounds__(64, SX_ANALYSIS_WAVES) SX_K(solo_enc_analysis_kernel)(SxEncStream* states, const i16* __restrict__ pcm, int n_streams,
                                                                   int n_packets, int p0, int pc, SxNsqIn* __restrict__ nsq_in,
-                                                                  SxCodeIn* __restrict__ code_in, const i32* __restrict__ map, const u32* verdict) {
+                                                                  SxCodeIn* __restrict__ code_in, const i16* __restrict__ lo,
+                                                                  const SxPreOut* __restrict__ pre, const i32* __restrict__ map, const u32* verdict) {
     __shared__ SxEncWork w;
     const int s = blockIdx.x;
     if (s >= n_streams || sx_map_refused(map, verdict)) return;
@@ -66,7 +89,11 @@
     SX_K(solo_enc_enter)(&w, rec);
     for (int p = p0; p < p0 + pc; p++) {
         const size_t pk = (size_t)s * n_packets + p;
+#ifdef SX_ENC_PREPASS
+        sx_enc_stage_a(rec, &w, lo + pk * SX_BAND, pre + pk * 2, nsq_in + pk * 2, code_in + pk);
+#else
         sx_enc_stage_a(rec, &w, pcm + pk * (size_t)(SX_FRAME * 2 * SX_UNI(w.st.fpp)), nsq_in + pk * 2, code_in + pk);
+#endif
         wv_sync();
     }
     SX_K(solo_enc_leave)(&w, rec);
@@ -324,10 +351,27 @@
 static hipError_t SX_K(solo_enc_launch_ctl_list)(void* states, const SxStreamCtl* recs, int n, hipStream_t s) {
     return sx_launch_ctl_batches(recs, n, [&](const SxStreamCtlList& l, int k) { hipLaunchKernelGGL(SX_K(solo_enc_ctl_list_kernel), dim3(k), dim3(64), 0, s, (SxEncStream*)states, l, k); });
 }
+#ifdef SX_ENC_PREPASS
+static hipError_t SX_K(solo_enc_launch_pre)(void* states, const int16_t* pcm, int n_streams, int n_packets, int p0, int pc, void* lo, void* pre, void* code_in,
+                                            const int32_t* map, const uint32_t* verdict, hipStream_t s) {
+    hipLaunchKernelGGL(SX_K(solo_enc_pre_kernel), dim3((n_streams + SX_PRE_STREAMS - 1) / SX_PRE_STREAMS), dim3(64), 0, s, (SxEncStream*)states, pcm, n_streams, n_packets, p0, pc, (i16*)lo,
+                       (SxPreOut*)pre, (SxCodeIn*)code_in, map, verdict);
+    return hipGetLastError();
+}
+#endif
 static hipError_t SX_K(solo_enc_launch_analysis)(void* states, const int16_t* pcm, int n_streams, int n_packets, int p0, int pc, void* nsq_in,
-                                                 void* code_in, const int32_t* map, const uint32_t* verdict, hipStream_t s) {
+                                                 void* code_in, void* lo, void* pre, int with_pre, const int32_t* map, const uint32_t* verdict, hipStream_t s) {
+#ifdef SX_ENC_PREPASS
+    if (!lo || !pre) return hipErrorInvalidValue;
+    if (with_pre) {
+        const hipError_t e = SX_K(solo_enc_launch_pre)(states, pcm, n_streams, n_packets, p0, pc, lo, pre, code_in, map, verdict, s);
+        if (e != hipSuccess) return e;
+    }
+#else
+    (void)with_pre;
+#endif
     hipLaunchKernelGGL(SX_K(solo_enc_analysis_kernel), dim3(n_streams), dim3(64), 0, s, (SxEncStream*)states, pcm, n_streams, n_packets, p0, pc,
-                       (SxNsqIn*)nsq_in, (SxCodeIn*)code_in, map, verdict);
+                       (SxNsqIn*)nsq_in, (SxCodeIn*)code_in, (const i16*)lo, (const SxPreOut*)pre, map, verdict);
     return hipGetLastError();
 }
 static size_t SX_K(solo_enc_rc_scratch_bytes)(int n_streams, int pc) {
@@ -378,6 +422,11 @@
                                                   unsigned int* started, hipStream_t s);
 static const solo_enc_ops SX_K(solo_enc_ops_table) = {
     sizeof(SxEncStream), sizeof(SxNsqIn), sizeof(SxNsqOut), sizeof(SxCodeIn), SX_PACKET,
+#ifdef SX_ENC_PREPASS
+    SX_BAND * sizeof(i16), sizeof(SxPreOut), SX_K(solo_enc_launch_pre),
+#else
+    0, 0, nullptr,
+#endif
     SX_K(solo_enc_launch_init), SX_K(solo_enc_launch_init_list), SX_K(solo_enc_launch_ctl_list), SX_K(solo_enc_launch_analysis), SX_K(solo_launch_nsq), SX_K(solo_enc_launch_coding), SX_K(solo_enc_rc_scratch_bytes),
     SX_K(solo_nsq_workgroups), SX_K(solo_nsq_ring_bytes), SX_K(solo_enc_launch_front), SX_K(solo_launch_nsq_persist), SX_K(solo_enc_front_scratch_bytes), SX_K(solo_nsq_persist_workgroups), SX_K(solo_nsq_stage_bytes),
     SX_FRONT_WAVES, SX_FRONT_PER_CU};
diff --git a/solo_amd/csrc/solo_enc_ops.h b/solo_amd/csrc/solo_enc_ops.h
--- a/solo_amd/csrc/solo_enc_ops.h
+++ b/solo_amd/csrc/solo_enc_ops.h
@@ -8,11 +8,14 @@
 struct solo_enc_ops {
     size_t state_bytes, nsq_in_bytes, nsq_out_bytes, code_in_bytes;
     int packet_samples;
+    size_t lo_bytes, pre_out_bytes;
+    hipError_t (*pre)(void* states, const int16_t* pcm, int n_streams, int n_packets, int p0, int pc, void* lo, void* pre_out, void* code_in,
+                      const int32_t* map, const uint32_t* verdict, hipStream_t s);
     hipError_t (*init)(void* states, int n_streams, int silk_rate_bps, int useMDIndex, int hb_joint, int useDTX, int frames_per_packet, hipStream_t s);
     hipError_t (*init_list)(void* states, const SxStreamCtl* recs, int n, int hb_joint, int frames_per_packet, hipStream_t s);
     hipError_t (*ctl_list)(void* states, const SxStreamCtl* recs, int n, hipStream_t s);
-    hipError_t (*analysis)(void* states, const int16_t* pcm, int n_streams, int n_packets, int p0, int pc, void* nsq_in, void* code_in, const int32_t* map,
-                           const uint32_t* verdict, hipStream_t s);
+    hipError_t (*analysis)(void* states, const int16_t* pcm, int n_streams, int n_packets, int p0, int pc, void* nsq_in, void* code_in, void* lo,
+                           void* pre_out, int with_pre, const int32_t* map, const uint32_t* verdict, hipStream_t s);
     int (*nsq)(void* states, const void* in, void* out, int n_streams, int n_packets, int p0, int pc, unsigned int* started, void* ring, const int32_t* map,
                const uint32_t* verdict, void* hip_stream);
     hipError_t (*coding)(void* states, const void* code_in, const void* nsq_out, int n_streams, int n_packets, int p0, int pc, int slot,
diff --git a/solo_amd/csrc/solo_enc_pre.h b/solo_amd/csrc/solo_enc_pre.h
--- /dev/null
+++ b/solo_amd/csrc/solo_enc_pre.h
@@ -0,0 +1,116 @@
+#pragma once
+#include "solo_enc_front.h"
+
+struct alignas(16) SxPreOut {
+    i32 speech_activity_Q8, SNR_dB_Q7;
+    i32 input_quality_bands_Q15[4];
+    i32 input_tilt_Q15;
+    i32 pad_;
+    SxVAD vad;
+};
+static_assert(sizeof(SxVAD) == 28 * 4 && sizeof(SxPreOut) == 144, "SxPreOut: 8 words for the analysis kernel, the detector's state behind them");
+
+struct alignas(16) SxV8h { i16 v[8]; };
+
+SX_HD void sx_vad_lane(SxVAD& v, const i16* pIn, SxPreOut* o) {
+    constexpr int steps = SX_FRAME >> 3, qsteps = steps >> 2;
+    static_assert(steps % 4 == 0, "a quarter of a frame is a whole number of eight-sample steps");
+    i32 e[4], last[4] = {0, 0, 0, 0};
+#pragma unroll
+    for (int b = 0; b < 4; b++) e[b] = v.XnrgSubfr[b];
+    i32 a0 = v.AnaState[0], a1 = v.AnaState[1], b0 = v.AnaState1[0], b1 = v.AnaState1[1], c0 = v.AnaState2[0], c1 = v.AnaState2[1];
+    i32 hprev = (i16)v.HPstate;
+    const SxV8h* in8 = (const SxV8h*)(const void*)pIn;
+    SxV8h nxt = in8[0];
+    i32 sum[4] = {0, 0, 0, 0};
+    int q = 0, tq = 0;
+#pragma clang loop unroll(disable)
+    for (int t = 0; t < steps; t++) {
+        const SxV8h x = nxt;
+        if (t + 1 < steps) nxt = in8[t + 1];
+        i32 l1[4], l2[2];
+#pragma unroll
+        for (int u = 0; u < 4; u++) {
+            i32 h;
+            sx_ana_filt_pair(x.v[2 * u], x.v[2 * u + 1], a0, a1, l1[u], h);
+            h >>= 3;
+            sum[3] = sx_smlabb(sum[3], h, h);
+        }
+#pragma unroll
+        for (int u = 0; u < 2; u++) {
+            i32 h;
+            sx_ana_filt_pair(l1[2 * u], l1[2 * u + 1], b0, b1, l2[u], h);
+            h >>= 3;
+            sum[2] = sx_smlabb(sum[2], h, h);
+        }
+        i32 l3, h3;
+        sx_ana_filt_pair(l2[0], l2[1], c0, c1, l3, h3);
+        h3 >>= 3;
+        sum[1] = sx_smlabb(sum[1], h3, h3);
+        const i32 hp = (i16)(l3 >> 1);
+        const i32 d = (i16)(hp - hprev) >> 3;
+        hprev = hp;
+        sum[0] = sx_smlabb(sum[0], d, d);
+        if (++tq == qsteps) {
+#pragma unroll
+            for (int b = 0; b < 4; b++) {
+                if (q < 3) e[b] = sx_add_pos_sat32(e[b], sum[b]);
+                else { e[b] = sx_add_pos_sat32(e[b], sum[b] >> 1); last[b] = sum[b]; }
+                sum[b] = 0;
+            }
+            tq = 0;
+            q++;
+        }
+    }
+    v.AnaState[0] = a0; v.AnaState[1] = a1; v.AnaState1[0] = b0; v.AnaState1[1] = b1; v.AnaState2[0] = c0; v.AnaState2[1] = c1;
+    v.HPstate = hprev;
+    const i32 min_coef = v.counter < 1000 ? 32767 / ((v.counter >> 4) + 1) : 0;
+    i32 t4[4][4];
+    i32 sumSquared = 0, input_tilt = 0, speech_nrg = 0;
+#pragma unroll
+    for (int b = 0; b < 4; b++) {
+        v.XnrgSubfr[b] = last[b];
+        sx_vad_band_terms(b, e[b], min_coef, v.NoiseLevelBias[b], v.NL[b], v.inv_NL[b], t4[b]);
+        sumSquared = sx_add(sumSquared, t4[b][1]);
+        input_tilt = sx_add(input_tilt, t4[b][2]);
+        speech_nrg = sx_add(speech_nrg, t4[b][3]);
+    }
+    v.counter++;
+    const i32 smooth_coef_Q16 = sx_vad_frame_terms(sumSquared, input_tilt, speech_nrg, &o->SNR_dB_Q7, &o->input_tilt_Q15, &o->speech_activity_Q8);
+#pragma unroll
+    for (int b = 0; b < 4; b++) o->input_quality_bands_Q15[b] = sx_vad_band_quality(v.NrgRatioSmth_Q8[b], t4[b][0], smooth_coef_Q16);
+    o->pad_ = 0;
+    o->vad = v;
+}
+
+template <typename CodeIn>
+SX_HD void sx_enc_pre(SxEncStream* states, const i32* map, const i16* pcm, int base, int cnt, int n_packets, int p0, int pc, i16* tl, i16* lo, SxPreOut* pre,
+                      CodeIn* code_in) {
+    for (int j = 0; j < cnt; j++) {
+        const int s = base + j;
+        SxEncStream* rec = &states[map ? SX_UNI(map[s]) : s];
+        const int fpp = SX_UNI(rec->core.fpp);
+        for (int p = p0; p < p0 + pc; p++) {
+            const size_t pk = (size_t)s * n_packets + p;
+            sx_qmf_decomp(&rec->hist, pcm + pk * (size_t)(SX_FRAME * 2 * fpp), tl, lo + pk * SX_BAND, code_in[pk].hi, fpp * 2 * SX_FRAME);
+        }
+    }
+    wv_sync();
+#if SX_NLANES == 1
+    for (int j = 0; j < cnt; j++)
+#else
+    const int j = (int)(threadIdx.x & 63u);
+    if (j < cnt)
+#endif
+    {
+        const int s = base + j;
+        SxEncState* st = &states[map ? map[s] : s].core;
+        SxVAD v = st->vad;
+        const int fpp = st->fpp;
+        for (int p = p0; p < p0 + pc; p++) {
+            const size_t pk = (size_t)s * n_packets + p;
+            for (int frame = 0; frame < fpp; frame++) sx_vad_lane(v, lo + pk * SX_BAND + frame * SX_FRAME, &pre[pk * 2 + frame]);
+        }
+        st->vad = v;
+    }
+}
```

Result: slower. 3.870 million 40ms packets/s (encode+decode) (-1.5%).
